# ZihaoW123/UniMM

Hardware: AMD Instinct MI355X
Metric: dialog-sequences/sec (fwd+bwd) at bs=240 seq=256 regions=36(+1 <IMG>) (higher is better)
Workload: dtype bf16; 1 GPU; UniMM-UL sparse training step (BASELINE configs[1]): bert_base_6layer_6conect, sequences_per_image=6, num_negative_samples=5, mask_prob=0.15, dropout on, MLM+UL / NSP / region-KL losses, fwd+bwd, optimizer step not included; global_batch=240, per_gpu_batch=240, seq_len=256, regions=37, parallelism=dp1, executor=eager launches, step_api=loss = combine(losses); loss.backward() (autograd, as train.py:164-168, :315)

## Files before the change

include/unimm_hip.h:

```cpp
#ifndef UNIMM_HIP_H
#define UNIMM_HIP_H

#include <stdint.h>

#ifdef __cplusplus
extern "C" {
#endif

#define UNIMM_OK 0
#define UNIMM_E_ARG (-1)
#define UNIMM_E_SHAPE (-2)
#define UNIMM_E_ALIGN (-3)
#define UNIMM_E_HIP (-4)

int unimm_version(void);
const char* unimm_arch(void);

enum {
  UNIMM_EPI_BIAS = 0,
  UNIMM_EPI_BIAS_GELU = 1,
  UNIMM_EPI_BIAS_DROP_RESID = 2,
  UNIMM_EPI_BIAS_RELU = 3,
  UNIMM_EPI_DGELU = 4,
  UNIMM_EPI_ADD = 5,
  UNIMM_EPI_MUL = 6,
  UNIMM_EPI_BIAS_GELU_DG = 7
};

typedef struct {
  const void* x;
  const void* w;
  const float* bias;
  const void* aux;
  void* out;
  void* out2;
  int32_t M, N, K;
  int32_t ldx, ldw, ldaux, ldo;
  int32_t epilogue;
  int32_t out_f32;
  uint32_t drop_key;
  uint32_t drop_thr;
  float drop_scale;
  const float* aux_mean;
  const float* aux_rstd;
  const float* aux_gamma;
  const float* aux_beta;
  int32_t tile;
  const uint32_t* drop_salt;
  void* splitk_ws;
  int64_t splitk_ws_bytes;
  int32_t splitk;
} unimm_gemm_nt_args;

int unimm_gemm_nt(const unimm_gemm_nt_args* args, void* stream);

typedef struct {
  const void* dy;
  const void* x;
  float* dw;
  float* dbias;
  int32_t M, N, K;
  int32_t lddy, ldx, lddw;
  const int32_t* m_dev;
  int32_t overwrite;
} unimm_gemm_tn_args;

int unimm_gemm_tn(const unimm_gemm_tn_args* args, void* stream);
int unimm_gemm_tn_grouped(const unimm_gemm_tn_args* args, int32_t count, void* stream);
int unimm_gemm_tn_grouped_ws(const unimm_gemm_tn_args* args, int32_t count, int32_t shared_chip, void* ws, int64_t ws_bytes,
                             void* stream);

typedef struct {
  const void* q; const void* k; const void* v;
  void* out;
  float* lse;
  const uint32_t* mask;
  const int32_t* q_off; const int32_t* q_len; const int32_t* k_off; const int32_t* k_len;
  int32_t B, H, Tq, Tk, D;
  int32_t ldq, ldk, ldv, ldo;
  int32_t mask_q_stride, mask_b_stride;
  float scale;
  uint32_t drop_key, drop_thr; float drop_scale;
  const uint32_t* drop_salt;
  const int32_t* ks_off; const int32_t* ks_len;
  int32_t ks_ins;
  const int32_t* order;
} unimm_attn_args;

int unimm_attn_fwd(const unimm_attn_args* args, void* stream);

int unimm_attn_probs(const unimm_attn_args* args, float* probs, void* stream);

typedef struct {
  const void* q; const void* k; const void* v; const void* out; const void* dout;
  const float* lse; float* delta;
  void* dq; void* dk; void* dv;
  const uint32_t* mask;
  const int32_t* q_off; const int32_t* q_len; const int32_t* k_off; const int32_t* k_len;
  int32_t B, H, Tq, Tk, D;
  int32_t ldq, ldk, ldv, ldo, lddo, lddq, lddk, lddv;
  int32_t mask_q_stride, mask_b_stride;
  float scale;
  uint32_t drop_key, drop_thr; float drop_scale;
  const uint32_t* drop_salt;
  const int32_t* order;
} unimm_attn_bwd_args;

int unimm_attn_bwd(const unimm_attn_bwd_args* args, void* stream);

enum { UNIMM_DT_U8 = 0, UNIMM_DT_I32 = 1, UNIMM_DT_I64 = 2, UNIMM_DT_F32 = 3 };

int unimm_mask_pack(const void* mask, int dtype, uint32_t* out, int64_t rows, int32_t t, void* stream);
int unimm_host_mask_pack(const void* mask, int dtype, uint32_t* out, int64_t rows, int32_t t, int32_t threads);
int unimm_host_memcpy(void* dst, const void* src, int64_t bytes, int32_t threads);
int unimm_mask_synth(const int32_t* mode, const int32_t* len, const int32_t* nans, uint32_t* text_words, uint32_t* co_words,
                     int32_t B, int32_t T, void* stream);

int unimm_plan_lengths(const uint32_t* text_words, int32_t t_q_stride, int32_t t_b_stride, const uint32_t* co_words,
                       int32_t c_q_stride, int32_t c_b_stride, int32_t R, const int32_t* labels, const int32_t* weights,
                       const float* nsp_weight, const int32_t* image_label, int32_t B, int32_t T, int32_t* header,
                       void* stream);
int unimm_plan_build(const int32_t* header, const int32_t* labels, const int32_t* weights, int32_t B, int32_t T,
                     int32_t* off, int32_t* lens, int64_t* rows, int64_t* inv, int32_t* lm_pos, int32_t* lm_idx,
                     int32_t* lm_label, int32_t* lm_weight, int32_t rows_cap, int32_t lm_cap, int32_t* dims_i, float* dims_f,
                     int32_t* order, void* stream);

int unimm_layernorm_fwd(const float* x, const float* gamma, const float* beta, float* y32, void* y16, float* mean,
                        float* rstd, int32_t M, int32_t H, float eps, uint32_t drop_key, uint32_t drop_thr,
                        float drop_scale, const uint32_t* drop_salt, void* stream);

int64_t unimm_colpartials_bytes(int32_t H);

int unimm_layernorm_bwd(const void* dy, const float* x, const float* mean, const float* rstd, const float* gamma,
                        void* dx, void* dx_drop, float* dgamma, float* dbeta, float* dbias, float* partials,
                        int32_t M, int32_t H, uint32_t drop_key, uint32_t drop_thr, float drop_scale,
                        uint32_t odrop_key, uint32_t odrop_thr, float odrop_scale, const uint32_t* drop_salt, void* stream);
int unimm_layernorm_bwd_partials(const void* dy, const float* x, const float* mean, const float* rstd, const float* gamma,
                                 void* dx, void* dx_drop, float* partials, int32_t M, int32_t H, uint32_t drop_key,
                                 uint32_t drop_thr, float drop_scale, uint32_t odrop_key, uint32_t odrop_thr,
                                 float odrop_scale, int32_t* blocks_out, const int32_t* m_dev, const uint32_t* drop_salt,
                                 void* stream);
#define UNIMM_FINISH_MAX 8
typedef struct {
  const float* partials;
  float* dst[4];
  int32_t blocks, nq, H, pad_;
} unimm_finish_desc;
int unimm_colpartials_finish_grouped(const unimm_finish_desc* descs, int32_t count, void* stream);

typedef struct {
  const int32_t* ids; const int32_t* pos; const int32_t* typ;
  const float* word; const float* post; const float* type; const float* ext;
  const float* gamma; const float* beta;
  int32_t M, H, type_vocab;
  float eps;
  uint32_t drop_key, drop_thr; float drop_scale;
  const int32_t* m_dev;
  const int64_t* rows;
  const uint32_t* drop_salt;
} unimm_embed_args;

int unimm_embed_fwd(const unimm_embed_args* args, float* y32, void* y16, void* stream);
int unimm_embed_bwd(const unimm_embed_args* args, const void* dy, float* dword, float* dpos, float* dtype,
                    float* dext, float* dgamma, float* dbeta, float* partials, void* stream);

int unimm_colsum(const void* dy, float* db, int32_t M, int32_t N, int32_t ld, void* stream);

int unimm_cast_f32_bf16(const float* src, void* dst, int64_t n, void* stream);
int unimm_transpose_cast(const float* src, void* dst, int32_t R, int32_t C, int32_t ldd, void* stream);
int unimm_transpose_bf16(const void* src, void* dst, int32_t R, int32_t C, int32_t lds, int32_t ldd, void* stream);
int unimm_sum_slabs_bf16(const float* slabs, int32_t count, int64_t stride, void* out, int64_t n, void* stream);
typedef struct {
  const float* src;
  void* dst;
  int32_t R, C, ldd, tile0;
} unimm_transpose_desc;
int unimm_transpose_cast_grouped(const unimm_transpose_desc* table, int32_t count, int32_t total_tiles, void* stream);

int unimm_pack_image(const float* feat, const float* loc, void* out, int32_t rows, int32_t F, int32_t ld, void* stream);

int unimm_mul_dropout(const float* a, const float* b, float* out, int64_t n, uint32_t drop_key, uint32_t drop_thr,
                      float drop_scale, const uint32_t* drop_salt, void* stream);
int unimm_mul_dropout_bwd(const float* a, const float* b, const float* dout, float* da, float* db, int64_t n,
                          uint32_t drop_key, uint32_t drop_thr, float drop_scale, const uint32_t* drop_salt, void* stream);

int unimm_sum_dropout(const float* a, const float* b, float* out, int64_t n, uint32_t drop_key, uint32_t drop_thr,
                      float drop_scale, const uint32_t* drop_salt, void* stream);
int unimm_sum_dropout_bwd(const float* a, const float* b, const float* dout, float* da, float* db, int64_t n,
                          uint32_t drop_key, uint32_t drop_thr, float drop_scale, const uint32_t* drop_salt, void* stream);

typedef struct {
  const float* a; const float* b; const float* bias; float* out; float* rowsum;
  int32_t M, N, K;
  int64_t sa_m, sa_k, sb_k, sb_n, ldo;
// ... 147 lines not shown
```

unimm_amd/bucket_plan.py:

```python
from __future__ import annotations

from typing import List, Tuple

from . import params as PM

ARENA_ALIGN = 64
CHIP_SLOTS = 256


def big_tiles_of(M: int, N: int, K: int) -> int:
    if N >= 256 and K >= 256 and M >= 1024:
        return ((N + 255) // 256) * ((K + 255) // 256)
    return 0


def flush_due(n_problems: int, tiles: int, rounds: int) -> bool:
    if n_problems >= 40:
        return True
    if tiles >= rounds * CHIP_SLOTS:
        return True
    waste = (-tiles) % CHIP_SLOTS
    return tiles >= max(2, rounds // 2) * CHIP_SLOTS - 32 and waste <= CHIP_SLOTS // 8


def arena_ranges(cfg) -> List[Tuple[str, int, int]]:
    out, off = [], 0
    for gname, items in PM.arena_groups(cfg):
        lo = off
        for _, shape in items:
            n = 1
            for s in shape:
                n *= s
            off += (n + ARENA_ALIGN - 1) // ARENA_ALIGN * ARENA_ALIGN
        out.append((gname, lo, off))
    return out


def _self_block(h, inter):
    return [(h, inter), (inter, h), (h, h), (3 * h, h)]


def backward_events(cfg, n_seq: int, text_rows: int, lm_rows: int, regions: int = 37, dual_stream: bool = True,
                    image_head_side: bool = True):
    del dual_stream
    H, Hv, Hb = cfg.hidden_size, cfg.v_hidden_size, cfg.bi_hidden_size
    I, Iv = cfg.intermediate_size, cfg.v_intermediate_size
    Mt, Mi = text_rows, n_seq * regions
    img = 1
    ev = []
    hs = img if image_head_side else 0
    ev.append(("w", hs, Mi, cfg.v_target_size, Hv))
    ev.append(("w", hs, Mi, Hv, Hv))
    if lm_rows > 0:
        ev.append(("w", 0, lm_rows, cfg.vocab_size, H))
        ev.append(("w", 0, lm_rows, H, H))
    ev.append(("b", "heads", False, True, False))
    sched = PM.encoder_schedule(cfg)
    entries = list(reversed(sched))
    pos = 0
    tail_done = False

    def image_tail():
        nonlocal tail_done
        if tail_done or any(k in ("c", "v") for k, _ in entries[pos:]):
            return
        tail_done = True
        ev.extend([("w", img, Mi, Hv, cfg.v_feature_size), ("w", img, Mi, Hv, 5)])
        ev.append(("b", "image_embeddings", bool(img), False, True))

    while pos < len(entries):
        image_tail()
        seg = []
        while pos < len(entries) and entries[pos][0] != "c":
            seg.append(entries[pos])
            pos += 1
        for kind, i in seg:
            if kind == "v":
                ev += [("w", img, Mi, n, k) for n, k in _self_block(Hv, Iv)]
                ev.append(("b", f"v{i}", bool(img), False, False))
        for kind, i in seg:
            if kind == "t":
                ev += [("w", 0, Mt, n, k) for n, k in _self_block(H, I)]
                ev.append(("b", f"t{i}", False, False, False))
        if pos < len(entries):
            _, i = entries[pos]
            pos += 1
            ev += [("w", img, Mi, Hv, Iv), ("w", img, Mi, Iv, Hv), ("w", img, Mi, Hv, Hb)]
            ev += [("w", 0, Mt, H, I), ("w", 0, Mt, I, H), ("w", 0, Mt, H, Hb)]
            ev += [("w", img, Mi, 3 * Hb, Hv), ("w", 0, Mt, 3 * Hb, H)]
            ev.append(("b", f"c{i}", False, False, False))
    image_tail()
    ev.append(("b", "text_embeddings", False, True, False))
    return ev


def hand_overs(cfg, n_seq, text_rows, lm_rows, regions=37, wgrad_group_rounds=2, dual_stream=True, image_head_side=True):
    q = [[], []]
    nq, nf = [0, 0], [0, 0]
    pending, calls, launches = [], [], []

    def flush(side):
        if q[side]:
            launches.append((side, len(q[side]), sum(big_tiles_of(*p) for p in q[side])))
        q[side] = []
        nf[side] = nq[side]

    def due(side):
        return flush_due(len(q[side]), sum(big_tiles_of(*p) for p in q[side]), wgrad_group_rounds)

    for e in backward_events(cfg, n_seq, text_rows, lm_rows, regions, dual_stream, image_head_side):
        if e[0] == "w":
            _, side, M, N, K = e
            q[side].append((M, N, K))
            nq[side] += 1
            continue
        _, group, on_side, force, force_img = e
        pending.append((group, nq[0], nq[1]))
        if q[1] and (force or force_img or due(1)):
            flush(1)
        if not on_side and (force or due(0)):
            flush(0)
        if on_side:
            continue
        ready = [p for p in pending if nf[0] >= p[1] and nf[1] >= p[2]]
        pending = [p for p in pending if p not in ready]
        calls += [(g, j + 1 < len(ready)) for j, (g, _, _) in enumerate(ready)]
    assert not pending, pending
    return calls, launches


def collectives(cfg, calls):
    ranges = {g: (lo, hi) for g, lo, hi in arena_ranges(cfg)}
    out, run = [], None
    for group, more in calls:
        lo, hi = ranges[group]
        if run and (run[0] == hi or run[1] == lo):
            run = [min(lo, run[0]), max(hi, run[1]), run[2] + 1]
        else:
            if run:
                out.append(tuple(run))
            run = [lo, hi, 1]
        if not more:
            out.append(tuple(run))
            run = None
    assert run is None
    return out


def exchange_plan(cfg, n_seq, text_rows, lm_rows, **kw):
    calls, launches = hand_overs(cfg, n_seq, text_rows, lm_rows, **kw)
    cs = collectives(cfg, calls)
    return dict(calls=calls, launches=launches, collectives=cs, bytes=[(hi - lo) * 4 for lo, hi, _ in cs])
```

unimm_amd/csrc/api.hip:

```cpp
#include "common.h"

extern "C" int unimm_version(void) { return 19; }
extern "C" const char* unimm_arch(void) { return "gfx950"; }
```

unimm_amd/csrc/gemm.hip:

```cpp
#include "gemm_nt.h"

struct ProfRec { hipEvent_t a, b; int variant; int tag; double flops; };
int unimm_nt_launch_cfg1(const GemmNtParams& p, int epi, bool out_f32, int want_persist, hipStream_t s, const NtSplit& sk);
int unimm_nt_launch_cfg3(const GemmNtParams& p, int epi, bool out_f32, int want_persist, hipStream_t s, const NtSplit& sk);
int unimm_nt_launch_cfg6(const GemmNtParams& p, int epi, bool out_f32, int want_persist, hipStream_t s, const NtSplit& sk);
int unimm_nt_launch_cfg7(const GemmNtParams& p, int epi, bool out_f32, int want_persist, hipStream_t s, const NtSplit& sk);
int unimm_nt_launch_cfg8(const GemmNtParams& p, int epi, bool out_f32, int want_persist, hipStream_t s, const NtSplit& sk);
int unimm_nt_launch_cfg9(const GemmNtParams& p, int epi, bool out_f32, int want_persist, hipStream_t s, const NtSplit& sk);
int unimm_nt_launch_cfg10(const GemmNtParams& p, int epi, bool out_f32, int want_persist, hipStream_t s, const NtSplit& sk);
int unimm_nt_launch_cfg12(const GemmNtParams& p, int epi, bool out_f32, int want_persist, hipStream_t s, const NtSplit& sk);
int unimm_nt_launch_cfg14(const GemmNtParams& p, int epi, bool out_f32, int want_persist, hipStream_t s, const NtSplit& sk);
int unimm_nt_launch_cfg15(const GemmNtParams& p, int epi, bool out_f32, int want_persist, hipStream_t s, const NtSplit& sk);

int unimm_cu_count() {
  static int n = 0;
  if (n == 0) {
    int dev = 0;
    hipDeviceProp_t prop;
    if (hipGetDevice(&dev) == hipSuccess && hipGetDeviceProperties(&prop, dev) == hipSuccess) n = prop.multiProcessorCount;
    if (n <= 0) n = 256;
    if (n < 8) n = 8;
  }
  return n;
}
// ... 562 lines not shown
      for (const Cand& c : cand) {
        const long tiles = (long)((p.M + c.bm - 1) / c.bm) * ((p.N + c.bn - 1) / c.bn);
        const long slots = (long)cus * c.w;
        const double area = (double)c.bm * c.bn / 65536.0;
        const long rem = tiles % slots;
        const double cost = ((double)(tiles / slots) * c.w + (rem ? (double)((rem + cus - 1) / cus) : 0.0)) * area / c.eff;
        if (cost < best) { best = cost; cfg = c.cfg; }
      }
    }
  }
  if (cfg == 8 && ((size_t)p.M * (size_t)p.ldx * 2 >= ((size_t)1 << 32) || (size_t)p.N * (size_t)p.ldw * 2 >= ((size_t)1 << 32))) cfg = 3;
  if (cfg == 8) return unimm_nt_launch_cfg8(p, epi, out_f32, wp, s, nosplit);
  if (cfg == 6) return unimm_nt_launch_cfg6(p, epi, out_f32, wp, s, nosplit);
  if (cfg == 7) return unimm_nt_launch_cfg7(p, epi, out_f32, wp, s, sk);
  if (cfg == 9) return unimm_nt_launch_cfg9(p, epi, out_f32, wp, s, sk);
  if (cfg == 10) return unimm_nt_launch_cfg10(p, epi, out_f32, wp, s, sk);
  if (cfg == 3) return unimm_nt_launch_cfg3(p, epi, out_f32, wp, s, nosplit);
  if (cfg == 12) return unimm_nt_launch_cfg12(p, epi, out_f32, wp, s, nosplit);
  if (cfg == 14) return unimm_nt_launch_cfg14(p, epi, out_f32, wp, s, sk);
  if (cfg == 15) return unimm_nt_launch_cfg15(p, epi, out_f32, wp, s, sk);
  return unimm_nt_launch_cfg1(p, epi, out_f32, wp, s, sk);
}

}

ProfRec* unimm_prof_begin(int variant, double flops, hipStream_t s) { return prof_begin(variant, flops, s); }
void unimm_prof_end(ProfRec* r, hipStream_t s) { prof_end(r, s); }

extern "C" int unimm_gemm_nt(const unimm_gemm_nt_args* a, void* stream) {
  if (a == nullptr || a->x == nullptr || a->w == nullptr || a->out == nullptr) return UNIMM_E_ARG;
  if (a->M <= 0 || a->N <= 0 || a->K <= 0 || (a->K % 64) != 0) return UNIMM_E_SHAPE;
  if ((a->ldx % 8) || (a->ldw % 8) || a->ldx < a->K || a->ldw < a->K || a->ldo < a->N) return UNIMM_E_ALIGN;
  if (((uintptr_t)a->x | (uintptr_t)a->w | (uintptr_t)a->out) & 15) return UNIMM_E_ALIGN;
  if (a->out_f32 ? (a->ldo % 4) : (a->ldo % 4)) return UNIMM_E_ALIGN;
  const bool needs_aux = a->epilogue == UNIMM_EPI_BIAS_DROP_RESID || a->epilogue == UNIMM_EPI_DGELU ||
                         a->epilogue == UNIMM_EPI_ADD || a->epilogue == UNIMM_EPI_MUL;
  if (needs_aux && (a->aux == nullptr || (a->ldaux % 4) || a->ldaux < a->N)) return UNIMM_E_ARG;
  if (a->epilogue == UNIMM_EPI_BIAS_DROP_RESID && !a->out_f32) return UNIMM_E_ARG;
  if (((needs_aux ? (uintptr_t)a->aux : 0) | (uintptr_t)a->out2) & 15) return UNIMM_E_ALIGN;
  GemmNtParams p;
  p.x = (const bf16_t*)a->x; p.w = (const bf16_t*)a->w; p.bias = a->bias; p.aux = a->aux;
  p.out = a->out; p.out2 = (bf16_t*)a->out2;
  p.M = a->M; p.N = a->N; p.K = a->K; p.ldx = a->ldx; p.ldw = a->ldw; p.ldaux = a->ldaux; p.ldo = a->ldo;
  p.drop.key = a->drop_key; p.drop.thr = a->drop_thr; p.drop.scale = a->drop_scale; p.drop.salt = a->drop_salt;
  const int n_ln = (a->aux_mean != nullptr) + (a->aux_rstd != nullptr) + (a->aux_gamma != nullptr) + (a->aux_beta != nullptr);
  if (n_ln != 0 && (n_ln != 4 || a->epilogue != UNIMM_EPI_BIAS_DROP_RESID)) return UNIMM_E_ARG;
  p.aux_mean = a->aux_mean; p.aux_rstd = a->aux_rstd; p.aux_gamma = a->aux_gamma; p.aux_beta = a->aux_beta;
  NtTune tune;
  if (!nt_tune_decode(a->tile, tune)) return UNIMM_E_ARG;
  p.gn = tune.gn > 0 ? tune.gn : 4;
  hipStream_t s = (hipStream_t)stream;
  const bool f32 = a->out_f32 != 0;
  p.ksplit = 1; p.slabs = nullptr; p.counters = nullptr;
  if (a->splitk != 0 && a->splitk != 1 && (a->splitk_ws == nullptr || a->splitk_ws_bytes < 32768 || ((uintptr_t)a->splitk_ws & 255) ||
                                           a->splitk > 8 || a->splitk < -1))
    return UNIMM_E_ARG;
  const NtSplit sk{a->splitk, a->splitk_ws, (long)a->splitk_ws_bytes};
  if (a->epilogue < 0 || a->epilogue > UNIMM_EPI_BIAS_GELU_DG) return UNIMM_E_ARG;
  return launch_nt(p, a->epilogue, f32, tune, s, sk);
}

namespace {

int check_tn(const unimm_gemm_tn_args* a) {
  if (a->dy == nullptr || a->x == nullptr || a->dw == nullptr) return UNIMM_E_ARG;
  if (a->M <= 0 || a->N <= 0 || a->K <= 0) return UNIMM_E_SHAPE;
  if ((a->lddy % 8) || (a->ldx % 8) || a->lddy < a->N || a->ldx < a->K || a->lddw < a->K) return UNIMM_E_ALIGN;
  if (((uintptr_t)a->dy | (uintptr_t)a->x) & 15) return UNIMM_E_ALIGN;
  return UNIMM_OK;
}

inline bool tn_is_big(const unimm_gemm_tn_args* a) { return a->N >= 256 && a->K >= 256 && a->M >= 1024; }

int launch_tn_group(const unimm_gemm_tn_args* const* a, int count, bool big, bool shared, bool legacy_loop, void* ws,
                    int64_t ws_bytes, hipStream_t s) {
  GemmTnGroup g;
  const int tb = big ? 256 : 128;
  int tiles = 0, max_m = 0;
  double flops = 0.0;
  const unimm_gemm_tn_args* sorted[TN_MAXG];
  for (int i = 0; i < count; ++i) sorted[i] = a[i];
#ifndef UNIMM_TN_NOSORT
  for (int i = 1; i < count; ++i) {
    const unimm_gemm_tn_args* x = sorted[i];
    int j = i - 1;
    while (j >= 0 && sorted[j]->M < x->M) { sorted[j + 1] = sorted[j]; --j; }
    sorted[j + 1] = x;
  }
#endif
  a = sorted;
  for (int i = 0; i < count; ++i) {
    GemmTnParams& p = g.pr[i];
    p.dy = (const bf16_t*)a[i]->dy; p.x = (const bf16_t*)a[i]->x; p.dw = a[i]->dw; p.dbias = a[i]->dbias;
    p.m_dev = a[i]->m_dev;
    p.overwrite = a[i]->overwrite;
    p.M = a[i]->M; p.N = a[i]->N; p.K = a[i]->K; p.lddy = a[i]->lddy; p.ldx = a[i]->ldx; p.lddw = a[i]->lddw;
    p.tile0 = tiles;
    tiles += ((p.N + tb - 1) / tb) * ((p.K + tb - 1) / tb);
    max_m = p.M > max_m ? p.M : max_m;
    flops += 2.0 * p.M * (double)p.N * p.K;
  }
  g.count = count; g.total_tiles = tiles;
  const int slots = big ? 256 : 512;
  int max_s = max_m / 1024;
  max_s = max_s < 1 ? 1 : (max_s > 32 ? 32 : max_s);
  int splits = 1;
// ... 148 lines not shown
```

unimm_amd/csrc/gemm_nt.h:

```cpp
#pragma once
#include <type_traits>
#include "common.h"
#include <stdlib.h>

struct GemmNtParams {
  const bf16_t* x; const bf16_t* w; const float* bias; const void* aux;
  void* out; bf16_t* out2;
  int M, N, K, ldx, ldw, ldaux, ldo;
  int gn;
  DropoutArg drop;
  const float* aux_mean; const float* aux_rstd; const float* aux_gamma; const float* aux_beta;
  int ksplit; float* slabs; int* counters;
};
struct NtSplit { int want; void* ws; long ws_bytes; };

struct ProfRec;
ProfRec* unimm_prof_begin(int variant, double flops, hipStream_t s);
void unimm_prof_end(ProfRec* r, hipStream_t s);
int unimm_cu_count();

namespace {

__device__ __forceinline__ void tile_of(int lid, int nbm, int nbn, int gn, int& tm, int& tn) {
  const int per_group = nbm * gn;
  const int g = lid / per_group;
  const int r = lid - g * per_group;
  const int gw = (nbn - g * gn) < gn ? (nbn - g * gn) : gn;
  tm = r / gw;
  tn = g * gn + (r - tm * gw);
}

template <int WM_, int WN_, int MT_, int BK_, int STAGES_, int PP_ = 0, int XS_ = 0>
struct Cfg {
  static constexpr int WM = WM_, WN = WN_, MT = MT_, BK = BK_, STAGES = STAGES_;
  static constexpr int XS = XS_ ? XS_ : STAGES_;
  static constexpr bool PP = PP_ != 0;
  static constexpr int BM = 16 * MT * WM, BN = 64 * WN, NW = WM * WN, THREADS = 64 * NW;
  static constexpr int ROWB = BK * 2;
  static constexpr int RPI = 1024 / ROWB;
  static constexpr int STAGE_BYTES = (BM + BN) * ROWB;
  static constexpr int G = (BM + BN) / RPI / NW;
  static constexpr int JP = MT == 6 ? 3 : (MT < 4 ? MT : 4);
  static constexpr int SLAB_ROWS = 16 * JP;
  static constexpr int SLAB_BYTES = NW * SLAB_ROWS * 68 * 4;
  static constexpr int WB = BN * ROWB, XB = BM * ROWB;
  static constexpr int GW = BN / RPI / NW, GX = BM / RPI / NW;
  static constexpr int RING_BYTES = STAGES * WB + XS * XB;
  static constexpr int LDS = RING_BYTES > SLAB_BYTES ? RING_BYTES : SLAB_BYTES;
  static constexpr int WG_PER_CU = LDS <= 53 * 1024 ? 3 : (LDS <= 80 * 1024 ? 2 : 1);
  static constexpr int MIN_WAVES = (WG_PER_CU * NW + 3) / 4;
  static_assert((BM + BN) % (RPI * NW) == 0, "tile rows must split evenly over the waves");
};

template <int BK> __device__ __forceinline__ int kswz(int row) { return BK == 64 ? ((row >> 1) & 7) : ((row >> 2) & 3); }

template <class C> struct RingStage {
  uint32_t so[C::G];
  u32x4 srd_w, srd_x;
  uint32_t lds;
};
template <class C>
__device__ __forceinline__ void ring_stage_init(RingStage<C>& st, const GemmNtParams& p, int n0, int m0, uint32_t lds0, int wave, int lane) {
  constexpr int CPR = C::ROWB / 16;
  static_assert(C::BN % (C::RPI * C::NW) == 0, "an LDS-DMA instruction round must not straddle the W / X boundary");
  const uint64_t bw = (uint64_t)(uintptr_t)(p.w + (size_t)n0 * p.ldw), bx = (uint64_t)(uintptr_t)(p.x + (size_t)m0 * p.ldx);
// ... 239 lines not shown
      (void)pfa1; (void)pfamu; (void)pfars;
      if (m >= p.M || !ncols_ok) continue;
      if constexpr (PRE) {
        uint32_t pw[8];
#pragma unroll
        for (int e = 0; e < 4; ++e) { pw[e] = __float_as_uint(lo[e]); pw[4 + e] = __float_as_uint(hi[e]); }
        bf16_t* op = reinterpret_cast<bf16_t*>(p.out) + (size_t)m * p.ldo + n;
        bf16_t* up = p.out2 != nullptr ? p.out2 + (size_t)m * p.ldo + n : nullptr;
        if (vec_out) {
          u32x4 ow, uw;
#pragma unroll
          for (int k2 = 0; k2 < 4; ++k2) {
            ow[k2] = __builtin_amdgcn_perm(pw[2 * k2 + 1], pw[2 * k2], 0x05040100u);
            uw[k2] = __builtin_amdgcn_perm(pw[2 * k2 + 1], pw[2 * k2], 0x07060302u);
          }
          __builtin_nontemporal_store(ow, reinterpret_cast<u32x4*>(op));
          if (up != nullptr) __builtin_nontemporal_store(uw, reinterpret_cast<u32x4*>(up));
        } else {
          for (int e = 0; e < 8; ++e)
            if (n + e < p.N) {
              op[e] = (bf16_t)(pw[e] & 0xffffu);
              if (up != nullptr) up[e] = (bf16_t)(pw[e] >> 16);
            }
        }
        continue;
      }
      float v[8], u[8];
#pragma unroll
      for (int e = 0; e < 4; ++e) { v[e] = lo[e] + b[e]; v[4 + e] = hi[e] + b[4 + e]; }
      if constexpr (EPI == UNIMM_EPI_BIAS_DROP_RESID || EPI == UNIMM_EPI_DGELU || EPI == UNIMM_EPI_ADD || EPI == UNIMM_EPI_MUL) {
        float a[8];
        if constexpr (EPI == UNIMM_EPI_BIAS_DROP_RESID) {
          const float* ap = reinterpret_cast<const float*>(p.aux) + (size_t)m * p.ldaux;
          if (vec_aux) {
            f32x4 r0, r1;
            if (PF > 0) { r0 = pfa0; r1 = pfa1; }
            else {
              r0 = __builtin_nontemporal_load(reinterpret_cast<const f32x4*>(ap + colA));
              r1 = __builtin_nontemporal_load(reinterpret_cast<const f32x4*>(ap + colB));
            }
#pragma unroll
            for (int e = 0; e < 4; ++e) { a[e] = r0[e]; a[4 + e] = r1[e]; }
          } else {
#pragma unroll
            for (int e = 0; e < 8; ++e) a[e] = (n + e < p.N) ? ap[n + e] : 0.f;
          }
          if (aux_ln) {
            const bool pfd = PF > 0 && (FAST || pf_on);
            const float mu = pfd ? pfamu : p.aux_mean[m], rs = pfd ? pfars : p.aux_rstd[m];
#pragma unroll
            for (int e = 0; e < 8; ++e) a[e] = (a[e] - mu) * rs * lg[e] + lb[e];
          }
          if (p.drop.thr != 0u) {
            const uint32_t kb = (SPLITCOL && FAST)
                ? (drop_bits4(p.drop, (uint32_t)m, (uint32_t)p.N, (uint32_t)colA) | (drop_bits4(p.drop, (uint32_t)m, (uint32_t)p.N, (uint32_t)colB) << 4))
                : drop_bits8(p.drop, (uint32_t)m, (uint32_t)p.N, (uint32_t)n);
#pragma unroll
            for (int e = 0; e < 8; ++e) v[e] = ((kb >> e) & 1u) ? v[e] * p.drop.scale : 0.f;
          }
#pragma unroll
          for (int e = 0; e < 8; ++e) v[e] += a[e];
        } else {
          const bf16_t* ap = reinterpret_cast<const bf16_t*>(p.aux) + (size_t)m * p.ldaux + n;
          if (vec_aux) {
            const u32x4 raw = PF > 0 ? __builtin_bit_cast(u32x4, pfa0)
                                     : __builtin_nontemporal_load(reinterpret_cast<const u32x4*>(ap));
#pragma unroll
            for (int e = 0; e < 4; ++e) { a[2 * e] = __uint_as_float(raw[e] << 16); a[2 * e + 1] = __uint_as_float(raw[e] & 0xffff0000u); }
          } else {
#pragma unroll
            for (int e = 0; e < 8; ++e) a[e] = (n + e < p.N) ? bf2f(ap[e]) : 0.f;
          }
          if constexpr (EPI == UNIMM_EPI_DGELU) {
#pragma unroll
            for (int e = 0; e < 8; ++e) v[e] *= gelu_erf_grad(a[e]);
          } else if constexpr (EPI == UNIMM_EPI_MUL) {
#pragma unroll
            for (int e = 0; e < 8; ++e) v[e] *= a[e];
          } else {
#pragma unroll
            for (int e = 0; e < 8; ++e) v[e] += a[e];
          }
        }
      }
      if constexpr (EPI == UNIMM_EPI_BIAS_GELU || EPI == UNIMM_EPI_BIAS_GELU_DG) {
        if constexpr (EPI == UNIMM_EPI_BIAS_GELU) {
#pragma unroll
          for (int e = 0; e < 8; ++e) { u[e] = v[e]; v[e] = gelu_erf(v[e]); }
        } else {
#pragma unroll
          for (int e = 0; e < 8; ++e) { const float x = v[e]; gelu_and_grad(x, v[e], u[e]); }
        }
        if (p.out2 != nullptr) {
          bf16_t* up = p.out2 + (size_t)m * p.ldo + n;
          if (full && (p.ldo % 8) == 0)
            __builtin_nontemporal_store(u32x4{pack2bf(u[0], u[1]), pack2bf(u[2], u[3]), pack2bf(u[4], u[5]), pack2bf(u[6], u[7])},
                                        reinterpret_cast<u32x4*>(up));
          else
            for (int e = 0; e < 8; ++e) if (n + e < p.N) up[e] = f2bf(u[e]);
        }
      }
      if constexpr (EPI == UNIMM_EPI_BIAS_RELU) {
#pragma unroll
        for (int e = 0; e < 8; ++e) v[e] = fmaxf(v[e], 0.f);
      }
      if constexpr (OUT_F32) {
        float* op = reinterpret_cast<float*>(p.out) + (size_t)m * p.ldo;
        if (vec_out) {
          __builtin_nontemporal_store(f32x4{v[0], v[1], v[2], v[3]}, reinterpret_cast<f32x4*>(op + colA));
// ... 454 lines not shown
```

unimm_amd/csrc/rowops.hip:

```cpp
#include "common.h"
#include "rows.h"

namespace {

template <typename T>
__global__ void mask_pack_ballot_kernel(const T* __restrict__ m, uint32_t* __restrict__ out, size_t ngroups) {
  const size_t wave = (size_t)blockIdx.x * (blockDim.x >> 6) + (threadIdx.x >> 6);
  const size_t nwaves = (size_t)gridDim.x * (blockDim.x >> 6);
  const int lane = threadIdx.x & 63;
  for (size_t g = wave; g < ngroups; g += nwaves) {
    const bool bit = m[g * 64 + lane] != (T)0;
    const unsigned long long bal = __ballot(bit);
    if (lane == 0) {
      out[2 * g] = (uint32_t)bal;
      out[2 * g + 1] = (uint32_t)(bal >> 32);
    }
  }
}

template <typename T>
__global__ void mask_pack_generic_kernel(const T* __restrict__ m, uint32_t* __restrict__ out, size_t rows, int t,
                                         int nw) {
  const size_t i = (size_t)blockIdx.x * blockDim.x + threadIdx.x;
  if (i >= rows * nw) return;
// ... 144 lines not shown
    if (rows != nullptr) for (int i = mv + t; i < rows_cap; i += 256) rows[i] = 0;
    if (lm_pos != nullptr)
      for (int i = nlm + t; i < lm_cap; i += 256) { lm_pos[i] = 0; lm_idx[i] = 0; lm_lab[i] = -1; lm_w[i] = 0; }
    if (order != nullptr)
      for (int i = t; i < B; i += 256) {
        const int li = header[i];
        int rank = 0;
        for (int j = 0; j < B; ++j) { const int lj = header[j]; rank += (lj > li || (lj == li && j < i)) ? 1 : 0; }
        order[rank] = i;
      }
    return;
  }
  int a = 0, c = 0;
  for (int i = t; i < b; i += 256) { a += header[i]; c += header[B + i]; }
  for (int o = 32; o > 0; o >>= 1) { a += __shfl_xor(a, o, 64); c += __shfl_xor(c, o, 64); }
  __shared__ int pa[4], pc[4];
  if ((t & 63) == 0) { pa[t >> 6] = a; pc[t >> 6] = c; }
  __syncthreads();
  if (t == 0) { s_off = pa[0] + pa[1] + pa[2] + pa[3]; s_lmoff = pc[0] + pc[1] + pc[2] + pc[3]; }
  __syncthreads();
  int len = header[b], o0 = s_off;
  if (rows != nullptr && o0 + len > rows_cap) {
    o0 = min(o0, rows_cap - 1);
    len = max(1, min(len, rows_cap - o0));
  }
  if (t == 0) { off[b] = o0; lens[b] = len; }
  if (t < T) {
    const bool in = t < len;
    if (in && rows != nullptr) rows[o0 + t] = (int64_t)b * T + t;
    if (inv != nullptr) inv[(size_t)b * T + t] = in ? (int64_t)(o0 + t) : (int64_t)-1;
  }
  if (labels == nullptr || lm_pos == nullptr) return;
  const int lab = t < T ? labels[(size_t)b * T + t] : -1;
  const int wt = (weights != nullptr && t < T) ? weights[(size_t)b * T + t] : 0;
  const bool sel = t < T && (weights != nullptr ? wt != 0 : lab != -1);
  const unsigned long long bal = __ballot(sel);
  const int lane = t & 63, wv = t >> 6;
  if (lane == 0) wave_cnt[wv] = __popcll(bal);
  __syncthreads();
  if (sel) {
    int r = __popcll(bal & ((1ull << lane) - 1ull));
    for (int w = 0; w < wv; ++w) r += wave_cnt[w];
    const int dst = s_lmoff + r;
    if (dst < lm_cap) {
      lm_pos[dst] = b * T + t;
      lm_idx[dst] = rows != nullptr ? min(o0 + t, rows_cap - 1) : o0 + t;
      lm_lab[dst] = lab;
      lm_w[dst] = weights != nullptr ? wt : 1;
    }
  }
}


__global__ __launch_bounds__(256) void layernorm_fwd_kernel(const float* __restrict__ x, const float* __restrict__ gamma,
                                                            const float* __restrict__ beta, float* __restrict__ y32,
                                                            bf16_t* __restrict__ y,
                                                            float* __restrict__ mean_o, float* __restrict__ rstd_o, int M,
                                                            int H, float eps, DropoutArg drop) {
  drop_resolve(drop);
  const int lane = threadIdx.x & 63;
  const int wave = blockIdx.x * (blockDim.x >> 6) + (threadIdx.x >> 6);
  const int nwaves = gridDim.x * (blockDim.x >> 6);
  Row8 g, b;
  load_vec_f32(gamma, H, lane, g);
  load_vec_f32(beta, H, lane, b);
  Row8 xv;
  if (wave < M) load_vec_f32(x + (size_t)wave * H, H, lane, xv);
  for (int row = wave; row < M; row += nwaves) {
    Row8 nx;
    const int nrow = row + nwaves;
    if (nrow < M) load_vec_f32(x + (size_t)nrow * H, H, lane, nx);
    float mean, rstd;
    row_stats(xv, H, mean, rstd, eps);
#pragma unroll
    for (int i = 0; i < MAXC; ++i) {
      const uint32_t kb = drop.thr != 0u ? drop_bits8(drop, (uint32_t)row, (uint32_t)H, (uint32_t)((lane + 64 * i) * 8)) : 0u;
#pragma unroll
      for (int j = 0; j < 8; ++j) {
        float v = (xv.v[i][j] - mean) * rstd * g.v[i][j] + b.v[i][j];
        if (drop.thr != 0u) v = ((kb >> j) & 1u) ? v * drop.scale : 0.f;
        xv.v[i][j] = v;
      }
    }
    if (y32 != nullptr) store_row_f32(y32 + (size_t)row * H, H, lane, xv);
    if (y != nullptr) store_row_bf16(y + (size_t)row * H, H, lane, xv);
    if (lane == 0 && mean_o != nullptr) { mean_o[row] = mean; rstd_o[row] = rstd; }
    if (nrow < M) xv = nx;
  }
}

__global__ __launch_bounds__(256) void layernorm_bwd_kernel(const bf16_t* __restrict__ dy, const float* __restrict__ x,
                                                            const float* __restrict__ mean_i,
                                                            const float* __restrict__ rstd_i,
                                                            const float* __restrict__ gamma, bf16_t* __restrict__ dx,
                                                            bf16_t* __restrict__ dx_drop, float* __restrict__ partials,
                                                            int M, int H, DropoutArg drop, DropoutArg out_drop,
                                                            const int32_t* __restrict__ m_dev) {
  __shared__ float red[4 * 1024];
  drop_resolve(drop);
  drop_resolve(out_drop);
  if (m_dev != nullptr) M = min(M, m_dev[0]);
  const int lane = threadIdx.x & 63, wv = threadIdx.x >> 6;
  const int wave = blockIdx.x * 4 + wv;
  const int nwaves = gridDim.x * 4;
  Row8 g;
  load_vec_f32(gamma, H, lane, g);
  Row8 dg, db, dbias;
#pragma unroll
  for (int i = 0; i < MAXC; ++i)
#pragma unroll
    for (int j = 0; j < 8; ++j) { dg.v[i][j] = 0.f; db.v[i][j] = 0.f; dbias.v[i][j] = 0.f; }
  const float invH = 1.0f / (float)H;
  u32x4 pdy[MAXC];
  f32x4 pxa[MAXC], pxb[MAXC];
  float pmean = 0.f, prstd = 0.f;
#define UNIMM_LNB_PREFETCH(r_)                                                                                 \
  {                                                                                                            \
    _Pragma("unroll") for (int i = 0; i < MAXC; ++i) {                                                         \
      const int c = lane + 64 * i;                                                                             \
      if (c * 8 < H) {                                                                                         \
        pdy[i] = *reinterpret_cast<const u32x4*>(dy + (size_t)(r_) * H + c * 8);                               \
        pxa[i] = *reinterpret_cast<const f32x4*>(x + (size_t)(r_) * H + c * 8);                                \
        pxb[i] = *reinterpret_cast<const f32x4*>(x + (size_t)(r_) * H + c * 8 + 4);                            \
      }                                                                                                        \
    }                                                                                                          \
    pmean = mean_i[r_]; prstd = rstd_i[r_];                                                                    \
  }
  if (wave < M) UNIMM_LNB_PREFETCH(wave)
  for (int row = wave; row < M; row += nwaves) {
    Row8 dyv, xv;
#pragma unroll
    for (int i = 0; i < MAXC; ++i) {
      if ((lane + 64 * i) * 8 < H) {
#pragma unroll
        for (int j = 0; j < 4; ++j) {
          dyv.v[i][2 * j] = __uint_as_float(pdy[i][j] << 16);
          dyv.v[i][2 * j + 1] = __uint_as_float(pdy[i][j] & 0xffff0000u);
          xv.v[i][j] = pxa[i][j];
          xv.v[i][4 + j] = pxb[i][j];
        }
      } else {
#pragma unroll
        for (int j = 0; j < 8; ++j) { dyv.v[i][j] = 0.f; xv.v[i][j] = 0.f; }
      }
    }
    const float mean = pmean, rstd = prstd;
    if (row + nwaves < M) UNIMM_LNB_PREFETCH(row + nwaves)
    float s1 = 0.f, s2 = 0.f;
#pragma unroll
    for (int i = 0; i < MAXC; ++i) {
      const uint32_t kbo = out_drop.thr != 0u ? drop_bits8(out_drop, (uint32_t)row, (uint32_t)H, (uint32_t)((lane + 64 * i) * 8)) : 0u;
#pragma unroll
      for (int j = 0; j < 8; ++j) {
        float d = dyv.v[i][j];
        if (out_drop.thr != 0u) d = ((kbo >> j) & 1u) ? d * out_drop.scale : 0.f;
        const float xh = (xv.v[i][j] - mean) * rstd;
        const float gg = d * g.v[i][j];
        dg.v[i][j] += d * xh;
        db.v[i][j] += d;
        s1 += gg;
        s2 += gg * xh;
        dyv.v[i][j] = gg;
        xv.v[i][j] = xh;
      }
    }
    s1 = wave_sum(s1) * invH;
    s2 = wave_sum(s2) * invH;
    Row8 dd;
#pragma unroll
    for (int i = 0; i < MAXC; ++i) {
      const uint32_t kb = drop.thr != 0u ? drop_bits8(drop, (uint32_t)row, (uint32_t)H, (uint32_t)((lane + 64 * i) * 8)) : 0u;
#pragma unroll
      for (int j = 0; j < 8; ++j) {
        const float v = rstd * (dyv.v[i][j] - s1 - xv.v[i][j] * s2);
        dyv.v[i][j] = v;
        float vd = v;
        if (drop.thr != 0u) vd = ((kb >> j) & 1u) ? v * drop.scale : 0.f;
        dd.v[i][j] = vd;
        dbias.v[i][j] += vd;
      }
    }
    store_row_bf16(dx + (size_t)row * H, H, lane, dyv);
    if (dx_drop != nullptr) store_row_bf16(dx_drop + (size_t)row * H, H, lane, dd);
  }
#undef UNIMM_LNB_PREFETCH
  float* redf = red;
  for (int qn = 0; qn < 3; ++qn) {
    const Row8& src = qn == 0 ? dg : (qn == 1 ? db : dbias);
    __syncthreads();
#pragma unroll
    for (int i = 0; i < MAXC; ++i)
#pragma unroll
      for (int j = 0; j < 8; ++j) {
        const int col = (lane + 64 * i) * 8 + j;
        if (col < H) redf[wv * 1024 + col] = src.v[i][j];
      }
    __syncthreads();
    for (int col = threadIdx.x; col < H; col += 256)
      partials[((size_t)blockIdx.x * 3 + qn) * H + col] =
          redf[col] + redf[1024 + col] + redf[2048 + col] + redf[3072 + col];
  }
}

__global__ __launch_bounds__(1024) void colpartials_finish_kernel(const float* __restrict__ partials, int nblocks, int nq,
                                                                  int H, float* d0, float* d1, float* d2, float* d3) {
  __shared__ float red[16][64];
  const int cl = threadIdx.x & 63, sl = threadIdx.x >> 6;
  const int col = blockIdx.x * 64 + cl;
  const int qn = blockIdx.y;
  float* dst = qn == 0 ? d0 : (qn == 1 ? d1 : (qn == 2 ? d2 : d3));
  float s = 0.f;
  if (col < H && dst != nullptr) {
    float s0 = 0.f, s1 = 0.f, s2 = 0.f, s3 = 0.f, s4 = 0.f, s5 = 0.f, s6 = 0.f, s7 = 0.f;
    int b = sl;
    const size_t st = (size_t)16 * nq * H;
    const float* pp = partials + ((size_t)b * nq + qn) * H + col;
    for (; b + 7 * 16 < nblocks; b += 8 * 16, pp += 8 * st) {
      s0 += pp[0]; s1 += pp[st]; s2 += pp[2 * st]; s3 += pp[3 * st];
      s4 += pp[4 * st]; s5 += pp[5 * st]; s6 += pp[6 * st]; s7 += pp[7 * st];
    }
    for (; b < nblocks; b += 16, pp += st) s0 += pp[0];
    s = ((s0 + s1) + (s2 + s3)) + ((s4 + s5) + (s6 + s7));
  }
  red[sl][cl] = s;
// ... 331 lines not shown
      }
    }
    *reinterpret_cast<u32x4*>(out + (size_t)row * ld + c) =
        u32x4{pack2bf(v[0], v[1]), pack2bf(v[2], v[3]), pack2bf(v[4], v[5]), pack2bf(v[6], v[7])};
  }
}

template <bool SUM>
__global__ void mul_dropout_kernel(const float* __restrict__ a, const float* __restrict__ b, float* __restrict__ out,
                                   size_t n, DropoutArg drop) {
  drop_resolve(drop);
  const size_t i = (size_t)blockIdx.x * blockDim.x + threadIdx.x;
  if (i >= n) return;
  float v = SUM ? a[i] + b[i] : a[i] * b[i];
  if (drop.thr != 0u) v = drop_apply(drop, 0u, (uint32_t)n, (uint32_t)i, v);
  out[i] = v;
}

template <bool SUM>
__global__ void mul_dropout_bwd_kernel(const float* __restrict__ a, const float* __restrict__ b,
                                       const float* __restrict__ dout, float* __restrict__ da, float* __restrict__ db,
                                       size_t n, DropoutArg drop) {
  drop_resolve(drop);
  const size_t i = (size_t)blockIdx.x * blockDim.x + threadIdx.x;
  if (i >= n) return;
  float d = dout[i];
  if (drop.thr != 0u) d = drop_apply(drop, 0u, (uint32_t)n, (uint32_t)i, d);
  const float av = a[i], bv = b[i];
  da[i] = av > 0.f ? (SUM ? d : d * bv) : 0.f;
  db[i] = bv > 0.f ? (SUM ? d : d * av) : 0.f;
}

__global__ void gelu_bwd_kernel(const bf16_t* __restrict__ dt, const bf16_t* __restrict__ u, bf16_t* __restrict__ du,
                                size_t n8) {
  size_t i = (size_t)blockIdx.x * blockDim.x + threadIdx.x;
  const size_t stride = (size_t)gridDim.x * blockDim.x;
  for (; i < n8; i += stride) {
    const u32x4 a = *reinterpret_cast<const u32x4*>(dt + i * 8);
    const u32x4 b = *reinterpret_cast<const u32x4*>(u + i * 8);
    u32x4 o;
#pragma unroll
    for (int j = 0; j < 4; ++j) {
      const float d0 = __uint_as_float(a[j] << 16), d1 = __uint_as_float(a[j] & 0xffff0000u);
      const float u0 = __uint_as_float(b[j] << 16), u1 = __uint_as_float(b[j] & 0xffff0000u);
      o[j] = pack2bf(d0 * gelu_erf_grad(u0), d1 * gelu_erf_grad(u1));
    }
    *reinterpret_cast<u32x4*>(du + i * 8) = o;
  }
}

__global__ void gather_rows_kernel(const bf16_t* __restrict__ src, const int32_t* __restrict__ idx, bf16_t* __restrict__ dst,
                                   int n, int H, int scatter, const int32_t* __restrict__ n_dev) {
  if (n_dev != nullptr) n = min(n, n_dev[0]);
  const int cpr = H / 8;
  size_t i = (size_t)blockIdx.x * blockDim.x + threadIdx.x;
  const size_t total = (size_t)n * cpr;
  const size_t stride = (size_t)gridDim.x * blockDim.x;
  for (; i < total; i += stride) {
    const int r = (int)(i / cpr), c = (int)(i % cpr) * 8;
    const int g = idx[r];
    if (scatter) *reinterpret_cast<u32x4*>(dst + (size_t)g * H + c) = *reinterpret_cast<const u32x4*>(src + (size_t)r * H + c);
    else *reinterpret_cast<u32x4*>(dst + (size_t)r * H + c) = *reinterpret_cast<const u32x4*>(src + (size_t)g * H + c);
  }
}

inline DropoutArg mk_drop(uint32_t key, uint32_t thr, float scale, const uint32_t* salt = nullptr) {
  DropoutArg d; d.key = key; d.thr = thr; d.scale = scale; d.salt = salt; d.key2 = 0u; return d;
}

}

extern "C" int unimm_mask_pack(const void* mask, int dtype, uint32_t* out, int64_t rows, int32_t t, void* stream) {
  if (!mask || !out || rows <= 0 || t <= 0) return UNIMM_E_ARG;
  hipStream_t s = (hipStream_t)stream;
  switch (dtype) {
    case UNIMM_DT_U8: return mask_pack_impl<uint8_t>(mask, out, (size_t)rows, t, s);
    case UNIMM_DT_I32: return mask_pack_impl<int32_t>(mask, out, (size_t)rows, t, s);
    case UNIMM_DT_I64: return mask_pack_impl<int64_t>(mask, out, (size_t)rows, t, s);
    case UNIMM_DT_F32: return mask_pack_impl<float>(mask, out, (size_t)rows, t, s);
    default: return UNIMM_E_ARG;
  }
}

extern "C" int unimm_layernorm_fwd(const float* x, const float* gamma, const float* beta, float* y32, void* y16, float* mean,
                                   float* rstd, int32_t M, int32_t H, float eps, uint32_t drop_key, uint32_t drop_thr,
                                   float drop_scale, const uint32_t* drop_salt, void* stream) {
  if (!x || !gamma || !beta || (!y32 && !y16)) return UNIMM_E_ARG;
  if (M <= 0 || H <= 0 || H > MAXC * 512 || (H % 8)) return UNIMM_E_SHAPE;
  int blocks = (M + 3) / 4;
  blocks = blocks > 2048 ? 2048 : blocks;
  hipLaunchKernelGGL(layernorm_fwd_kernel, dim3(blocks), dim3(256), 0, (hipStream_t)stream, x, gamma, beta, y32,
                     (bf16_t*)y16, mean, rstd, M, H, eps, mk_drop(drop_key, drop_thr, drop_scale, drop_salt));
  UNIMM_CHECK_LAUNCH();
  return UNIMM_OK;
}

extern "C" int64_t unimm_colpartials_bytes(int32_t H) { return (int64_t)RED_BLOCKS * 4 * H * sizeof(float); }

extern "C" int unimm_layernorm_bwd(const void* dy, const float* x, const float* mean, const float* rstd, const float* gamma,
                                   void* dx, void* dx_drop, float* dgamma, float* dbeta, float* dbias, float* partials,
                                   int32_t M, int32_t H, uint32_t drop_key, uint32_t drop_thr, float drop_scale,
                                   uint32_t odrop_key, uint32_t odrop_thr, float odrop_scale, const uint32_t* drop_salt,
                                   void* stream) {
  if (!dy || !x || !mean || !rstd || !gamma || !dx || !partials) return UNIMM_E_ARG;
  if (M <= 0 || H <= 0 || H > MAXC * 512 || (H % 8)) return UNIMM_E_SHAPE;
  int blocks = (M + 3) / 4;
  blocks = blocks > RED_BLOCKS ? RED_BLOCKS : blocks;
  hipStream_t s = (hipStream_t)stream;
  hipLaunchKernelGGL(layernorm_bwd_kernel, dim3(blocks), dim3(256), 0, s, (const bf16_t*)dy, x, mean, rstd,
                     gamma, (bf16_t*)dx, (bf16_t*)dx_drop, partials, M, H, mk_drop(drop_key, drop_thr, drop_scale, drop_salt),
                     mk_drop(odrop_key, odrop_thr, odrop_scale, drop_salt), (const int32_t*)nullptr);
  UNIMM_CHECK_LAUNCH();
  hipLaunchKernelGGL(colpartials_finish_kernel, dim3((H + 63) / 64, 3), dim3(1024), 0, s, partials, blocks, 3, H, dgamma,
                     dbeta, dbias, (float*)nullptr);
  UNIMM_CHECK_LAUNCH();
  return UNIMM_OK;
}

extern "C" int unimm_layernorm_bwd_partials(const void* dy, const float* x, const float* mean, const float* rstd,
                                            const float* gamma, void* dx, void* dx_drop, float* partials, int32_t M, int32_t H,
                                            uint32_t drop_key, uint32_t drop_thr, float drop_scale, uint32_t odrop_key,
                                            uint32_t odrop_thr, float odrop_scale, int32_t* blocks_out, const int32_t* m_dev,
                                            const uint32_t* drop_salt, void* stream) {
  if (!dy || !x || !mean || !rstd || !gamma || !dx || !partials || !blocks_out) return UNIMM_E_ARG;
  if (M <= 0 || H <= 0 || H > MAXC * 512 || (H % 8)) return UNIMM_E_SHAPE;
  int blocks = (M + 3) / 4;
  blocks = blocks > RED_BLOCKS ? RED_BLOCKS : blocks;
  hipLaunchKernelGGL(layernorm_bwd_kernel, dim3(blocks), dim3(256), 0, (hipStream_t)stream, (const bf16_t*)dy, x, mean, rstd,
                     gamma, (bf16_t*)dx, (bf16_t*)dx_drop, partials, M, H, mk_drop(drop_key, drop_thr, drop_scale, drop_salt),
                     mk_drop(odrop_key, odrop_thr, odrop_scale, drop_salt), m_dev);
  UNIMM_CHECK_LAUNCH();
  *blocks_out = blocks;
  return UNIMM_OK;
}

extern "C" int unimm_colpartials_finish_grouped(const unimm_finish_desc* descs, int32_t count, void* stream) {
  if (descs == nullptr || count < 1) return UNIMM_E_ARG;
  for (int base = 0; base < count; base += UNIMM_FINISH_MAX) {
    const int n = count - base < UNIMM_FINISH_MAX ? count - base : UNIMM_FINISH_MAX;
    FinishGroup g;
    int hmax = 0, qmax = 0;
    for (int i = 0; i < n; ++i) {
      const unimm_finish_desc& d = descs[base + i];
      if (d.partials == nullptr || d.blocks < 1 || d.nq < 1 || d.nq > 4 || d.H < 1) return UNIMM_E_ARG;
      g.d[i] = d;
      hmax = d.H > hmax ? d.H : hmax;
      qmax = d.nq > qmax ? d.nq : qmax;
    }
    hipLaunchKernelGGL(colpartials_finish_grouped_kernel, dim3((hmax + 63) / 64, qmax, n), dim3(1024), 0, (hipStream_t)stream, g);
    UNIMM_CHECK_LAUNCH();
  }
  return UNIMM_OK;
}

extern "C" int unimm_embed_fwd(const unimm_embed_args* a, float* y32, void* y, void* stream) {
  if (!a || !a->ids || !a->pos || !a->typ || !a->word || !a->post || !a->type || !a->ext || !a->gamma || !a->beta || !y ||
      !y32)
    return UNIMM_E_ARG;
  if (a->M <= 0 || a->H <= 0 || a->H > MAXC * 512 || (a->H % 8)) return UNIMM_E_SHAPE;
  EmbArgs e;
  e.ids = a->ids; e.pos = a->pos; e.typ = a->typ;
  e.word = a->word; e.post = a->post; e.type = a->type;
  e.ext = a->ext; e.gamma = a->gamma; e.beta = a->beta;
  e.M = a->M; e.H = a->H; e.type_vocab = a->type_vocab; e.eps = a->eps;
  e.drop = mk_drop(a->drop_key, a->drop_thr, a->drop_scale, a->drop_salt);
  e.m_dev = a->m_dev; e.rows = a->rows;
  int blocks = (a->M + 3) / 4;
  blocks = blocks > 2048 ? 2048 : blocks;
  hipLaunchKernelGGL(embed_fwd_kernel, dim3(blocks), dim3(256), 0, (hipStream_t)stream, e, y32, (bf16_t*)y);
  UNIMM_CHECK_LAUNCH();
  return UNIMM_OK;
}

namespace {
int embed_bwd_any(const unimm_embed_args* a, const void* dy, bool dy_f32, float* dword, float* dpos, float* dtype,
                  float* dext, float* dgamma, float* dbeta, float* partials, void* stream);
}
extern "C" int unimm_embed_bwd(const unimm_embed_args* a, const void* dy, float* dword, float* dpos, float* dtype,
                               float* dext, float* dgamma, float* dbeta, float* partials, void* stream) {
  return embed_bwd_any(a, dy, false, dword, dpos, dtype, dext, dgamma, dbeta, partials, stream);
}
extern "C" int unimm_embed_bwd_f32(const unimm_embed_args* a, const float* dy, float* dword, float* dpos, float* dtype,
                                   float* dext, float* dgamma, float* dbeta, float* partials, void* stream) {
  return embed_bwd_any(a, dy, true, dword, dpos, dtype, dext, dgamma, dbeta, partials, stream);
}
namespace {
int embed_bwd_any(const unimm_embed_args* a, const void* dy, bool dy_f32, float* dword, float* dpos, float* dtype,
                  float* dext, float* dgamma, float* dbeta, float* partials, void* stream) {
  if (!a || !dy || !dword || !dpos || !dtype || !dext || !dgamma || !dbeta || !partials) return UNIMM_E_ARG;
  if (a->M <= 0 || a->H <= 0 || a->H > MAXC * 512 || (a->H % 8) || a->type_vocab != 2) return UNIMM_E_SHAPE;
  EmbArgs e;
  e.ids = a->ids; e.pos = a->pos; e.typ = a->typ;
  e.word = a->word; e.post = a->post; e.type = a->type;
  e.ext = a->ext; e.gamma = a->gamma; e.beta = a->beta;
  e.M = a->M; e.H = a->H; e.type_vocab = a->type_vocab; e.eps = a->eps;
  e.drop = mk_drop(a->drop_key, a->drop_thr, a->drop_scale, a->drop_salt);
  e.m_dev = a->m_dev; e.rows = a->rows;
  int blocks = (a->M + 3) / 4;
  blocks = blocks > RED_BLOCKS ? RED_BLOCKS : blocks;
  hipStream_t s = (hipStream_t)stream;
  if (dy_f32) hipLaunchKernelGGL(embed_bwd_kernel<float>, dim3(blocks), dim3(256), 0, s, e, (const float*)dy, dword, dpos, dext, partials);
  else hipLaunchKernelGGL(embed_bwd_kernel<bf16_t>, dim3(blocks), dim3(256), 0, s, e, (const bf16_t*)dy, dword, dpos, dext, partials);
  UNIMM_CHECK_LAUNCH();
  hipLaunchKernelGGL(colpartials_finish_kernel, dim3((a->H + 63) / 64, 4), dim3(1024), 0, s, partials, blocks, 4, a->H,
                     dgamma, dbeta, dtype, dtype + a->H);
  UNIMM_CHECK_LAUNCH();
  return UNIMM_OK;
}
}

extern "C" int unimm_plan_lengths(const uint32_t* text_words, int32_t t_q_stride, int32_t t_b_stride, const uint32_t* co_words,
                                  int32_t c_q_stride, int32_t c_b_stride, int32_t R, const int32_t* labels, const int32_t* weights,
                                  const float* nsp_weight, const int32_t* image_label, int32_t B, int32_t T, int32_t* header,
                                  void* stream) {
  if (header == nullptr || (text_words == nullptr && co_words == nullptr && labels == nullptr)) return UNIMM_E_ARG;
  if (B <= 0 || T <= 0 || T > 256 || R < 0 || R > 256) return UNIMM_E_SHAPE;
  hipLaunchKernelGGL(plan_lengths_kernel, dim3(B), dim3(256), 0, (hipStream_t)stream, text_words, t_q_stride, t_b_stride,
                     co_words, c_q_stride, c_b_stride, R, labels, weights, nsp_weight, image_label, B, T, (T + 31) / 32, header);
  UNIMM_CHECK_LAUNCH();
  return UNIMM_OK;
}

extern "C" int unimm_plan_build(const int32_t* header, const int32_t* labels, const int32_t* weights, int32_t B, int32_t T,
                                int32_t* off, int32_t* lens, int64_t* rows, int64_t* inv, int32_t* lm_pos, int32_t* lm_idx,
                                int32_t* lm_label, int32_t* lm_weight, int32_t rows_cap, int32_t lm_cap, int32_t* dims_i,
                                float* dims_f, int32_t* order, void* stream) {
  if ((dims_i == nullptr) != (dims_f == nullptr)) return UNIMM_E_ARG;
  if (header == nullptr || off == nullptr || lens == nullptr) return UNIMM_E_ARG;
  if (lm_pos != nullptr && (lm_idx == nullptr || lm_label == nullptr || lm_weight == nullptr || labels == nullptr)) return UNIMM_E_ARG;
  if (B <= 0 || T <= 0 || T > 256) return UNIMM_E_SHAPE;
  hipLaunchKernelGGL(plan_build_kernel, dim3(B + 1), dim3(256), 0, (hipStream_t)stream, header, labels, weights, B, T, off, lens,
                     rows, inv, lm_pos, lm_idx, lm_label, lm_weight, rows_cap, lm_cap, dims_i, dims_f, order);
  UNIMM_CHECK_LAUNCH();
  return UNIMM_OK;
}

extern "C" int unimm_colsum(const void* dy, float* db, int32_t M, int32_t N, int32_t ld, void* stream) {
  if (!dy || !db) return UNIMM_E_ARG;
  if (M <= 0 || N <= 0 || (ld % 8) || ld < ((N + 7) & ~7)) return UNIMM_E_ALIGN;
  int ysplit = (M + 255) / 256;
  ysplit = ysplit > 64 ? 64 : ysplit;
  hipLaunchKernelGGL(colsum_kernel, dim3((N + 511) / 512, ysplit), dim3(256), 0, (hipStream_t)stream, (const bf16_t*)dy, db,
                     M, N, ld);
  UNIMM_CHECK_LAUNCH();
  return UNIMM_OK;
}

extern "C" int unimm_cast_f32_bf16(const float* src, void* dst, int64_t n, void* stream) {
  if (!src || !dst || n <= 0) return UNIMM_E_ARG;
  if (((uintptr_t)src | (uintptr_t)dst) & 15) return UNIMM_E_ALIGN;
  int64_t blocks = (n / 8 + 255) / 256;
  blocks = blocks > 4096 ? 4096 : (blocks < 1 ? 1 : blocks);
  hipLaunchKernelGGL(cast_f32_bf16_kernel, dim3((unsigned)blocks), dim3(256), 0, (hipStream_t)stream, src, (bf16_t*)dst,
                     (size_t)n);
  UNIMM_CHECK_LAUNCH();
  return UNIMM_OK;
}

extern "C" int unimm_transpose_cast(const float* src, void* dst, int32_t R, int32_t C, int32_t ldd, void* stream) {
  if (!src || !dst || R <= 0 || C <= 0 || ldd < R) return UNIMM_E_ARG;
  hipLaunchKernelGGL(transpose_cast_kernel, dim3((C + 31) / 32, (ldd + 31) / 32), dim3(256), 0, (hipStream_t)stream, src,
                     (bf16_t*)dst, R, C, ldd);
  UNIMM_CHECK_LAUNCH();
  return UNIMM_OK;
}

extern "C" int unimm_transpose_bf16(const void* src, void* dst, int32_t R, int32_t C, int32_t lds, int32_t ldd, void* stream) {
  if (!src || !dst || R <= 0 || C <= 0 || lds < C || ldd < R) return UNIMM_E_ARG;
  if ((lds % 8) || (ldd % 8) || (((uintptr_t)src | (uintptr_t)dst) & 15)) return UNIMM_E_ALIGN;
  hipLaunchKernelGGL(transpose_bf16_kernel, dim3((C + 63) / 64, (ldd + 63) / 64), dim3(256), 0, (hipStream_t)stream,
                     (const bf16_t*)src, (bf16_t*)dst, R, C, lds, ldd);
  UNIMM_CHECK_LAUNCH();
  return UNIMM_OK;
}

extern "C" int unimm_sum_slabs_bf16(const float* slabs, int32_t count, int64_t stride, void* out, int64_t n, void* stream) {
  if (!slabs || !out || count <= 0 || n <= 0 || stride < n) return UNIMM_E_ARG;
  if ((n % 8) || (stride % 4) || (((uintptr_t)slabs | (uintptr_t)out) & 15)) return UNIMM_E_ALIGN;
  int64_t blocks = (n / 8 + 255) / 256;
  blocks = blocks > 2048 ? 2048 : blocks;
  hipLaunchKernelGGL(sum_slabs_bf16_kernel, dim3((unsigned)blocks), dim3(256), 0, (hipStream_t)stream, slabs, count,
                     (size_t)stride, (bf16_t*)out, (size_t)(n / 8));
  UNIMM_CHECK_LAUNCH();
  return UNIMM_OK;
}

extern "C" int unimm_mask_synth(const int32_t* mode, const int32_t* len, const int32_t* nans, uint32_t* text_words,
                                uint32_t* co_words, int32_t B, int32_t T, void* stream) {
  if (!mode || !len || !nans || !text_words || !co_words || B <= 0 || T <= 0) return UNIMM_E_ARG;
// ... 26 lines not shown

extern "C" int unimm_mul_dropout(const float* a, const float* b, float* out, int64_t n, uint32_t drop_key, uint32_t drop_thr,
                                 float drop_scale, const uint32_t* drop_salt, void* stream) {
  if (!a || !b || !out || n <= 0) return UNIMM_E_ARG;
  hipLaunchKernelGGL(mul_dropout_kernel<false>, dim3((unsigned)((n + 255) / 256)), dim3(256), 0, (hipStream_t)stream,
                     a, b, out, (size_t)n, mk_drop(drop_key, drop_thr, drop_scale, drop_salt));
  UNIMM_CHECK_LAUNCH();
  return UNIMM_OK;
}

extern "C" int unimm_mul_dropout_bwd(const float* a, const float* b, const float* dout, float* da, float* db, int64_t n,
                                     uint32_t drop_key, uint32_t drop_thr, float drop_scale, const uint32_t* drop_salt,
                                     void* stream) {
  if (!a || !b || !dout || !da || !db || n <= 0) return UNIMM_E_ARG;
  hipLaunchKernelGGL(mul_dropout_bwd_kernel<false>, dim3((unsigned)((n + 255) / 256)), dim3(256), 0, (hipStream_t)stream,
                     a, b, dout, da, db, (size_t)n,
                     mk_drop(drop_key, drop_thr, drop_scale, drop_salt));
  UNIMM_CHECK_LAUNCH();
  return UNIMM_OK;
}

extern "C" int unimm_sum_dropout(const float* a, const float* b, float* out, int64_t n, uint32_t drop_key, uint32_t drop_thr,
                                 float drop_scale, const uint32_t* drop_salt, void* stream) {
  if (!a || !b || !out || n <= 0) return UNIMM_E_ARG;
  hipLaunchKernelGGL(mul_dropout_kernel<true>, dim3((unsigned)((n + 255) / 256)), dim3(256), 0, (hipStream_t)stream,
                     a, b, out, (size_t)n, mk_drop(drop_key, drop_thr, drop_scale, drop_salt));
  UNIMM_CHECK_LAUNCH();
  return UNIMM_OK;
}

extern "C" int unimm_sum_dropout_bwd(const float* a, const float* b, const float* dout, float* da, float* db, int64_t n,
                                     uint32_t drop_key, uint32_t drop_thr, float drop_scale, const uint32_t* drop_salt,
                                     void* stream) {
  if (!a || !b || !dout || !da || !db || n <= 0) return UNIMM_E_ARG;
  hipLaunchKernelGGL(mul_dropout_bwd_kernel<true>, dim3((unsigned)((n + 255) / 256)), dim3(256), 0, (hipStream_t)stream,
                     a, b, dout, da, db, (size_t)n,
                     mk_drop(drop_key, drop_thr, drop_scale, drop_salt));
  UNIMM_CHECK_LAUNCH();
  return UNIMM_OK;
}

extern "C" int unimm_gelu_bwd(const void* dt, const void* u, void* du, int64_t n, void* stream) {
  if (!dt || !u || !du || n <= 0 || (n % 8)) return UNIMM_E_ARG;
  int64_t blocks = (n / 8 + 255) / 256;
  blocks = blocks > 8192 ? 8192 : blocks;
  hipLaunchKernelGGL(gelu_bwd_kernel, dim3((unsigned)blocks), dim3(256), 0, (hipStream_t)stream, (const bf16_t*)dt,
                     (const bf16_t*)u, (bf16_t*)du, (size_t)(n / 8));
  UNIMM_CHECK_LAUNCH();
  return UNIMM_OK;
}

extern "C" int unimm_gather_rows(const void* src, const int32_t* idx, void* dst, int32_t n, int32_t H, int32_t scatter,
                                 const int32_t* n_dev, void* stream) {
  if (!src || !idx || !dst || n <= 0 || H <= 0 || (H % 8)) return UNIMM_E_ARG;
  size_t blocks = ((size_t)n * (H / 8) + 255) / 256;
  blocks = blocks > 8192 ? 8192 : blocks;
  hipLaunchKernelGGL(gather_rows_kernel, dim3((unsigned)blocks), dim3(256), 0, (hipStream_t)stream, (const bf16_t*)src, idx,
                     (bf16_t*)dst, n, H, scatter, n_dev);
  UNIMM_CHECK_LAUNCH();
  return UNIMM_OK;
}
```

unimm_amd/engine.py:

```python
from __future__ import annotations

import math
import zlib
from contextlib import contextmanager
from typing import Dict, List, Optional

import torch

from . import bucket_plan as BP
from . import dropout as DR
from . import lib as L
from . import params as PM
from .arena import FlatArena
from .inputs import DialogMaskSpec, HostStager, PackedMask

BF16 = torch.bfloat16
F32 = torch.float32


def _site(name: str) -> int:
    return zlib.crc32(name.encode()) & 0xFFFFFFFF


def _rup(x, m):
# ... 27 lines not shown
        self.arena: Optional[FlatArena] = None
        self.seed = 0x5EED
        self.step = 0
        self._w_version = None
        self.lin: Dict[str, _Lin] = {}
        self.ln: Dict[str, tuple] = {}
        self.grad_bucket_hook = None
        self._anchor = None
        self.last_seq_t = None
        self.unpad = True
        self._wq = []
        self.lazy_ln = True
        self.attn_longest_first = True
        self.wgrad_stream = False
        self._side = None
        self.dual_stream = True
        self._text_stream = None
        self._text_scope = None
        self._vside = None
        self.text_priority = False
        self._tstream = None
        self._on_side = False
        self._wq_img = []
        self._fq, self._fq_img = [], []
        self.last_plan = None
        self._arena_users = []
        self.wgrad_ws_bytes = 0
        self._wgrad_ws = {}
        self._plist = []
        self.gemm_tile = 0
        self.wgrad_group_rounds = 4
        self.row_bucket, self.lm_bucket = 1, 1
        self.salt_word = None
        self._inject_header = None
        self.graphs = None
        self.image_tile = 0
        self.wgrad_overwrite = True
        self._bwd_fresh = False
        self.debug_fresh = False
        self.tile_table = {}
        self.small_rows = 12000
        self._step_rows = None
        self.image_head_side = True
        self.attn_sink = None
        self.skinny_dx_rows = 3072
        self.prof_conn = None
        self.splitk = True
        self.splitk_ws_bytes = 48 << 20
        self._splitk_ws = {}
        self._pending = []
        self._nq = [0, 0]
        self._nf = [0, 0]
        self._reported = set()
        self.host_staging = True
        self._stager = None

    def schedule_key(self):
        return (self.dual_stream, self.unpad, self.lazy_ln, self.gemm_tile, self.wgrad_group_rounds, self.wgrad_stream, self.splitk,
                self.attn_longest_first, self.wgrad_overwrite, tuple(sorted(self.tile_table.items())), self.image_tile,
                self.small_rows, self.image_head_side, self.skinny_dx_rows, self.wgrad_ws_bytes, self.text_priority)

    def register_arena_user(self, obj):
        import weakref
        self._arena_users.append(weakref.ref(obj))

    def ensure(self, device):
        device = torch.device(device)
        if device.type != "cuda":
            raise L.UnimmHipError("unimm_amd runs on the GPU only (gfx950); move the model with .cuda() first")
        L.lib()
        if self.arena is not None and self.arena.is_current() and self.arena.device == device:
            return
        if self.arena is not None:
            users = [u() for u in self._arena_users]
            users = [type(u).__name__ for u in users if u is not None]
            if users:
                raise L.UnimmHipError(
                    "the model's parameters were re-pointed (module.to(), load_state_dict(assign=True), a replaced "
                    f"Parameter) while {', '.join(users)} still hold the engine's flat arena: build the optimizer / "
                    "data-parallel wrapper after the model has reached its final device")
        self.cfg.validate_for_hip()
        named = {n: p for n, p in self.model.named_parameters()}
        self.arena = FlatArena(named, PM.arena_groups(self.cfg), device=device, no_grad=PM.no_grad_names(self.cfg))
        A = self.arena
        self.w16 = torch.zeros(A.numel, dtype=BF16, device=device)
        self._anchor = torch.zeros(1, device=device, requires_grad=True)
        self._plist = list(named.values())
        self._build_tables(device)
        self._w_version = None
        self._wt_table = None

    def invalidate_weights(self):
        self._w_version = None

    def _weight_version(self):
        v = self.arena.flat._version
        for p in self._plist:
            v += p._version
        return v

    def _fused(self, names):
        A = self.arena
        o0, shape0 = A.offsets[names[0]]
        rows = sum(A.offsets[n][1][0] for n in names)
        tail = shape0[1:]
        n_el = rows * (tail[0] if tail else 1)
        shp = (rows,) + tail
        o = o0
        for n in names:
            oo, s = A.offsets[n]
            assert oo == o, f"arena layout: {n} not contiguous"
            o += s[0] * (s[1] if len(s) > 1 else 1)
        return (self.w16[o0:o0 + n_el].view(shp), A.flat[o0:o0 + n_el].view(shp), A.grad_flat[o0:o0 + n_el].view(shp))
# ... 60 lines not shown
        ln("lmtr", "cls.predictions.transform.LayerNorm")
        self._mk_lin("dec", [PM.WORD_EMB], None, device)
        d = self.lin["dec"]
        d.bias, d.gb = A.view("cls.predictions.bias"), A.grad("cls.predictions.bias")
        self._mk_lin("imgtr", ["cls.imagePredictions.transform.dense.weight"],
                     ["cls.imagePredictions.transform.dense.bias"], device)
        ln("imgtr", "cls.imagePredictions.transform.LayerNorm")
        self._mk_lin("imgdec", ["cls.imagePredictions.decoder.weight"], ["cls.imagePredictions.decoder.bias"], device)
        F = cfg.v_feature_size
        self.vemb_k = F + 64
        self.vemb_w = torch.zeros((cfg.v_hidden_size, self.vemb_k), dtype=BF16, device=device)
        self.vemb_b = torch.zeros(cfg.v_hidden_size, dtype=F32, device=device)
        e = "bert.embeddings."
        self.tab = {k: A.view(e + n + ".weight") for k, n in
                    (("word", "word_embeddings"), ("pos", "position_embeddings"), ("type", "token_type_embeddings"),
                     ("ext", "token_type_embeddings_extension"))}
        self.part = {h: torch.empty(L.colpartials_bytes(h) // 4, dtype=F32, device=device)
                     for h in {cfg.hidden_size, cfg.v_hidden_size}}
        self.part_side = {h: torch.empty(L.colpartials_bytes(h) // 4, dtype=F32, device=device)
                          for h in {cfg.hidden_size, cfg.v_hidden_size}}

    def refresh_weights(self, force=False, cast=True):
        A = self.arena
        ver = self._weight_version()
        if not force and ver == self._w_version:
            return
        if cast:
            L.cast_f32_bf16(A.flat, self.w16, A.numel)
        if self._wt_table is None:
            ents = []
            for key, wnames in self._wt_src:
                lin = self.lin[key]
                if lin.wt is None:
                    continue
                o0, _ = A.offsets[wnames[0]]
                ents.append((A.flat[o0:o0 + lin.N * lin.K].view(lin.N, lin.K), lin.wt))
            self._wt_table = L.transpose_table(ents, A.flat.device)
        L.transpose_cast_grouped(*self._wt_table)
        cfg = self.cfg
        F = cfg.v_feature_size
        v = "bert.v_embeddings."
        self.vemb_w[:, :F].copy_(A.view(v + "image_embeddings.weight"))
        self.vemb_w[:, F:F + 5].copy_(A.view(v + "image_location_embeddings.weight"))
        torch.add(A.view(v + "image_embeddings.bias"), A.view(v + "image_location_embeddings.bias"), out=self.vemb_b)
        self._w_version = ver

    def _drop(self, name, p, train):
        if not train or p <= 0.0:
            return L.NO_DROP
        if self.salt_word is not None:
            return DR.drop_arg(p, DR.site_key(self.seed, _site(name))) + (self.salt_word,)
        return DR.drop_arg(p, DR.make_key(self.seed, self.step, _site(name)))

    def _linear(self, x, lin, epi=L.EPI_BIAS, aux=None, want_u=False, drop=None, out_f32=False, ldo=None, M=None, out=None):
        M = x.shape[0] if M is None else M
        ldo = ldo or lin.N
        if out is None:
            out = torch.empty((M, ldo), dtype=F32 if out_f32 else BF16, device=x.device)
        u = torch.empty((M, ldo), dtype=BF16, device=x.device) if want_u else None
        aux_ln = None
        if isinstance(aux, _LazyLN):
            aux, aux_ln = aux.x, (aux.mean, aux.rstd, aux.gamma, aux.beta)
        sk = self._splitk(M, lin.N, lin.K)
        if sk is not None:
            L.gemm_nt(x, lin.w, out, bias=lin.bias, epilogue=epi, aux=aux, out2=u, drop=drop, M=M, N=lin.N, K=lin.K, aux_ln=aux_ln,
                      tile=sk[0], splitk=sk[1], splitk_ws=sk[2])
        else:
            L.gemm_nt(x, lin.w, out, bias=lin.bias, epilogue=epi, aux=aux, out2=u, drop=drop, M=M, N=lin.N, K=lin.K, aux_ln=aux_ln,
                      tile=self._tile(M, lin.N, lin.K))
        return (out, u) if want_u else out

    def _tile(self, M, N, K=None):
        if self.gemm_tile != 0:
            return self.gemm_tile
        if self._step_rows is None:
            return 0
        if self.tile_table and K is not None:
            code = self.tile_table.get(("i" if self._on_side else "t", N, K))
            if code is not None and self._step_rows < self.small_rows:
                return code
        if self._step_rows >= self.small_rows:
            return self.image_tile if (self._on_side and self.image_tile) else 0
        if self._on_side:
            return 14
        t128 = ((M + 127) // 128) * ((N + 127) // 128)
        return 7 if t128 < 256 else 1

    def _splitk(self, M, N, K):
        if not self.splitk or self._on_side or self.gemm_tile != 0 or self._step_rows is None or self._step_rows >= self.small_rows:
            return None
        if M != self._step_rows:
            return None
        if K < 2048 or N > 1024 or ((M + 127) // 128) * ((N + 127) // 128) > 256:
            return None
        dev = self.arena.flat.device
        key = int(torch.cuda.current_stream(dev).cuda_stream)
        ws = self._splitk_ws.get(key)
        if ws is None:
            ws = self._splitk_ws[key] = torch.zeros(self.splitk_ws_bytes, dtype=torch.uint8, device=dev)
        return 1, 2, ws

    def _linear32(self, x, key, relu=False, out=None):
        w32, b32 = self.lin32[key][:2]
        N, K = w32.shape
        M = x.shape[0]
        if out is None:
            out = torch.empty((M, N), dtype=F32, device=x.device)
        return L.linear_f32(x, w32, out, M, N, K, (x.stride(0), 1), (1, w32.stride(0)), bias=b32, relu=relu)

    def _linear32_bwd(self, dy, x, key):
        w32, _, gw, gb = self.lin32[key]
        N, K = w32.shape
        M = dy.shape[0]
        L.linear_f32(dy, x, gw, N, K, M, (1, dy.stride(0)), (x.stride(0), 1), accumulate=True, rowsum=gb)
        dx = torch.empty((M, K), dtype=F32, device=dy.device)
        return L.linear_f32(dy, w32, dx, M, K, N, (dy.stride(0), 1), (w32.stride(0), 1))

    def _wgrad(self, dy, x, gw, M, N, K, dbias=None, m_dev=None, sole=False):
        ow = bool(sole and self._bwd_fresh and self.wgrad_overwrite)
        (self._wq_img if self._on_side else self._wq).append((dy, x, gw, M, N, K, dbias, m_dev, ow))
        self._nq[1 if self._on_side else 0] += 1
        if self.prof_conn is not None:
# ... 151 lines not shown
        if not self._dual():
            was, self._on_side = self._on_side, True
            try:
                yield
            finally:
                self._on_side = was
            return
        side = self._side_stream()
        was, self._on_side = self._on_side, True
        main = self._text_stream
        if was or main is None or L.scoped_stream() is not self._text_scope:
            try:
                with torch.cuda.stream(side), L.stream_scope(side):
                    yield
            finally:
                self._on_side = was
            return
        torch.cuda.set_stream(side)
        try:
            with L.stream_scope(side):
                yield
        finally:
            torch.cuda.set_stream(main)
            self._on_side = was

    @contextmanager
    def _img_if(self, flag):
        if flag:
            with self._img():
                yield
        else:
            yield

    def _to_img(self, *reads):
        if not self._dual():
            return
        side = self._side_stream()
        ev = torch.cuda.Event()
        ev.record(torch.cuda.current_stream())
        side.wait_event(ev)
        for t in reads:
            self._touch(t, side)

    def _to_txt(self, *reads):
        if not self._dual() or self._vside is None:
            return
        main = torch.cuda.current_stream()
        ev = torch.cuda.Event()
        ev.record(self._vside)
        main.wait_event(ev)
        for t in reads:
            self._touch(t, main)

    def _layernorm_bwd(self, dy, x, mean, rstd, key, dbias=None, drop=L.NO_DROP, out_drop=L.NO_DROP, defer=True, m_dev=None):
        gmm, _, gg, gb = self.ln[key]
        M, H = x.shape
        dx = torch.empty((M, H), dtype=BF16, device=x.device)
        dxd = torch.empty((M, H), dtype=BF16, device=x.device) if drop[1] != 0 else None
        if not defer:
            scratch = (self.part_side if self._on_side else self.part)[H]
            L.layernorm_bwd(dy, x, mean, rstd, gmm, dx, dxd, gg, gb, dbias, scratch, M, H, drop=drop, out_drop=out_drop)
            return dx, (dxd if dxd is not None else dx)
        part = torch.empty(self.part[H].numel(), dtype=F32, device=x.device)
        blocks = L.layernorm_bwd_partials(dy, x, mean, rstd, gmm, dx, dxd, part, M, H, drop=drop, out_drop=out_drop, m_dev=m_dev)
        (self._fq_img if self._on_side else self._fq).append((part, blocks, H, [gg, gb, dbias]))
        return dx, (dxd if dxd is not None else dx)

    def _attn(self, q, k, v, mask, B, H, Tq, Tk, D, drop, save, qvar=None, kvar=None, tag=None):
        out = torch.empty((q.shape[0], H * D), dtype=BF16, device=q.device)
        lse = torch.empty((B, H, Tq), dtype=F32, device=q.device) if save else None
        words, mq, mb = mask
        L.attn_fwd(q, k, v, out, lse, words, B, H, Tq, Tk, D, 1.0 / math.sqrt(D), mq, mb, drop, qvar=qvar, kvar=kvar)
        if self.attn_sink is not None:
            if qvar is not None or kvar is not None:
                raise RuntimeError("attention probabilities are collected on the padded schedule only")
            probs = torch.empty((B, H, Tq, Tk), dtype=F32, device=q.device)
            L.attn_probs(q, k, probs, words, B, H, Tq, Tk, D, 1.0 / math.sqrt(D), mq, mb, drop)
            self.attn_sink[tag] = probs
        return out, lse

    def _self_block(self, key, x32, x, mask, B, T, heads, pname, p_attn, p_hid, st, var=None):
        train, tape = st["train"], st["tape"]
        save = tape is not None
        Hd = x.shape[1]
        D = Hd // heads
        qkv_l, so, ff1, ff2 = (self.lin[key + s] for s in (".qkv", ".so", ".ff1", ".ff2"))
        qkv = self._linear(x, qkv_l)
        q, k, v = qkv[:, :Hd], qkv[:, Hd:2 * Hd], qkv[:, 2 * Hd:]
        d_attn = self._drop(pname + "attn", p_attn, train)
        ctx, lse = self._attn(q, k, v, mask, B, heads, T, T, D, d_attn, save, qvar=var, kvar=var, tag=key)
        d_so = self._drop(pname + "so", p_hid, train)
        pre1 = self._linear(ctx, so, L.EPI_BIAS_DROP_RESID, aux=x32, drop=d_so, out_f32=True)
        x1_32, x1, m1, r1 = self._layernorm(pre1, key + ".ln1", save, lazy=True)
        h, u = self._linear(x1, ff1, L.EPI_BIAS_GELU_DG, want_u=True) if save else (self._linear(x1, ff1, L.EPI_BIAS_GELU), None)
        d_out = self._drop(pname + "out", p_hid, train)
        pre2 = self._linear(h, ff2, L.EPI_BIAS_DROP_RESID, aux=x1_32, drop=d_out, out_f32=True)
        x2_32, x2, m2, r2 = self._layernorm(pre2, key + ".ln2", save, lazy=True)
        md = var[2] if var is not None else None
        if save:
            def bwd(dx2):
                dpre2, dpre2d = self._layernorm_bwd(dx2, pre2, m2, r2, key + ".ln2", dbias=ff2.gb, drop=d_out, m_dev=md)
                du = self._linear_bwd(dpre2d, h, ff2, L.EPI_MUL, aux=u, bias_grad=False, m_dev=md)
                dx1 = self._linear_bwd(du, x1, ff1, L.EPI_ADD, aux=dpre2, m_dev=md)
                dpre1, dpre1d = self._layernorm_bwd(dx1, pre1, m1, r1, key + ".ln1", dbias=so.gb, drop=d_so, m_dev=md)
                dctx = self._linear_bwd(dpre1d, ctx, so, bias_grad=False, m_dev=md)
                dqkv = torch.empty_like(qkv)
                delta = torch.empty_like(lse)
                words, mq, mb = mask
                L.attn_bwd(q, k, v, ctx, dctx, lse, delta, dqkv[:, :Hd], dqkv[:, Hd:2 * Hd], dqkv[:, 2 * Hd:], words,
                           B, heads, T, T, D, 1.0 / math.sqrt(D), mq, mb, d_attn, qvar=var, kvar=var)
                return self._linear_bwd(dqkv, x, qkv_l, L.EPI_ADD, aux=dpre1, m_dev=md)
            tape.append((key, bwd))
        return x2_32, x2

    def _conn_block(self, key, i, xv32, xv, xt32, xt, B, R, T, vmask, comask, st, var=None):
        cfg = self.cfg
        train, tape = st["train"], st["tape"]
        save = tape is not None
        pn = f"bert.encoder.c_layer.{i}."
        Hb, nh = cfg.bi_hidden_size, cfg.bi_num_attention_heads
        D = Hb // nh
        lq1, lq2, d1, d2 = (self.lin[key + s] for s in (".qkv1", ".qkv2", ".d1", ".d2"))
        vff1, vff2, tff1, tff2 = (self.lin[key + s] for s in (".vff1", ".vff2", ".tff1", ".tff2"))
        with self._img():
            qkv1 = self._linear(xv, lq1)
        qkv2 = self._linear(xt, lq2)
        self._to_txt(qkv1)
        self._to_img(qkv2)
        q1, k1, v1 = qkv1[:, :Hb], qkv1[:, Hb:2 * Hb], qkv1[:, 2 * Hb:]
        q2, k2, v2 = qkv2[:, :Hb], qkv2[:, Hb:2 * Hb], qkv2[:, 2 * Hb:]
        da1 = self._drop(pn + "attn1", cfg.v_attention_probs_dropout_prob, train)
        da2 = self._drop(pn + "attn2", cfg.attention_probs_dropout_prob, train)
        db1 = self._drop(pn + "bo1", cfg.v_hidden_dropout_prob, train)
        db2 = self._drop(pn + "bo2", cfg.hidden_dropout_prob, train)
        dvo = self._drop(pn + "vout", cfg.v_hidden_dropout_prob, train)
        dto = self._drop(pn + "tout", cfg.hidden_dropout_prob, train)
        with self._img():
            ctx_v, lse_v = self._attn(q1, k2, v2, comask, B, nh, R, T, D, da2, save, kvar=var, tag=key + "/2")
            prev = self._linear(ctx_v, d1, L.EPI_BIAS_DROP_RESID, aux=xv32, drop=db1, out_f32=True)
            av32, av, mv1, rv1 = self._layernorm(prev, key + ".lnb1", save, lazy=True)
            if save:
                hv, uv = self._linear(av, vff1, L.EPI_BIAS_GELU_DG, want_u=True)
            else:
                hv, uv = self._linear(av, vff1, L.EPI_BIAS_GELU), None
            prev2 = self._linear(hv, vff2, L.EPI_BIAS_DROP_RESID, aux=av32, drop=dvo, out_f32=True)
            ov32, ov, mv2, rv2 = self._layernorm(prev2, key + ".lnv", save, lazy=True)
        ctx_t, lse_t = self._attn(q2, k1, v1, vmask, B, nh, T, R, D, da1, save, qvar=var, tag=key + "/1")
        pret = self._linear(ctx_t, d2, L.EPI_BIAS_DROP_RESID, aux=xt32, drop=db2, out_f32=True)
        at32, at, mt1, rt1 = self._layernorm(pret, key + ".lnb2", save, lazy=True)
        if save:
            ht, ut = self._linear(at, tff1, L.EPI_BIAS_GELU_DG, want_u=True)
        else:
            ht, ut = self._linear(at, tff1, L.EPI_BIAS_GELU), None
        pret2 = self._linear(ht, tff2, L.EPI_BIAS_DROP_RESID, aux=at32, drop=dto, out_f32=True)
        ot32, ot, mt2, rt2 = self._layernorm(pret2, key + ".lnt", save, lazy=True)
        md = var[2] if var is not None else None
        if save:
            def bwd(dov, dot):
                sc = 1.0 / math.sqrt(D)
                with self._img():
                    dqkv1 = torch.empty_like(qkv1)
                dqkv2 = torch.empty_like(qkv2)
                self._to_txt(dqkv1)
                self._to_img(dqkv2)
                with self._img():
# ... 63 lines not shown

    def _on_text_stream(self, fn, *args):
        if not self.arena.flat.is_cuda:
            return fn(*args)
        caller = torch.cuda.current_stream()
        if not (self.text_priority and self._dual()):
            self._text_stream = caller
            try:
                with L.stream_scope(caller) as sc:
                    self._text_scope = sc.ptr
                    return fn(*args)
            finally:
                self._text_stream = self._text_scope = None
        if self._tstream is None:
            self._tstream = torch.cuda.Stream(device=self.arena.flat.device, priority=-1)
        hp = self._tstream
        hp.wait_stream(caller)
        self._text_stream = hp
        try:
            with torch.cuda.stream(hp), L.stream_scope(hp) as sc:
                self._text_scope = sc.ptr
                return fn(*args)
        finally:
            self._text_stream = self._text_scope = None
            caller.wait_stream(hp)

    def enable_graphs(self, on=True, **kw):
        from .graphs import StepGraphs
        self.graphs = StepGraphs(self, **kw) if on else None
        return self.graphs

    def count_rows(self, inp: dict, lm_rows="labelled"):
        dev = self.arena.device
        ids, feat = inp["input_ids"], inp["image_feat"]
        B, T = ids.shape
        R = feat.shape[1]
        am, im, cm = inp.get("attention_mask"), inp.get("image_attention_mask"), inp.get("co_attention_mask")
        if am is None or isinstance(am, DialogMaskSpec) or cm is None:
            raise ValueError("count_rows needs dense attention_mask / co_attention_mask tensors")
        self._dev_masks = []
        tmask = self._pack_mask(am, dev, T)
        comask = self._pack_mask(cm, dev, R)
        self._dev_masks = []
        labels, weights = inp.get("masked_lm_labels"), inp.get("lm_weight")
        lab32 = self._i32(labels.reshape(B, T), dev) if labels is not None else None
        w32 = self._i32(weights.reshape(B, T), dev) if (weights is not None and labels is not None) else None
        il = inp.get("image_label")
        il32 = self._i32(il.reshape(B, R), dev) if (il is not None and inp.get("image_target") is not None) else None
        nw_in = inp.get("nsp_weight")
        nw_dev = nw_in.reshape(-1)[:2].to(F32).contiguous() if (torch.is_tensor(nw_in) and nw_in.is_cuda) else None
        header = L.plan_lengths(tmask, comask, R, lab32, w32, nw_dev, B, T, image_label=il32)
        return header.tolist()

    def forward(self, inp: dict, train: bool, save: bool, lm_rows: str, want_pred_v: bool):
        return self._on_text_stream(self._forward, inp, train, save, lm_rows, want_pred_v)

    def forward_with_attention(self, inp, train, lm_rows, want_pred_v):
        was = (self.unpad, self.dual_stream, self.attn_sink)
        self.unpad, self.dual_stream, self.attn_sink = False, False, {}
        try:
            out = self.forward(inp, train=train, save=False, lm_rows=lm_rows, want_pred_v=want_pred_v)
            sink = self.attn_sink
        finally:
            self.unpad, self.dual_stream, self.attn_sink = was

        def order(prefix):
            ks = [k for k in sink if k.startswith(prefix) and "/" not in k]
            return sorted(ks, key=lambda k: int("".join(ch for ch in k if ch.isdigit())))
        att_t = [sink[k] for k in order("t")]
        att_v = [sink[k] for k in order("v")]
        cs = sorted({k.split("/")[0] for k in sink if "/" in k}, key=lambda k: int("".join(ch for ch in k if ch.isdigit())))
        att_c = [(sink[k + "/1"], sink[k + "/2"]) for k in cs]
        return out, (att_t, att_v, att_c)

    def backward(self, out, g_lm, g_img, g_nsp, g_nsp_scores=None):
        return self._on_text_stream(self._backward, out, g_lm, g_img, g_nsp, g_nsp_scores)

    def losses(self, out, inp):
        return self._on_text_stream(self._losses, out, inp)

    def _prep_masks(self, inp, B, T, R, dev):
        ids, feat = inp["input_ids"], inp["image_feat"]
        am = inp.get("attention_mask")
        spec = am if isinstance(am, DialogMaskSpec) else None
        if spec is not None:
            if len(spec) != B or int(spec.length.max()) > T:
                raise ValueError(f"DialogMaskSpec for {len(spec)} sequences / max length {int(spec.length.max())} "
                                 f"does not fit input_ids of shape {tuple(ids.shape)}")
            if inp.get("co_attention_mask") is not None:
                raise ValueError("co_attention_mask must be None when attention_mask is a DialogMaskSpec (it is derived)")
            am = torch.ones((B, T), dtype=torch.uint8, device=dev)
        if am is None:
            am = torch.ones((B, T), dtype=torch.uint8, device=dev)
        if am.dim() not in (2, 3):
            raise ValueError(f"Wrong shape for txt input_ids (shape {tuple(ids.shape)}) or attention_mask (shape {tuple(am.shape)})")
        im = inp.get("image_attention_mask")
        if im is None:
            im = torch.ones((B, R), dtype=torch.uint8, device=dev)
        if im.dim() not in (2, 3):
            raise ValueError(f"Wrong shape for img input_ids (shape {tuple(feat.shape)}) or attention_mask (shape {tuple(im.shape)})")
        self._dev_masks = []
        if spec is not None:
            tw, cw = L.mask_synth(*spec.to_device(dev), T)
            nw = tw.shape[-1]
            tmask, comask = (tw, nw, T * nw), (cw, 0, nw)
            vmask = self._pack_mask(im, dev, R)
        else:
            cm = inp.get("co_attention_mask")
# ... 6 lines not shown
        self._dev_masks = []
        return tmask, vmask, comask

    def _prep_plan(self, inp, B, T, R, tmask, comask, lm_rows, dev):
        ids = inp["input_ids"]
        tt = inp.get("token_type_ids")
        ids32 = self._i32(ids.reshape(-1), dev)
        typ32 = self._i32(tt.reshape(-1), dev) if tt is not None else torch.zeros(B * T, dtype=torch.int32, device=dev)
        pos = inp.get("position_ids")
        pos32 = self._i32(pos.reshape(-1), dev) if pos is not None else \
            torch.arange(T, dtype=torch.int32, device=dev).repeat(B)
        labels, weights = inp.get("masked_lm_labels"), inp.get("lm_weight")
        want_sel = lm_rows == "labelled" and labels is not None
        lab32 = self._i32(labels.reshape(B, T), dev) if labels is not None else None
        w32 = self._i32(weights.reshape(B, T), dev) if (weights is not None and labels is not None) else None
        nw_in = inp.get("nsp_weight")
        nw_dev = nw_in.reshape(-1)[:2].to(F32).contiguous() if (torch.is_tensor(nw_in) and nw_in.is_cuda) else None
        il = inp.get("image_label")
        il32 = self._i32(il.reshape(B, R), dev) if (il is not None and inp.get("image_target") is not None) else None
        plan, sel, n_img = None, None, None
        dyn = None
        if self.unpad or want_sel or nw_dev is not None or il32 is not None:
            header = L.plan_lengths(tmask, comask, R, lab32, w32, nw_dev, B, T, image_label=il32)
            hh = self._inject_header if self._inject_header is not None else header.tolist()
            n_img = sum(hh[2 * B + 2:3 * B + 2]) if il32 is not None else None
            lens_h, n_lm = hh[:B], (sum(hh[B:2 * B]) if want_sel else 0)
            Mv = sum(lens_h)
            Mcap = min(_rup(Mv, self.row_bucket), B * T)
            ncap = _rup(n_lm, self.lm_bucket) if n_lm > 0 else 0
            unpadded = self.unpad and (Mv < B * T or self.row_bucket > 1)
            di, df = torch.zeros(8, dtype=torch.int32, device=dev), torch.zeros(8, dtype=F32, device=dev)
            built = L.plan_build(header, lab32 if want_sel else None, w32 if want_sel else None, B, T, Mcap if unpadded else Mv,
                                 ncap, want_rows=unpadded, dims=(di, df))
            dyn = dict(m=di[0:1], n_lm=di[1:2], n_img=di[2:3], inv_lm=df[0:1], inv_img=df[1:2])
            if unpadded:
                plan = dict(Mv=Mcap, lens_h=lens_h, rows=built["rows"], inv=built["inv"],
                            var=(built["off"], built["lens"], dyn["m"], built["order"] if self.attn_longest_first else None))
            if want_sel:
                sel = dict(n=ncap, pos=built["lm_pos"], idx=built["lm_idx"] if unpadded else built["lm_pos"],
                           label=built["lm_label"], weight=built["lm_weight"])
            if nw_dev is not None:
                import struct
                st_nspw = struct.unpack("<2f", struct.pack("<2i", hh[2 * B], hh[2 * B + 1]))
            else:
                st_nspw = None
        else:
            st_nspw = None
        self.last_plan = plan
        var = plan["var"] if plan is not None else None
        Mt = plan["Mv"] if plan is not None else B * T
        self._step_rows = Mt

        return dict(ids32=ids32, typ32=typ32, pos32=pos32, labels=labels, lab32=lab32, w32=w32, il32=il32, plan=plan, sel=sel,
                    n_img=n_img, dyn=dyn, st_nspw=st_nspw, var=var, Mt=Mt)

    def _forward(self, inp: dict, train: bool, save: bool, lm_rows: str, want_pred_v: bool):
        cfg = self.cfg
        dev = self.arena.device
        self.refresh_weights()
        ids = inp["input_ids"]
        B, T = ids.shape
        feat = inp["image_feat"]
        R = feat.shape[1]
        img_idx = inp.get("image_index")
        if img_idx is not None:
            img_idx = img_idx.to(dev, dtype=torch.int64, non_blocking=True).reshape(-1)
            if img_idx.numel() != B:
                raise ValueError("image_index needs one entry per sequence")
        elif feat.shape[0] != B:
            raise ValueError(f"image_feat has {feat.shape[0]} rows for {B} sequences and no image_index was given")
        if T > 256 or R > 256:
            raise ValueError("sequence / region count above 256 is not supported by the attention kernels")
        H, Hv = cfg.hidden_size, cfg.v_hidden_size
        st = dict(train=train, tape=[] if save else None)
        tape = st["tape"]

        tmask, vmask, comask = self._prep_masks(inp, B, T, R, dev)
        A = self.arena
        F = cfg.v_feature_size
        self._to_img()
        with self._img():
            featd = feat.to(dev, dtype=F32, non_blocking=True)
            locd = inp["image_loc"].to(dev, dtype=F32, non_blocking=True)
            if img_idx is not None:
                featd, locd = featd.index_select(0, img_idx), locd.index_select(0, img_idx)
            featd, locd = featd.contiguous().view(B * R, F), locd.contiguous().view(B * R, 5)
            packed = torch.empty((B * R, self.vemb_k), dtype=BF16, device=dev)
            L.pack_image(featd, locd, packed, B * R, F, self.vemb_k)
            prev = torch.empty((B * R, Hv), dtype=F32, device=dev)
            L.gemm_nt(packed, self.vemb_w, prev, bias=self.vemb_b, M=B * R, N=Hv, K=self.vemb_k)
            d_embv = self._drop("emb_v", cfg.hidden_dropout_prob, train)
            xv32, xv, mv, rv = self._layernorm(prev, "emb_v", save, drop=d_embv)
            if save:
                v = "bert.v_embeddings."

                def bwd_embv(dxv):
                    dbias = A.grad(v + "image_embeddings.bias")
                    before = dbias.clone()
                    dpre, _ = self._layernorm_bwd(dxv, prev, mv, rv, "emb_v", dbias=dbias, out_drop=d_embv, defer=False)
                    A.grad(v + "image_location_embeddings.bias").add_(dbias - before)
                    self._wgrad(dpre, packed, A.grad(v + "image_embeddings.weight"), B * R, Hv, F, sole=True)
                    self._wgrad(dpre, packed[:, F:], A.grad(v + "image_location_embeddings.weight"), B * R, Hv, 5, sole=True)

        pl = self._prep_plan(inp, B, T, R, tmask, comask, lm_rows, dev)
        ids32, typ32, pos32, labels = pl["ids32"], pl["typ32"], pl["pos32"], pl["labels"]
        il32, plan, sel, n_img, dyn, st_nspw, var, Mt = (pl[k] for k in ("il32", "plan", "sel", "n_img", "dyn", "st_nspw", "var", "Mt"))
        erows = plan["rows"] if plan is not None else None
        emd = plan["var"][2] if plan is not None else None
        gmm, bta, ggm, gbt = self.ln["emb_t"]
        d_embt = self._drop("emb_t", cfg.hidden_dropout_prob, train)
        xt = torch.empty((Mt, H), dtype=BF16, device=dev)
        xt32 = torch.empty((Mt, H), dtype=F32, device=dev)
        tabs = (self.tab["word"], self.tab["pos"], self.tab["type"], self.tab["ext"])
        L.embed_fwd(ids32, pos32, typ32, *tabs, gmm, bta, xt32, xt, Mt, H, cfg.type_vocab_size, drop=d_embt, m_dev=emd, rows=erows)
        A = self.arena
        e = "bert.embeddings."
        if save:
            def bwd_embt(dxt):
                L.embed_bwd(ids32, pos32, typ32, *tabs, gmm, bta, dxt, A.grad(e + "word_embeddings.weight"),
                            A.grad(e + "position_embeddings.weight"), A.grad(e + "token_type_embeddings.weight"),
                            A.grad(e + "token_type_embeddings_extension.weight"), ggm, gbt, self.part[H], Mt, H,
                            cfg.type_vocab_size, drop=d_embt, m_dev=emd, rows=erows)

        sched = PM.encoder_schedule(cfg)
        st_frozen = dict(train=train, tape=None)
        pos = 0
        while pos < len(sched):
            seg = []
            while pos < len(sched) and sched[pos][0] != "c":
                seg.append(sched[pos])
                pos += 1
            for kind, i in seg:
                if kind == "v":
                    fz = i < cfg.fixed_v_layer
                    with self._img():
                        xv32, xv = self._self_block(f"v{i}", xv32, xv, vmask, B, R, cfg.v_num_attention_heads,
                                                    f"bert.encoder.v_layer.{i}.", cfg.v_attention_probs_dropout_prob,
                                                    cfg.v_hidden_dropout_prob, st_frozen if fz else st)
                    if save and not fz:
                        tape[-1] = ("v", tape[-1][0], tape[-1][1])
            for kind, i in seg:
                if kind == "t":
                    fz = i < cfg.fixed_t_layer
                    xt32, xt = self._self_block(f"t{i}", xt32, xt, tmask, B, T, cfg.num_attention_heads, f"bert.encoder.layer.{i}.",
                                                cfg.attention_probs_dropout_prob, cfg.hidden_dropout_prob, st_frozen if fz else st, var=var)
                    if save and not fz:
                        tape[-1] = ("t", tape[-1][0], tape[-1][1])
            if pos < len(sched):
                i = sched[pos][1]
                pos += 1
                if cfg.with_coattention:
                    with self._conn_tag():
                        xv32, xv, xt32, xt = self._conn_block(f"c{i}", i, xv32, xv, xt32, xt, B, R, T, vmask, comask, st, var=var)
                    if save:
                        tape[-1] = ("c", tape[-1][0], tape[-1][1])
        img = None
        pred_v_out = None
        if want_pred_v or inp.get("image_target") is not None:
            with self._img_if(self.image_head_side):
                itr, idec = self.lin["imgtr"], self.lin["imgdec"]
                C = cfg.v_target_size
                if save:
                    tv, uvh = self._linear(xv, itr, L.EPI_BIAS_GELU, want_u=True, out_f32=True)
                else:
                    tv, uvh = self._linear(xv, itr, L.EPI_BIAS_GELU, out_f32=True), None
                _, hvn, mh, rh = self._layernorm(tv, "imgtr", save, want32=False)
                pred_v = self._linear(hvn, idec, out_f32=True, ldo=_rup(C, 4))
            pred_v_out = pred_v.view(B, R, -1)[:, :, :C]
            img = dict(tv=tv, u=uvh, hn=hvn, mean=mh, rstd=rh, pred=pred_v)
        self._to_txt(xv32, xv, img["pred"] if img is not None else None)
        seq_t, seq_v = xt, xv

        xt32, xv32 = self._dense32(xt32), self._dense32(xv32)
        out = dict(seq_out_t=seq_t, seq_out_v=seq_v, seq32_t=xt32, seq32_v=xv32, B=B, T=T, R=R, plan=plan, Mt=Mt,
                   nsp_weight_host=st_nspw, n_img=n_img, img_label32=il32, dyn=dyn, img=img)
        if pred_v_out is not None:
            out["pred_v"] = pred_v_out
        cls_idx_t = var[0] if var is not None else torch.arange(0, B * T, T, dtype=torch.int32, device=dev)
        cls_idx_v = torch.arange(0, B * R, R, dtype=torch.int32, device=dev)
        cls_t = torch.empty((B, H), dtype=F32, device=dev)
        cls_v = torch.empty((B, Hv), dtype=F32, device=dev)
        L.gather_rows(xt32.view(BF16), cls_idx_t, cls_t.view(BF16), B, 2 * H)
        L.gather_rows(xv32.view(BF16), cls_idx_v, cls_v.view(BF16), B, 2 * Hv)
        pooled_t = self._linear32(cls_t, "tpool", relu=True)
        pooled_v = self._linear32(cls_v, "vpool", relu=True)
        d_fuse = self._drop("fuse", 0.1, train)
        fused = torch.empty_like(pooled_t)
        L.mul_dropout(pooled_t, pooled_v, fused, fused.numel(), d_fuse, fusion_sum=cfg.fusion_method == "sum")
        nsp = torch.zeros((B, 4), dtype=F32, device=dev)
        self._linear32(fused, "nsp", out=nsp)
        out["nsp"] = nsp[:, :2]

        V = cfg.vocab_size
        Vp = _rup(V, 64)
        lmtr, dec = self.lin["lmtr"], self.lin["dec"]
        lm = None
        if lm_rows == "labelled" and labels is not None:
            n = sel["n"]
            if n > 0:
                xs = torch.empty((n, H), dtype=BF16, device=dev)
                L.gather_rows(seq_t, sel["idx"], xs, n, H, n_dev=dyn["n_lm"])
                lm = self._lm_head(xs, n, sel["label"], sel["weight"], save, n_dev=dyn["n_lm"])
                lm.update(idx=sel["idx"], pos_idx=sel["pos"], n=n, n_dev=dyn["n_lm"], inv_dev=dyn["inv_lm"])
            out["lm"] = lm
        elif lm_rows == "all":
            out["pred_t"] = self.decode_rows(self.padded(out, seq_t), B * T).view(B, T, Vp)[:, :, :V]

        if save:
            out["bwd"] = dict(tape=tape, embt=bwd_embt, embv=bwd_embv, pooled_t=pooled_t, pooled_v=pooled_v, fused=fused,
                              d_fuse=d_fuse, nsp_pad=nsp, cls_t=cls_t, cls_v=cls_v, cls_idx_t=cls_idx_t,
                              cls_idx_v=cls_idx_v)
        return out

    @staticmethod
    def padded(out, x):
        plan = out.get("plan")
        if plan is None:
            return x
        full = torch.zeros((out["B"] * out["T"], x.shape[1]), dtype=x.dtype, device=x.device)
        if "rows32" not in plan:
            plan["rows32"] = plan["rows"].to(torch.int32)
        w = 2 if x.dtype == F32 else 1
        L.gather_rows(x.view(BF16) if w == 2 else x, plan["rows32"], full.view(BF16) if w == 2 else full, x.shape[0],
                      w * x.shape[1], scatter=True, n_dev=plan["var"][2])
        return full

    def _lm_head(self, xs, n, lab_sel, w_sel, save, n_dev=None):
        cfg = self.cfg
        V = cfg.vocab_size
        Vp = _rup(V, 64)
        lmtr, dec = self.lin["lmtr"], self.lin["dec"]
        if save:
            t1, u = self._linear(xs, lmtr, L.EPI_BIAS_GELU, want_u=True, out_f32=True)
        else:
            t1, u = self._linear(xs, lmtr, L.EPI_BIAS_GELU, out_f32=True), None
        _, hn, mean, rstd = self._layernorm(t1, "lmtr", save, want32=False)
        logits = self._linear(hn, dec, out_f32=True, ldo=Vp)
        rowloss, rownll, lse = (torch.empty(n, dtype=F32, device=xs.device) for _ in range(3))
        L.lm_loss_fwd(logits, lab_sel, w_sel, rowloss, rownll, lse, n, V, n_dev=n_dev)
        return dict(xs=xs, t1=t1, u=u, hn=hn, mean=mean, rstd=rstd, logits=logits, rowloss=rowloss, rownll=rownll,
                    lse=lse, labels=lab_sel, weights=w_sel)

    def decode_rows(self, x, n):
        t1 = self._linear(x, self.lin["lmtr"], L.EPI_BIAS_GELU, M=n, out_f32=True)
        _, hn, _, _ = self._layernorm(t1, "lmtr", False, want32=False)
        return self._linear(hn, self.lin["dec"], out_f32=True, ldo=_rup(self.cfg.vocab_size, 64))

    def _losses(self, out, inp):
        cfg = self.cfg
        dev = self.arena.device
        B, R = out["B"], out["R"]
        res = {}
        lm = out.get("lm")
        lm_loss = torch.empty(1, dtype=F32, device=dev)
        if lm is None:
            lm_loss.fill_(float("nan"))
# ... 4 lines not shown
        C = cfg.v_target_size
        label = inp["image_label"]
        n_img = out["n_img"] if out.get("n_img") is not None else int((label == 1).sum())
        tgt = inp["image_target"].to(dev, dtype=F32, non_blocking=True)
        if inp.get("image_index") is not None and tgt.shape[0] != B:
            tgt = tgt.index_select(0, inp["image_index"].to(dev, dtype=torch.int64).reshape(-1))
        tgt = tgt.contiguous().view(B * R, C)
        lab32 = out["img_label32"].reshape(-1) if out.get("img_label32") is not None else self._i32(label.reshape(-1), dev)
        rl, lse = torch.empty(B * R, dtype=F32, device=dev), torch.empty(B * R, dtype=F32, device=dev)
        img_loss = torch.empty(1, dtype=F32, device=dev)
        if cfg.predict_feature:
            L.mse_loss_fwd(img["pred"], tgt, lab32, rl, B * R, C)
            inv_img, inv_img_dev = 1.0 / max(n_img, 1), None
        else:
            L.kl_loss_fwd(img["pred"], tgt, lab32, rl, lse, B * R, C)
            inv_img = 1.0 / n_img if n_img > 0 else float("inf")
            inv_img_dev = out["dyn"]["inv_img"] if (out.get("dyn") is not None and out.get("n_img") is not None) else None
        L.reduce_sum(rl, B * R, img_loss, inv_img, scale_dev=inv_img_dev)
        img.update(target=tgt, label=lab32, lse=lse, inv=inv_img, inv_dev=inv_img_dev)
        res["img_loss"] = img_loss
        nw = inp.get("nsp_weight")
        if nw is None:
            w0, w1 = 1.0, 1.0
        else:
            w = out["nsp_weight_host"] if out.get("nsp_weight_host") is not None else \
                [float(x) for x in nw.reshape(-1, 2)[0].tolist()]
            w0, w1 = 1.0, w[1] / w[0]
        nlab = self._i32(inp["next_sentence_label"].reshape(-1), dev)
        nsp_loss = torch.empty(1, dtype=F32, device=dev)
        L.nsp_loss_fwd(out["bwd"]["nsp_pad"] if "bwd" in out else out["nsp"], nlab, w0, w1, nsp_loss, B)
        out["nsp_state"] = (nlab, w0, w1)
        res["nsp_loss"] = nsp_loss
        return res

    def _backward(self, out, g_lm, g_img, g_nsp, g_nsp_scores=None):
        cfg = self.cfg
        dev = self.arena.device
        bw = out["bwd"]
        B, T, R = out["B"], out["T"], out["R"]
        H, Hv = cfg.hidden_size, cfg.v_hidden_size
        seq_t, seq_v = out["seq_out_t"], out["seq_out_v"]
        self.arena.attach_grads()
        self._bwd_fresh = bool(self.arena.fresh)
        self._reported = set()
        if self._bwd_fresh and self.debug_fresh and bool(self.arena.grad_flat.any()):
            raise RuntimeError("the gradient arena is marked fresh (zeroed since the last backward) but holds non-zero values: "
                               "something wrote into .grad / grad_flat between zero_grad() and backward() without clearing "
                               "`model.engine.arena.fresh` (INTEGRATION.md, 'Gradient arena')")
        self._step_rows = out["Mt"]

        def gvec(g):
            return torch.zeros(1, dtype=F32, device=dev) if g is None else g.detach().to(F32).reshape(1).contiguous()

        dseq_t = torch.zeros((out["Mt"], H), dtype=BF16, device=dev)
        img = out["img"]
        C = cfg.v_target_size
        itr, idec = self.lin["imgtr"], self.lin["imgdec"]
        Cp = idec.wt.shape[1]
        gimg = gvec(g_img)
        self._to_img(gimg, img["target"], img["lse"], img["label"])
        with self._img_if(self.image_head_side):
            dpred = torch.empty((B * R, Cp), dtype=BF16, device=dev)
            if cfg.predict_feature:
                L.mse_loss_bwd(img["pred"], img["target"], img["label"], gimg, img["inv"], dpred, B * R, C)
            else:
                L.kl_loss_bwd(img["pred"], img["target"], img["label"], img["lse"], gimg, img["inv"], dpred, B * R, C,
                              inv_dev=img.get("inv_dev"))
            dhn_v = self._linear_bwd(dpred, img["hn"], idec, M=B * R, N=C)
            dtv, _ = self._layernorm_bwd(dhn_v, img["tv"], img["mean"], img["rstd"], "imgtr")
            duv = torch.empty_like(dtv)
            L.gelu_bwd(dtv, img["u"], duv, duv.numel())
            dseq_v = self._linear_bwd(duv, seq_v, itr)
        lm = out.get("lm")
        if lm is not None:
            n, V = lm["n"], cfg.vocab_size
            Vp = _rup(V, 64)
            lmtr, dec = self.lin["lmtr"], self.lin["dec"]
            dlog = torch.empty((n, Vp), dtype=BF16, device=dev)
            nd = lm.get("n_dev")
            L.lm_loss_bwd(lm["logits"], lm["labels"], lm["weights"], lm["lse"], gvec(g_lm), 1.0 / n, dlog, n, V, n_dev=nd,
                          inv_dev=lm.get("inv_dev"))
            if n <= self.skinny_dx_rows:
                self._linear_bwd(dlog, lm["hn"], dec, M=n, N=V, m_dev=nd, need_dx=False)
                dhn = self._decoder_dx(dlog, dec, n, V)
            else:
                dhn = self._linear_bwd(dlog, lm["hn"], dec, M=n, N=V, m_dev=nd)
            dt1, _ = self._layernorm_bwd(dhn, lm["t1"], lm["mean"], lm["rstd"], "lmtr", m_dev=nd)
            du = torch.empty_like(dt1)
            L.gelu_bwd(dt1, lm["u"], du, du.numel())
            dxs = self._linear_bwd(du, lm["xs"], lmtr, m_dev=nd)
            L.gather_rows(dxs, lm["idx"], dseq_t, n, H, scatter=True, n_dev=nd)
        nlab, w0, w1 = out["nsp_state"]
        dnsp = torch.empty((B, 2), dtype=F32, device=dev)
        extra = None
        if g_nsp_scores is not None:
            extra = g_nsp_scores.detach().to(device=dev, dtype=F32).reshape(B, 2).contiguous()
        L.nsp_loss_bwd(bw["nsp_pad"], nlab, w0, w1, gvec(g_nsp), dnsp, B, extra=extra)
        dfused = self._linear32_bwd(dnsp, bw["fused"], "nsp")
        dpt, dpv = torch.empty_like(dfused), torch.empty_like(dfused)
        L.mul_dropout_bwd(bw["pooled_t"], bw["pooled_v"], dfused, dpt, dpv, dfused.numel(), bw["d_fuse"],
                          fusion_sum=cfg.fusion_method == "sum")
        dcls_t = self._linear32_bwd(dpt, bw["cls_t"], "tpool")
        L.rows_add_f32(dseq_t, bw["cls_idx_t"], dcls_t, B, dcls_t.shape[1])
        dcls_v = self._linear32_bwd(dpv, bw["cls_v"], "vpool")
        self._to_img(dcls_v)
        with self._img_if(self.image_head_side):
            L.rows_add_f32(dseq_v, bw["cls_idx_v"], dcls_v, B, dcls_v.shape[1])
# ... 73 lines not shown
```

unimm_amd/engine_x3.py:

```python
from __future__ import annotations

import math

import torch

from . import lib as L
from . import params as PM
from .engine import BF16, F32, Engine, _rup


class _Lin3:
    __slots__ = ("w32", "w3", "wt3", "bias", "gw", "gb", "N", "K", "Np", "Kp")

    def __init__(self, w32, bias, gw, gb, device, make_wt=True):
        self.w32, self.bias, self.gw, self.gb = w32, bias, gw, gb
        self.N, self.K = w32.shape
        self.Np, self.Kp = _rup(self.N, 64), _rup(self.K, 64)
        self.w3 = torch.zeros((self.N, 3 * self.Kp), dtype=BF16, device=device)
        self.wt3 = torch.zeros((self.K, 3 * self.Np), dtype=BF16, device=device) if make_wt else None


class EngineX3(Engine):
    compute_dtype = "fp32x3"

# ... 202 lines not shown
        da1 = self._drop(pn + "attn1", cfg.v_attention_probs_dropout_prob, train)
        da2 = self._drop(pn + "attn2", cfg.attention_probs_dropout_prob, train)
        db1 = self._drop(pn + "bo1", cfg.v_hidden_dropout_prob, train)
        db2 = self._drop(pn + "bo2", cfg.hidden_dropout_prob, train)
        dvo = self._drop(pn + "vout", cfg.v_hidden_dropout_prob, train)
        dto = self._drop(pn + "tout", cfg.hidden_dropout_prob, train)
        with self._img():
            ctx_v, ctx_v3, lse_v = self._attn(q1, k2, v2, comask, B, nh, R, T, D, da2, save, kvar=var, tag=key + "/2")
            prev = self._lin3(ctx_v3, d1, L.EPI_BIAS_DROP_RESID, aux=xv32, drop=db1)
            av32, av3, mv1, rv1 = self._ln3(prev, key + ".lnb1", save)
            uv = self._lin3(av3, vff1)
            hv3 = self._op3(uv, op=L.X3_GELU)[0]
            prev2 = self._lin3(hv3, vff2, L.EPI_BIAS_DROP_RESID, aux=av32, drop=dvo)
            ov32, ov3, mv2, rv2 = self._ln3(prev2, key + ".lnv", save)
        ctx_t, ctx_t3, lse_t = self._attn(q2, k1, v1, vmask, B, nh, T, R, D, da1, save, qvar=var, tag=key + "/1")
        pret = self._lin3(ctx_t3, d2, L.EPI_BIAS_DROP_RESID, aux=xt32, drop=db2)
        at32, at3, mt1, rt1 = self._ln3(pret, key + ".lnb2", save)
        ut = self._lin3(at3, tff1)
        ht3 = self._op3(ut, op=L.X3_GELU)[0]
        pret2 = self._lin3(ht3, tff2, L.EPI_BIAS_DROP_RESID, aux=at32, drop=dto)
        ot32, ot3, mt2, rt2 = self._ln3(pret2, key + ".lnt", save)
        md = var[2] if var is not None else None
        if save:
            def bwd(dov, dot):
                with self._img():
                    dqkv1 = self._qkv_grad(qkv1)
                dqkv2 = self._qkv_grad(qkv2)
                self._to_txt(dqkv1)
                self._to_img(dqkv2)
                with self._img():
                    dp, dpd3 = self._ln3_bwd(dov, prev2, mv2, rv2, key + ".lnv", dbias=vff2.gb, drop=dvo)
                    duv3 = self._op3(self._lin3_bwd(dpd3, hv3, vff2, bias_grad=False), op=L.X3_MUL_DGELU, b=uv)[0]
                    dav = self._lin3_bwd(duv3, av3, vff1, add=dp)
                    dprev, dprevd3 = self._ln3_bwd(dav, prev, mv1, rv1, key + ".lnb1", dbias=d1.gb, drop=db1)
                    dctx_v = self._lin3_bwd(dprevd3, ctx_v3, d1, bias_grad=False)
                    self._attn_bwd(q1, k2, v2, ctx_v, dctx_v, lse_v, comask, dqkv1[:, :Hb], dqkv2[:, Hb:2 * Hb], dqkv2[:, 2 * Hb:3 * Hb],
                                   3 * Hb, B, nh, R, T, D, da2, kvar=var)
                dp, dpd3 = self._ln3_bwd(dot, pret2, mt2, rt2, key + ".lnt", dbias=tff2.gb, drop=dto, m_dev=md)
                dut3 = self._op3(self._lin3_bwd(dpd3, ht3, tff2, bias_grad=False, m_dev=md), op=L.X3_MUL_DGELU, b=ut)[0]
                dat = self._lin3_bwd(dut3, at3, tff1, m_dev=md, add=dp)
                dpret, dpretd3 = self._ln3_bwd(dat, pret, mt1, rt1, key + ".lnb2", dbias=d2.gb, drop=db2, m_dev=md)
                dctx_t = self._lin3_bwd(dpretd3, ctx_t3, d2, bias_grad=False, m_dev=md)
                self._attn_bwd(q2, k1, v1, ctx_t, dctx_t, lse_t, vmask, dqkv2[:, :Hb], dqkv1[:, Hb:2 * Hb], dqkv1[:, 2 * Hb:3 * Hb],
                               3 * Hb, B, nh, T, R, D, da1, qvar=var)
                self._to_img()
                self._to_txt()
                with self._img():
                    dxv = self._lin3_bwd(self._qkv_grad3(dqkv1), xv3, lq1, add=dprev)
                dxt = self._lin3_bwd(self._qkv_grad3(dqkv2), xt3, lq2, m_dev=md, add=dpret)
                return dxv, dxt
            tape.append((key, bwd))
        return ov32, ov3, ot32, ot3

    def _forward(self, inp: dict, train: bool, save: bool, lm_rows: str, want_pred_v: bool):
        cfg = self.cfg
        if cfg.fixed_t_layer or cfg.fixed_v_layer or not cfg.with_coattention:
            raise NotImplementedError("fixed_t_layer / fixed_v_layer / with_coattention=False run on the bf16 engine only")
        dev = self.arena.device
        self.refresh_weights()
        ids = inp["input_ids"]
        B, T = ids.shape
        feat = inp["image_feat"]
        R = feat.shape[1]
        img_idx = inp.get("image_index")
        if img_idx is not None:
            img_idx = img_idx.to(dev, dtype=torch.int64, non_blocking=True).reshape(-1)
            if img_idx.numel() != B:
                raise ValueError("image_index needs one entry per sequence")
        elif feat.shape[0] != B:
            raise ValueError(f"image_feat has {feat.shape[0]} rows for {B} sequences and no image_index was given")
        if T > 256 or R > 256:
            raise ValueError("sequence / region count above 256 is not supported by the attention kernels")
        H, Hv = cfg.hidden_size, cfg.v_hidden_size
        st = dict(train=train, tape=[] if save else None)
        tape = st["tape"]
        tmask, vmask, comask = self._prep_masks(inp, B, T, R, dev)
        pl = self._prep_plan(inp, B, T, R, tmask, comask, lm_rows, dev)
        ids32, typ32, pos32, labels = pl["ids32"], pl["typ32"], pl["pos32"], pl["labels"]
        il32, plan, sel, n_img, dyn, st_nspw, var, Mt = (pl[k] for k in ("il32", "plan", "sel", "n_img", "dyn", "st_nspw", "var", "Mt"))
        A = self.arena
        F = cfg.v_feature_size

        self._to_img()
        with self._img():
            featd = feat.to(dev, dtype=F32, non_blocking=True)
            locd = inp["image_loc"].to(dev, dtype=F32, non_blocking=True)
            if img_idx is not None:
                featd, locd = featd.index_select(0, img_idx), locd.index_select(0, img_idx)
            packed32 = torch.zeros((B * R, self.vemb_k), dtype=F32, device=dev)
            packed32[:, :F].copy_(featd.reshape(B * R, F))
            packed32[:, F:F + 5].copy_(locd.reshape(B * R, 5))
            packed3 = self._split(packed32)
            prev = torch.empty((B * R, Hv), dtype=F32, device=dev)
            L.gemm_nt(packed3, self.vemb_w3, prev, bias=self.vemb_b, M=B * R, N=Hv, K=3 * self.vemb_k)
            d_embv = self._drop("emb_v", cfg.hidden_dropout_prob, train)
            xv32, xv3, mv, rv = self._ln3(prev, "emb_v", save, drop=d_embv)
            if save:
                v = "bert.v_embeddings."

                def bwd_embv(dxv):
                    _, dpre3 = self._ln3_bwd(dxv, prev, mv, rv, "emb_v", dbias=A.grad(v + "image_embeddings.bias"), out_drop=d_embv,
                                             want32=False, dbias2=A.grad(v + "image_location_embeddings.bias"))
                    K3 = self.vemb_k
                    self._wgrad3(dpre3, packed3, A.grad(v + "image_embeddings.weight"), B * R, Hv, F, Hv, K3)
                    self._wgrad3(dpre3, packed3, A.grad(v + "image_location_embeddings.weight"), B * R, Hv, 5, Hv, K3, xcol0=F)

        erows = plan["rows"] if plan is not None else None
# ... 164 lines not shown
```

unimm_amd/graphs.py:

```python
from __future__ import annotations

import contextlib
import gc
import weakref
from collections import OrderedDict

import torch

from . import dropout as DR
from . import lib as L
from .inputs import PackedMask

_TENSOR_KEYS = ("input_ids", "image_feat", "image_loc", "token_type_ids", "position_ids", "attention_mask",
                "image_attention_mask", "co_attention_mask", "masked_lm_labels", "image_label", "image_target",
                "next_sentence_label", "lm_weight", "image_index")


def _rup(x, m):
    return (x + m - 1) // m * m


_KEPT = []
_FREE_POOLS = {}

# ... 162 lines not shown
                self.stats["eager"] += 1
                return None
            ent = self._capture_forward(sig, inp, opts, hh)
        else:
            self.entries.move_to_end(sig)
            for k, t in ent.sin.items():
                if isinstance(t, PackedMask):
                    t.words.copy_(inp[k].words, non_blocking=True)
                elif torch.is_tensor(t) and t is not inp[k]:
                    t.copy_(inp[k], non_blocking=True)
        ent.salt_val = self._set_salt()
        self._replay(ent.gF)
        self.stats["replays"] += 1
        tok = _Token()
        ent.inflight = weakref.ref(tok)
        ent.out["_token"] = tok
        if defer_outputs:
            return None, None, None, None, ent
        return self.outputs(ent) + (ent,)

    @staticmethod
    def outputs(ent):
        ls = ent.lvec.clone()
        return ls[0].reshape(ent.lshape), ls[1].reshape(ent.lshape), ls[2].reshape(ent.lshape), ent.nsp.clone()

    def _capture_forward(self, sig, inp, opts, hh):
        eng = self.eng
        dev = eng.arena.device
        while len(self.entries) >= self.max_entries:
            self.entries.popitem(last=False)
        ent = _Entry()
        side = int(eng._side_stream().cuda_stream) if eng._dual() else 0
        ent.pool, ent.stream = _take_pool(dev, sig, side)
        weakref.finalize(ent, _give_pool, _dev_index(dev), sig, side, ent.pool, ent.stream)
        ent.sin = {k: (v.clone() if torch.is_tensor(v) and v.is_cuda else
                       (PackedMask(v.words.clone(), v.shape) if isinstance(v, PackedMask) else v)) for k, v in inp.items()}
        ent.gB, ent.gin, ent.gkey = None, None, None
        ent.inflight, ent.salt_val = None, None
        was = (eng.row_bucket, eng.lm_bucket, eng.salt_word, eng._inject_header)
        if self.salt is None:
            self._set_salt()
        eng.row_bucket, eng.lm_bucket, eng.salt_word, eng._inject_header = self.row_bucket, self.lm_bucket, self.salt, hh
        try:
            ent.stream.wait_stream(torch.cuda.current_stream())
            with torch.cuda.stream(ent.stream):
                with torch.no_grad():
                    out = eng.forward(ent.sin, train=opts["train"], save=False, lm_rows="labelled", want_pred_v=True)
                    eng.losses(out, ent.sin)
                del out
            torch.cuda.current_stream().wait_stream(ent.stream)
            torch.cuda.synchronize()
            ent.gF = _new_graph()
            with _quiet_collector(), torch.cuda.graph(ent.gF, pool=ent.pool, stream=ent.stream, capture_error_mode="thread_local"):
                ent.out = eng.forward(ent.sin, train=opts["train"], save=True, lm_rows="labelled", want_pred_v=True)
                ent.losses = eng.losses(ent.out, ent.sin)
                ent.nsp = ent.out["nsp"]
                ls = ent.losses
                ent.lshape = tuple(ls["lm_loss"].shape)
                ent.lvec = torch.stack([ls["lm_loss"].reshape(()), ls["img_loss"].reshape(()), ls["nsp_loss"].reshape(())])
        finally:
            eng.row_bucket, eng.lm_bucket, eng.salt_word, eng._inject_header = was
        self.entries[sig] = ent
        self.stats["captures"] += 1
        return ent

    def _capture_backward(self, ent):
        eng = self.eng
        prog, cur = [], [None]
        hook = eng.grad_bucket_hook

        def begin():
            g = _new_graph()
            g.capture_begin(pool=ent.pool, capture_error_mode="thread_local")
            cur[0] = g

        def end():
            cur[0].capture_end()
            prog.append(cur[0])
            cur[0] = None

        def cut(group, more=False):
            if cur[0] is not None:
                end()
            prog.append((group, more))
            if not more and group != "text_embeddings":
                begin()
                eng._to_img()

        was = (eng.row_bucket, eng.lm_bucket, eng.salt_word)
        eng.row_bucket, eng.lm_bucket, eng.salt_word = self.row_bucket, self.lm_bucket, self.salt
        if hook is not None:
            eng.grad_bucket_hook = cut
        try:
            torch.cuda.synchronize()
            ent.stream.wait_stream(torch.cuda.current_stream())
            with _quiet_collector(), torch.cuda.stream(ent.stream):
                begin()
                try:
                    eng.backward(ent.out, *ent.gin)
                finally:
                    if cur[0] is not None:
                        end()
            torch.cuda.current_stream().wait_stream(ent.stream)
        finally:
            eng.row_bucket, eng.lm_bucket, eng.salt_word = was
            eng.grad_bucket_hook = hook
        if hook is not None and not any(isinstance(i, tuple) and i[0] == "text_embeddings" for i in prog):
# ... 38 lines not shown
```

unimm_amd/lib.py:

```python
from __future__ import annotations

import ctypes as C
import os
import threading

import torch

_PKG = os.path.dirname(os.path.abspath(__file__))
LIB_PATH = os.path.join(_PKG, "libunimm_hip.so")
ABI_VERSION = 19

EPI_BIAS, EPI_BIAS_GELU, EPI_BIAS_DROP_RESID, EPI_BIAS_RELU, EPI_DGELU, EPI_ADD, EPI_MUL, EPI_BIAS_GELU_DG = range(8)

_ERR = {-1: "UNIMM_E_ARG", -2: "UNIMM_E_SHAPE", -3: "UNIMM_E_ALIGN", -4: "UNIMM_E_HIP"}


class UnimmHipError(RuntimeError):
    pass


class GemmNtArgs(C.Structure):
    _fields_ = [("x", C.c_void_p), ("w", C.c_void_p), ("bias", C.c_void_p), ("aux", C.c_void_p),
                ("out", C.c_void_p), ("out2", C.c_void_p),
                ("M", C.c_int32), ("N", C.c_int32), ("K", C.c_int32),
                ("ldx", C.c_int32), ("ldw", C.c_int32), ("ldaux", C.c_int32), ("ldo", C.c_int32),
                ("epilogue", C.c_int32), ("out_f32", C.c_int32),
                ("drop_key", C.c_uint32), ("drop_thr", C.c_uint32), ("drop_scale", C.c_float),
                ("aux_mean", C.c_void_p), ("aux_rstd", C.c_void_p), ("aux_gamma", C.c_void_p), ("aux_beta", C.c_void_p),
                ("tile", C.c_int32), ("drop_salt", C.c_void_p),
                ("splitk_ws", C.c_void_p), ("splitk_ws_bytes", C.c_int64), ("splitk", C.c_int32)]


class GemmTnArgs(C.Structure):
    _fields_ = [("dy", C.c_void_p), ("x", C.c_void_p), ("dw", C.c_void_p), ("dbias", C.c_void_p),
                ("M", C.c_int32), ("N", C.c_int32), ("K", C.c_int32),
                ("lddy", C.c_int32), ("ldx", C.c_int32), ("lddw", C.c_int32), ("m_dev", C.c_void_p), ("overwrite", C.c_int32)]


_lib = None


def lib():
    global _lib
    if _lib is not None:
        return _lib
    path = os.environ.get("UNIMM_HIP_LIB", LIB_PATH)
    if not os.path.exists(path):
        raise UnimmHipError(
            f"{path} is missing: build it with `python -m unimm_amd.build` (hipcc, gfx950). "
            "unimm_amd has no CPU or PyTorch fallback for its kernels.")
    L = C.CDLL(path)
    L.unimm_version.restype = C.c_int
    L.unimm_arch.restype = C.c_char_p
    if L.unimm_version() != ABI_VERSION:
        raise UnimmHipError(f"libunimm_hip.so ABI {L.unimm_version()} != expected {ABI_VERSION}: rebuild")
    for name in SYMBOLS:
        fn = getattr(L, name)
        if name == "unimm_colpartials_bytes":
            fn.restype = C.c_int64
        elif name != "unimm_arch":
            fn.restype = C.c_int
    VP, I32, U32, F32, I64 = C.c_void_p, C.c_int32, C.c_uint32, C.c_float, C.c_int64
    L.unimm_gemm_nt.argtypes = [VP, VP]
    L.unimm_attn_fwd.argtypes = [VP, VP]
    L.unimm_attn_bwd.argtypes = [VP, VP]
    L.unimm_x3_split.argtypes = [VP, VP]
    L.unimm_x3_attn_fwd.argtypes = [VP, VP, VP]
    L.unimm_x3_attn_bwd.argtypes = [VP, VP, VP]
    L.unimm_attn_probs.argtypes = [VP, VP, VP]
    L.unimm_attn_decode.argtypes = [VP, VP]
    L.unimm_kv_cache_update.argtypes = [VP, VP]
    L.unimm_lm_topk.argtypes = [VP, I32, I32, I32, VP, I32, VP, I32, I32, VP, VP, VP, VP]
    L.unimm_gemm_tn_grouped.argtypes = [VP, I32, VP]
    L.unimm_gemm_tn_grouped_ws.argtypes = [VP, I32, I32, VP, I64, VP]
    L.unimm_colpartials_finish_grouped.argtypes = [VP, I32, VP]
    L.unimm_layernorm_fwd.argtypes = [VP] * 7 + [I32, I32, F32, U32, U32, F32, VP, VP]
    L.unimm_x3_layernorm_fwd.argtypes = [VP] * 7 + [I32, I32, F32, U32, U32, F32, VP, VP]
    L.unimm_layernorm_bwd_partials.argtypes = [VP] * 8 + [I32, I32, U32, U32, F32, U32, U32, F32, VP, VP, VP, VP]
    L.unimm_layernorm_bwd.argtypes = [VP] * 11 + [I32, I32, U32, U32, F32, U32, U32, F32, VP, VP]
    _lib = L
    return L


SYMBOLS = ["unimm_version", "unimm_arch", "unimm_gemm_nt", "unimm_gemm_tn", "unimm_gemm_tn_grouped", "unimm_attn_fwd", "unimm_attn_bwd",
           "unimm_mask_pack", "unimm_layernorm_fwd", "unimm_colpartials_bytes", "unimm_layernorm_bwd",
           "unimm_embed_fwd", "unimm_embed_bwd", "unimm_colsum", "unimm_cast_f32_bf16", "unimm_transpose_cast",
           "unimm_pack_image", "unimm_mul_dropout", "unimm_mul_dropout_bwd", "unimm_lm_loss_fwd",
           "unimm_lm_loss_bwd", "unimm_kl_loss_fwd", "unimm_kl_loss_bwd", "unimm_nsp_loss_fwd",
           "unimm_nsp_loss_bwd", "unimm_reduce_sum", "unimm_segment_sum", "unimm_gelu_bwd", "unimm_gather_rows", "unimm_prof_enable", "unimm_prof_collect", "unimm_adamw_step", "unimm_transpose_cast_grouped", "unimm_mask_synth", "unimm_neural_ndcg", "unimm_plan_lengths", "unimm_plan_build", "unimm_layernorm_bwd_partials",
           "unimm_colpartials_finish_grouped", "unimm_gemm_tn_grouped_ws", "unimm_linear_f32", "unimm_rows_add_f32", "unimm_transpose_bf16", "unimm_sum_slabs_bf16", "unimm_attn_probs",
           "unimm_x3_split", "unimm_x3_split_wt", "unimm_x3_layernorm_bwd_partials", "unimm_embed_bwd_f32", "unimm_x3_lm_loss_bwd",
           "unimm_x3_kl_loss_bwd", "unimm_x3_rows_add", "unimm_x3_attn_fwd", "unimm_x3_attn_bwd", "unimm_x3_attn_set_impl", "unimm_x3_layernorm_fwd", "unimm_prof_tag", "unimm_prof_tagged",
           "unimm_sum_dropout", "unimm_sum_dropout_bwd", "unimm_mse_loss_fwd", "unimm_mse_loss_bwd", "unimm_host_mask_pack", "unimm_host_memcpy",
           "unimm_attn_decode", "unimm_kv_cache_update", "unimm_lm_topk"]


def _check(rc, what):
    if rc != 0:
        raise UnimmHipError(f"{what} failed: {_ERR.get(rc, rc)}")


_tls = threading.local()


def scoped_stream():
    return getattr(_tls, "stream", None)


def _stream():
    s = getattr(_tls, "stream", None)
    if s is not None:
        return s
    return C.c_void_p(torch.cuda.current_stream().cuda_stream)


class stream_scope:

    def __init__(self, stream):
        self.ptr = C.c_void_p(stream.cuda_stream)

    def __enter__(self):
        self.old, _tls.stream = getattr(_tls, "stream", None), self.ptr
        return self

    def __exit__(self, *exc):
        _tls.stream = self.old
        return False


def _ptr(t):
    return C.c_void_p(t.data_ptr()) if t is not None else C.c_void_p(0)


def _P(t):
    return t.data_ptr() if t is not None else None


def _salt(*drops):
    for d in drops:
        if d is not None and len(d) > 3 and d[3] is not None:
            return d[3].data_ptr()
    return None


def _dev(*ts):
    for t in ts:
        if t is not None and not t.is_cuda:
            raise UnimmHipError("unimm_amd kernels need device tensors (got a CPU tensor)")


def gemm_nt(x, w, out, bias=None, epilogue=EPI_BIAS, aux=None, out2=None, drop=None, M=None, N=None, K=None, aux_ln=None, tile=0,
            splitk=0, splitk_ws=None):
    _dev(x, w, out, bias, aux, out2)
    st = getattr(_tls, "nt", None)
    if st is None:
        a = GemmNtArgs()
        st = _tls.nt = (a, C.addressof(a), lib().unimm_gemm_nt)
    a, addr, fn = st
    a.x, a.w, a.out = x.data_ptr(), w.data_ptr(), out.data_ptr()
    a.bias = bias.data_ptr() if bias is not None else None
    a.out2 = out2.data_ptr() if out2 is not None else None
    if aux is not None:
        a.aux, a.ldaux = aux.data_ptr(), aux.stride(0)
    else:
        a.aux, a.ldaux = None, 0
    a.M = x.shape[0] if M is None else M
    a.N = w.shape[0] if N is None else N
    a.K = x.shape[1] if K is None else K
    a.ldx, a.ldw, a.ldo = x.stride(0), w.stride(0), out.stride(0)
    a.epilogue = epilogue
    a.tile = tile
    a.out_f32 = 1 if out.dtype == torch.float32 else 0
    a.drop_key, a.drop_thr, a.drop_scale = drop[:3] if drop is not None else (0, 0, 0.0)
    a.drop_salt = _salt(drop)
    if splitk_ws is not None and splitk not in (0, 1):
        a.splitk, a.splitk_ws, a.splitk_ws_bytes = splitk, splitk_ws.data_ptr(), splitk_ws.numel() * splitk_ws.element_size()
    else:
        a.splitk, a.splitk_ws, a.splitk_ws_bytes = 0, None, 0
    if aux_ln is not None:
        _dev(*aux_ln)
        a.aux_mean, a.aux_rstd, a.aux_gamma, a.aux_beta = (t.data_ptr() for t in aux_ln)
    else:
        a.aux_mean = a.aux_rstd = a.aux_gamma = a.aux_beta = None
    rc = fn(addr, _stream())
    if rc != 0:
        _check(rc, "unimm_gemm_nt")
    return out


def gemm_tn(dy, x, dw, M=None, N=None, K=None, dbias=None, m_dev=None):
    _dev(dy, x, dw, dbias, m_dev)
    a = GemmTnArgs()
    a.dy, a.x, a.dw, a.dbias = _ptr(dy), _ptr(x), _ptr(dw), _ptr(dbias)
    a.m_dev = _P(m_dev)
    a.M = dy.shape[0] if M is None else M
    a.N = dy.shape[1] if N is None else N
    a.K = x.shape[1] if K is None else K
    a.lddy, a.ldx, a.lddw = dy.stride(0), x.stride(0), dw.stride(0)
    _check(lib().unimm_gemm_tn(C.byref(a), _stream()), "unimm_gemm_tn")
    return dw


def gemm_tn_grouped(problems, shared=None, ws=None):
    n = len(problems)
    if n == 0:
        return
    arr = (GemmTnArgs * n)()
    for a, (dy, x, dw, M, N, K, dbias, *rest) in zip(arr, problems):
        _dev(dy, x, dw, dbias)
        a.dy, a.x, a.dw, a.dbias = dy.data_ptr(), x.data_ptr(), dw.data_ptr(), (dbias.data_ptr() if dbias is not None else None)
        a.m_dev = rest[0].data_ptr() if rest and rest[0] is not None else None
        a.overwrite = 1 if (len(rest) > 1 and rest[1]) else 0
        a.M = dy.shape[0] if M is None else M
        a.N = dy.shape[1] if N is None else N
        a.K = x.shape[1] if K is None else K
        a.lddy, a.ldx, a.lddw = dy.stride(0), x.stride(0), dw.stride(0)
    if shared is None and ws is None:
        _check(lib().unimm_gemm_tn_grouped(C.addressof(arr), n, _stream()), "unimm_gemm_tn_grouped")
        return
    _check(lib().unimm_gemm_tn_grouped_ws(C.addressof(arr), n, int(shared or 0), _P(ws),
                                          ws.numel() if ws is not None else 0, _stream()), "unimm_gemm_tn_grouped_ws")


class AttnArgs(C.Structure):
    _fields_ = [("q", C.c_void_p), ("k", C.c_void_p), ("v", C.c_void_p), ("out", C.c_void_p),
                ("lse", C.c_void_p), ("mask", C.c_void_p),
                ("q_off", C.c_void_p), ("q_len", C.c_void_p), ("k_off", C.c_void_p), ("k_len", C.c_void_p),
# ... 149 lines not shown

def mask_pack(mask, out=None):
    _dev(mask)
    if mask.dtype not in _DT:
        raise UnimmHipError(f"mask dtype {mask.dtype} not supported (bool, uint8, int32, int64, float32)")
    mask = mask.contiguous()
    t = mask.shape[-1]
    rows = mask.numel() // t
    nw = (t + 31) // 32
    if out is None:
        out = torch.empty(mask.shape[:-1] + (nw,), dtype=torch.int32, device=mask.device)
    _check(lib().unimm_mask_pack(_ptr(mask), _DT[mask.dtype], _ptr(out), C.c_int64(rows), C.c_int32(t), _stream()),
           "unimm_mask_pack")
    return out


def host_mask_pack(mask, out=None, threads=0):
    if mask.is_cuda:
        raise UnimmHipError("host_mask_pack takes a CPU tensor (device masks: mask_pack)")
    if mask.dtype not in _DT:
        raise UnimmHipError(f"mask dtype {mask.dtype} not supported (bool, uint8, int32, int64, float32)")
    mask = mask.contiguous()
    t = mask.shape[-1]
    rows = mask.numel() // t
    nw = (t + 31) // 32
    if out is None:
        out = torch.empty(mask.shape[:-1] + (nw,), dtype=torch.int32)
    if out.is_cuda or out.dtype != torch.int32 or out.numel() != rows * nw or not out.is_contiguous():
        raise UnimmHipError("host_mask_pack: out must be a contiguous int32 CPU tensor of rows x ceil(T/32) words")
    _check(lib().unimm_host_mask_pack(C.c_void_p(mask.data_ptr()), _DT[mask.dtype], C.c_void_p(out.data_ptr()), C.c_int64(rows),
                                      C.c_int32(t), C.c_int32(threads)), "unimm_host_mask_pack")
    return out


def host_copy(dst, src, threads=0):
    if (dst.is_cuda or src.is_cuda or dst.dtype != src.dtype or dst.shape != src.shape or not dst.is_contiguous()
            or not src.is_contiguous() or src.numel() * src.element_size() < (8 << 20)):
        dst.copy_(src)
        return dst
    _check(lib().unimm_host_memcpy(C.c_void_p(dst.data_ptr()), C.c_void_p(src.data_ptr()), C.c_int64(src.numel() * src.element_size()),
                                   C.c_int32(threads)), "unimm_host_memcpy")
    return dst


def colpartials_bytes(H):
    return int(lib().unimm_colpartials_bytes(C.c_int32(H)))


class FinishDesc(C.Structure):
    _fields_ = [("partials", C.c_void_p), ("dst", C.c_void_p * 4), ("blocks", C.c_int32), ("nq", C.c_int32), ("H", C.c_int32),
                ("pad_", C.c_int32)]


def layernorm_bwd_partials(dy, x, mean, rstd, gamma, dx, dx_drop, partials, M, H, drop=None, out_drop=None, m_dev=None):
    drop = drop or NO_DROP
    out_drop = out_drop or NO_DROP
    _dev(dy, x, mean, rstd, gamma, dx, dx_drop, partials)
    blocks = C.c_int32(0)
    rc = lib().unimm_layernorm_bwd_partials(dy.data_ptr(), x.data_ptr(), mean.data_ptr(), rstd.data_ptr(), gamma.data_ptr(),
                                            dx.data_ptr(), _P(dx_drop), partials.data_ptr(), M, H, drop[0], drop[1], drop[2],
                                            out_drop[0], out_drop[1], out_drop[2], C.addressof(blocks), _P(m_dev),
                                            _salt(drop, out_drop), _stream())
    if rc != 0:
        _check(rc, "unimm_layernorm_bwd_partials")
    return blocks.value


def colpartials_finish_grouped(pending):
    n = len(pending)
    if n == 0:
        return
    arr = (FinishDesc * n)()
    for d, (part, blocks, H, dsts) in zip(arr, pending):
        d.partials, d.blocks, d.nq, d.H = part.data_ptr(), blocks, len(dsts), H
        for q, t in enumerate(dsts):
            d.dst[q] = t.data_ptr() if t is not None else None
    _check(lib().unimm_colpartials_finish_grouped(C.addressof(arr), n, _stream()), "unimm_colpartials_finish_grouped")


def layernorm_fwd(x, gamma, beta, y32, y16, mean, rstd, M, H, eps=1e-12, drop=NO_DROP):
    _dev(x, gamma, beta, y32, y16, mean, rstd)
    rc = lib().unimm_layernorm_fwd(x.data_ptr(), gamma.data_ptr(), beta.data_ptr(), _P(y32), _P(y16), _P(mean), _P(rstd), M, H, eps,
                                   drop[0], drop[1], drop[2], _salt(drop), _stream())
    if rc != 0:
        _check(rc, "unimm_layernorm_fwd")


def layernorm_bwd(dy, x, mean, rstd, gamma, dx, dx_drop, dgamma, dbeta, dbias, partials, M, H, drop=NO_DROP,
                  out_drop=NO_DROP):
    _dev(dy, x, mean, rstd, gamma, dx, dx_drop, dgamma, dbeta, dbias, partials)
    _check(lib().unimm_layernorm_bwd(_P(dy), _P(x), _P(mean), _P(rstd), _P(gamma), _P(dx), _P(dx_drop),
                                     _P(dgamma), _P(dbeta), _P(dbias), _P(partials), M, H, drop[0], drop[1], drop[2],
                                     out_drop[0], out_drop[1], out_drop[2], _salt(drop, out_drop), _stream()), "unimm_layernorm_bwd")


class EmbedArgs(C.Structure):
    _fields_ = [("ids", C.c_void_p), ("pos", C.c_void_p), ("typ", C.c_void_p),
                ("word", C.c_void_p), ("post", C.c_void_p), ("type", C.c_void_p), ("ext", C.c_void_p),
                ("gamma", C.c_void_p), ("beta", C.c_void_p),
                ("M", C.c_int32), ("H", C.c_int32), ("type_vocab", C.c_int32), ("eps", C.c_float),
                ("drop_key", C.c_uint32), ("drop_thr", C.c_uint32), ("drop_scale", C.c_float),
                ("m_dev", C.c_void_p), ("rows", C.c_void_p), ("drop_salt", C.c_void_p)]


def _embed_args(ids, pos, typ, word, post, type_, ext, gamma, beta, M, H, type_vocab, eps, drop, m_dev=None, rows=None):
    _dev(ids, pos, typ, word, post, type_, ext, gamma, beta, m_dev, rows)
    a = EmbedArgs()
    a.ids, a.pos, a.typ = _ptr(ids), _ptr(pos), _ptr(typ)
    a.word, a.post, a.type, a.ext = _ptr(word), _ptr(post), _ptr(type_), _ptr(ext)
    a.gamma, a.beta = _ptr(gamma), _ptr(beta)
    a.M, a.H, a.type_vocab, a.eps = M, H, type_vocab, eps
    a.drop_key, a.drop_thr, a.drop_scale = drop[:3]
    a.drop_salt = _salt(drop)
    a.m_dev, a.rows = _P(m_dev), _P(rows)
    return a
# ... 14 lines not shown
                                 _ptr(dbeta), _ptr(partials), _stream()), "unimm_embed_bwd")


def colsum(dy, db, M, N):
    _dev(dy, db)
    _check(lib().unimm_colsum(_ptr(dy), _ptr(db), C.c_int32(M), C.c_int32(N), C.c_int32(dy.stride(0)), _stream()),
           "unimm_colsum")


def cast_f32_bf16(src, dst, n=None):
    _dev(src, dst)
    _check(lib().unimm_cast_f32_bf16(_ptr(src), _ptr(dst), C.c_int64(src.numel() if n is None else n), _stream()),
           "unimm_cast_f32_bf16")


def mask_synth(mode, length, nans, T):
    _dev(mode, length, nans)
    B, nw = mode.numel(), (T + 31) // 32
    text = torch.empty((B, T, nw), dtype=torch.int32, device=mode.device)
    co = torch.empty((B, nw), dtype=torch.int32, device=mode.device)
    _check(lib().unimm_mask_synth(_ptr(mode), _ptr(length), _ptr(nans), _ptr(text), _ptr(co), C.c_int32(B), C.c_int32(T),
                                  _stream()), "unimm_mask_synth")
    return text, co


def plan_lengths(text_mask, co_mask, R, labels, weights, nsp_weight, B, T, image_label=None):
    tw, tq, tb = text_mask if text_mask is not None else (None, 0, 0)
    cw, cq, cb = co_mask if co_mask is not None else (None, 0, 0)
    ref = tw if tw is not None else (cw if cw is not None else labels)
    header = torch.zeros(3 * B + 2, dtype=torch.int32, device=ref.device)
    _dev(tw, cw, labels, weights, nsp_weight, image_label)
    _check(lib().unimm_plan_lengths(_ptr(tw), C.c_int32(tq), C.c_int32(tb), _ptr(cw), C.c_int32(cq), C.c_int32(cb), C.c_int32(R),
                                    _ptr(labels), _ptr(weights), _ptr(nsp_weight), _ptr(image_label), C.c_int32(B), C.c_int32(T),
                                    _ptr(header),
                                    _stream()), "unimm_plan_lengths")
    return header


def plan_build(header, labels, weights, B, T, Mv, n_lm, want_rows=True, dims=None):
    dev = header.device
    i32 = lambda n: torch.empty(max(n, 1), dtype=torch.int32, device=dev)
    off, lens = i32(B), i32(B)
    rows = torch.empty(Mv, dtype=torch.int64, device=dev) if want_rows else None
    inv = torch.empty(B * T, dtype=torch.int64, device=dev) if want_rows else None
    lm = [i32(n_lm) for _ in range(4)] if (n_lm > 0 and labels is not None) else [None] * 4
    di, df = dims if dims is not None else (None, None)
    _dev(di, df)
    order = i32(B)
    _check(lib().unimm_plan_build(_ptr(header), _ptr(labels), _ptr(weights), C.c_int32(B), C.c_int32(T), _ptr(off), _ptr(lens),
                                  _ptr(rows), _ptr(inv), *[_ptr(t) for t in lm], C.c_int32(Mv if want_rows else 0),
                                  C.c_int32(n_lm if lm[0] is not None else 0), _ptr(di), _ptr(df), _ptr(order), _stream()),
           "unimm_plan_build")
    return dict(off=off, lens=lens, rows=rows, inv=inv, lm_pos=lm[0], lm_idx=lm[1], lm_label=lm[2], lm_weight=lm[3], order=order)


def transpose_cast(src, dst, R, C_, ldd):
    _dev(src, dst)
    _check(lib().unimm_transpose_cast(_ptr(src), _ptr(dst), C.c_int32(R), C.c_int32(C_), C.c_int32(ldd), _stream()),
           "unimm_transpose_cast")


def transpose_bf16(src, dst, R, C_):
    _dev(src, dst)
    _check(lib().unimm_transpose_bf16(_ptr(src), _ptr(dst), C.c_int32(R), C.c_int32(C_), C.c_int32(src.stride(0)),
                                      C.c_int32(dst.stride(0)), _stream()), "unimm_transpose_bf16")


def sum_slabs_bf16(slabs, out, n):
    _dev(slabs, out)
    _check(lib().unimm_sum_slabs_bf16(_ptr(slabs), C.c_int32(slabs.shape[0]), C.c_int64(slabs.stride(0)), _ptr(out),
                                      C.c_int64(n), _stream()), "unimm_sum_slabs_bf16")


class TransposeDesc(C.Structure):
    _fields_ = [("src", C.c_void_p), ("dst", C.c_void_p), ("R", C.c_int32), ("C", C.c_int32), ("ldd", C.c_int32),
                ("tile0", C.c_int32)]


def transpose_table(entries, device):
    arr = (TransposeDesc * len(entries))()
    tiles = 0
    for d, (src, dst) in zip(arr, entries):
        _dev(src, dst)
        R, Cc = src.shape
        d.src, d.dst, d.R, d.C, d.ldd, d.tile0 = src.data_ptr(), dst.data_ptr(), R, Cc, dst.shape[1], tiles
        tiles += ((Cc + 31) // 32) * ((dst.shape[1] + 31) // 32)
    raw = torch.frombuffer(bytearray(bytes(arr)), dtype=torch.uint8).to(device)
    return raw, len(entries), tiles


def transpose_cast_grouped(table, count, tiles):
    _check(lib().unimm_transpose_cast_grouped(_ptr(table), C.c_int32(count), C.c_int32(tiles), _stream()),
           "unimm_transpose_cast_grouped")


def pack_image(feat, loc, out, rows, F, ld):
    _dev(feat, loc, out)
    _check(lib().unimm_pack_image(_ptr(feat), _ptr(loc), _ptr(out), C.c_int32(rows), C.c_int32(F), C.c_int32(ld),
                                  _stream()), "unimm_pack_image")


def mul_dropout(a, b, out, n, drop=NO_DROP, fusion_sum=False):
    _dev(a, b, out)
    fn = lib().unimm_sum_dropout if fusion_sum else lib().unimm_mul_dropout
    _check(fn(_ptr(a), _ptr(b), _ptr(out), C.c_int64(n), C.c_uint32(drop[0]), C.c_uint32(drop[1]),
                                   C.c_float(drop[2]), C.c_void_p(_salt(drop)), _stream()), "unimm_mul_dropout")
# ... 337 lines not shown
```

unimm_amd/modeling.py:

```python
from __future__ import annotations

import logging
import os
import warnings

import torch
from torch import nn

from . import params as PM
from .config import BertConfig
from .engine import Engine

logger = logging.getLogger(__name__)


def _build_param_tree(root: nn.Module, cfg) -> None:
    for name, shape in PM.state_dict_names(cfg).items():
        if name == PM.TIED_DECODER:
            continue
        parts = name.split(".")
        mod = root
        for part in parts[:-1]:
            if not hasattr(mod, part):
                mod.add_module(part, nn.Module())
# ... 9 lines not shown
    root.cls.predictions.decoder.register_parameter("weight", root.bert.embeddings.word_embeddings.weight)


def load_pretrained_state_dict(model: nn.Module, state_dict, default_gpu=True):
    sd = {}
    for key, v in state_dict.items():
        new_key = key
        if "gamma" in new_key:
            new_key = new_key.replace("gamma", "weight")
        if "beta" in new_key:
            new_key = new_key.replace("beta", "bias")
        if new_key.startswith("bert_pretrained."):
            new_key = new_key[len("bert_pretrained."):]
        sd[new_key] = v
    start_prefix = ""
    if not hasattr(model, "bert") and any(k.startswith("bert.") for k in sd):
        start_prefix = "bert."
    own = model.state_dict()
    missing, errors, usable = [], [], {}
    for k, t in own.items():
        src = sd.get(start_prefix + k)
        if src is None:
            missing.append(k)
        elif tuple(src.shape) != tuple(t.shape):
            errors.append(f"size mismatch for {k}: copying a param with shape {tuple(src.shape)} from checkpoint, "
                          f"the shape in current model is {tuple(t.shape)}.")
        else:
            usable[k] = src
    expected = {start_prefix + k for k in own}
    unexpected = [k for k in sd if k not in expected]
    if errors and default_gpu:
        raise RuntimeError("Error(s) in loading state_dict for {}:\n\t{}".format(model.__class__.__name__, "\n\t".join(errors)))
    model.load_state_dict(usable, strict=False)
    if missing and default_gpu:
        logger.info("Weights of {} not initialized from pretrained model: {}".format(model.__class__.__name__, missing))
    if unexpected and default_gpu:
        logger.info("Weights from pretrained model not used in {}: {}".format(model.__class__.__name__, unexpected))
    return missing, unexpected


class _HotPath(torch.autograd.Function):

    @staticmethod
    def forward(ctx, anchor, engine, inp, opts):
        ctx.set_materialize_grads(False)
        ctx.graph_entry = None
        if engine.graphs is not None and engine.graphs.eligible(inp, opts):
            res = engine.graphs.forward(inp, opts)
            if res is not None:
                ctx.engine, ctx.out, ctx.graph_entry = engine, None, res[4]
                ctx.graph_token = res[4].out.pop("_token", None)
                engine.last_seq_t = (None, None)
                return res[0], res[1], res[2], res[3]
        out = engine.forward(inp, train=opts["train"], save=True, lm_rows="labelled", want_pred_v=True)
        losses = engine.losses(out, inp)
        ctx.engine, ctx.out = engine, out
        engine.last_seq_t = (engine.padded(out, out["seq32_t"]) if opts["want_seq"] else None,
                             engine.padded(out, out["seq_out_t"]) if opts["want_seq"] else None)
        nsp = out["nsp"].clone()
        return losses["lm_loss"], losses["img_loss"], losses["nsp_loss"], nsp

    @staticmethod
    def backward(ctx, g_lm, g_img, g_nsp, g_scores):
        engine, out = ctx.engine, ctx.out
        ctx.out = None
        if ctx.graph_entry is not None:
            engine.graphs.backward(ctx.graph_entry, g_lm, g_img, g_nsp, g_scores)
            ctx.graph_token = None
            return None, None, None, None
        engine.backward(out, g_lm, g_img, g_nsp, g_scores)
        return None, None, None, None


class BertForMultiModalPreTraining(nn.Module):

    def __init__(self, config, compute_dtype="bf16"):
        super().__init__()
        if not isinstance(config, BertConfig):
            raise ValueError(
                "Parameter config in `{}(config)` should be an instance of class `BertConfig`. ".format(
                    self.__class__.__name__))
        self.config = config
        _build_param_tree(self, config)
        self.predict_feature = config.predict_feature
        if compute_dtype not in ("bf16", "fp32x3"):
            raise ValueError(f"compute_dtype must be 'bf16' or 'fp32x3', got {compute_dtype!r}")
        self.compute_dtype = compute_dtype
        if compute_dtype == "fp32x3":
            from .engine_x3 import EngineX3
            self._engine = EngineX3(self, config)
        else:
            self._engine = Engine(self, config)
        self.register_load_state_dict_post_hook(lambda module, incompatible: module._engine.invalidate_weights())

    @classmethod
    def from_pretrained(cls, pretrained_model_name_or_path, config, default_gpu=True, state_dict=None, *inputs, **kwargs):
        model = cls(config, *inputs, **kwargs)
        if state_dict is None and isinstance(pretrained_model_name_or_path, str):
            path = pretrained_model_name_or_path
            if os.path.isdir(path):
                path = os.path.join(path, "pytorch_model.bin")
            if os.path.isfile(path):
                state_dict = torch.load(path, map_location="cpu")
        if state_dict is None:
            warnings.warn(f"from_pretrained({pretrained_model_name_or_path!r}): no local weights found, "
                          "keeping random initialisation (no network access)")
            return model
# ... 46 lines not shown
            return lm_loss, img_loss, nsp_loss, seq_t, pred_t, nsp
        att = ([], [], [])
        with torch.no_grad():
            if output_all_attention_masks:
                out, att = eng.forward_with_attention(inp, train=self.training, lm_rows="all" if _want_lm_scores else "none",
                                                      want_pred_v=_want_pred_v)
            else:
                out = eng.forward(inp, train=self.training, save=False, lm_rows="all" if _want_lm_scores else "none",
                                  want_pred_v=_want_pred_v)
        seq_t = eng.padded(out, out["seq32_t"]).view(B, T, H)
        return out.get("pred_t"), out.get("pred_v"), out["nsp"], seq_t, att

    def forward_backward(self, input_ids, image_feat, image_loc, loss_weights, sep_indices=None, sep_len=None, token_type_ids=None,
                         position_ids=None, attention_mask=None, image_attention_mask=None, co_attention_mask=None,
                         masked_lm_labels=None, image_label=None, image_target=None, next_sentence_label=None, nsp_weight=None,
                         lm_weight=None, image_index=None, plan_header=None):
        if masked_lm_labels is None or next_sentence_label is None or image_target is None:
            raise ValueError("forward_backward needs the training inputs (masked_lm_labels, next_sentence_label, image_target)")
        eng = self._engine
        dev = self._device()
        eng.ensure(dev)
        inp = dict(input_ids=input_ids, image_feat=image_feat, image_loc=image_loc, token_type_ids=token_type_ids,
                   position_ids=position_ids, attention_mask=attention_mask, image_attention_mask=image_attention_mask,
                   co_attention_mask=co_attention_mask, masked_lm_labels=masked_lm_labels, image_label=image_label,
                   image_target=image_target, next_sentence_label=next_sentence_label, nsp_weight=nsp_weight,
                   lm_weight=lm_weight, image_index=image_index)
        eng.stage_host_inputs(inp)
        if plan_header is not None:
            inp["_plan_header"] = plan_header
        if self.training:
            eng.step += 1
        c_lm, c_nsp, c_img = (float(c) for c in loss_weights)
        key = (c_lm, c_nsp, c_img, dev)
        seeds = self._fb_seeds.get(key) if hasattr(self, "_fb_seeds") else None
        if seeds is None:
            if not hasattr(self, "_fb_seeds"):
                self._fb_seeds = {}
            w = torch.tensor([c_lm, c_img, c_nsp], dtype=torch.float32, device=dev)
            seeds = self._fb_seeds[key] = (w[0:1], w[1:2], w[2:3], w)
        g_lm, g_img, g_nsp, w = seeds
        opts = dict(train=self.training, want_seq=False)
        with torch.no_grad():
            res = None
            if eng.graphs is not None and eng.graphs.eligible(inp, opts):
                res = eng.graphs.forward(inp, opts, defer_outputs=True)
            if res is not None:
                ent = res[4]
                tok = ent.out.pop("_token", None)
                eng.graphs.backward(ent, g_lm, g_img, g_nsp, None)
                del tok
                lm_loss, img_loss, nsp_loss, nsp = eng.graphs.outputs(ent)
            else:
                inp.pop("_plan_header", None)
                out = eng.forward(inp, train=self.training, save=True, lm_rows="labelled", want_pred_v=True)
                ls = eng.losses(out, inp)
                lm_loss, img_loss, nsp_loss, nsp = ls["lm_loss"], ls["img_loss"], ls["nsp_loss"], out["nsp"].clone()
                eng.backward(out, g_lm.reshape(lm_loss.shape), g_img.reshape(img_loss.shape), g_nsp.reshape(nsp_loss.shape), None)
            eng.last_seq_t = None
            loss = torch.cat((lm_loss.reshape(1), img_loss.reshape(1), nsp_loss.reshape(1))).dot(w).reshape(())
        return loss, lm_loss, img_loss, nsp_loss, nsp

    def _device(self):
        return self.bert.embeddings.word_embeddings.weight.device

    @torch.no_grad()
    def sequence_log_likelihood(self, input_ids, image_feat, image_loc, masked_lm_labels, average=False, shared_context=None, **kw):
        if shared_context is not None and self.compute_dtype == "bf16":
            from .scoring import sequence_log_likelihood_shared
            return sequence_log_likelihood_shared(self, input_ids, image_feat, image_loc, masked_lm_labels, shared_context,
                                                  average=average, **kw)
        eng = self._engine
        eng.ensure(self._device())
        inp = dict(input_ids=input_ids, image_feat=image_feat, image_loc=image_loc, masked_lm_labels=masked_lm_labels,
                   lm_weight=None, **kw)
        eng.stage_host_inputs(inp)
        out = eng.forward(inp, train=False, save=False, lm_rows="labelled", want_pred_v=False)
        input_ids = inp["input_ids"]
        B, T = input_ids.shape
        scores = torch.zeros(B, dtype=torch.float32, device=eng.arena.device)
        lm = out.get("lm")
        if lm is not None:
            from . import lib as L
            seg = (lm["pos_idx"] // T).to(torch.int32)
            L.segment_sum(lm["rownll"], seg, scores, lm["n"], -1.0)
            if average:
                cnt = torch.bincount(seg.long(), minlength=B).clamp_min(1)
                scores = scores / cnt
        return scores, out["nsp"]

    @torch.no_grad()
    def generate_answers(self, input_ids, image_feat, image_loc, context_len, token_type_ids=None, position_ids=None,
                         image_attention_mask=None, image_index=None, *, beams=1, max_answer_len=20, min_answer_len=1,
                         length_penalty=0.0, banned_tokens=(0, 101, 103)):
        from .generation import generate_answers
        return generate_answers(self, input_ids, image_feat, image_loc, context_len, token_type_ids, position_ids,
                                image_attention_mask, image_index, beams=beams, max_answer_len=max_answer_len,
                                min_answer_len=min_answer_len, length_penalty=length_penalty, banned_tokens=banned_tokens)


class VisualDialogEncoder(nn.Module):

    def __init__(self, config_path, pretrained="bert-base-uncased", compute_dtype="bf16"):
        super().__init__()
        config = BertConfig.from_json_file(config_path)
        with warnings.catch_warnings():
            warnings.simplefilter("ignore")
            self.bert_pretrained = BertForMultiModalPreTraining.from_pretrained(pretrained, config, compute_dtype=compute_dtype)
# ... 45 lines not shown
```

Measured before the change: 6017 dialog-sequences/sec.

## Compute last text layer only on LM-labelled and CLS rows

Adds an optional sparse path for the final text encoder layer. Its attention output, FFN and layernorm are computed only for rows that feed a loss: the masked-LM labelled tokens plus the first token of each sequence. A new device kernel builds the sparse row index and the LM-to-sparse index map. The GEMM epilogue and layernorm backward gain a row-remap array so dropout masks stay tied to the original row ids. Wgrad scheduling is adjusted to the reduced row counts. This removes most of the last layer's dense FFN and projection work, at the cost of gather/scatter passes and extra planning kernels. The path is off unless the engine flag is enabled.

```diff
diff --git a/include/unimm_hip.h b/include/unimm_hip.h
--- a/include/unimm_hip.h
+++ b/include/unimm_hip.h
@@ -50,6 +50,7 @@
   void* splitk_ws;
   int64_t splitk_ws_bytes;
   int32_t splitk;
+  const int32_t* drop_rows;
 } unimm_gemm_nt_args;
 
 int unimm_gemm_nt(const unimm_gemm_nt_args* args, void* stream);
@@ -124,6 +125,9 @@
                      int32_t* off, int32_t* lens, int64_t* rows, int64_t* inv, int32_t* lm_pos, int32_t* lm_idx,
                      int32_t* lm_label, int32_t* lm_weight, int32_t rows_cap, int32_t lm_cap, int32_t* dims_i, float* dims_f,
                      int32_t* order, void* stream);
+int unimm_plan_sparse(const int32_t* header, const int32_t* labels, const int32_t* weights, const int32_t* off, int32_t B,
+                      int32_t T, int32_t* s_off, int32_t* s_row, int32_t* lm_sidx, int32_t rows_cap, int32_t s_cap,
+                      int32_t lm_cap, int32_t* n_s, void* stream);
 
 int unimm_layernorm_fwd(const float* x, const float* gamma, const float* beta, float* y32, void* y16, float* mean,
                         float* rstd, int32_t M, int32_t H, float eps, uint32_t drop_key, uint32_t drop_thr,
@@ -139,7 +143,7 @@
                                  void* dx, void* dx_drop, float* partials, int32_t M, int32_t H, uint32_t drop_key,
                                  uint32_t drop_thr, float drop_scale, uint32_t odrop_key, uint32_t odrop_thr,
                                  float odrop_scale, int32_t* blocks_out, const int32_t* m_dev, const uint32_t* drop_salt,
-                                 void* stream);
+                                 const int32_t* drop_rows, void* stream);
 #define UNIMM_FINISH_MAX 8
 typedef struct {
   const float* partials;
diff --git a/unimm_amd/bucket_plan.py b/unimm_amd/bucket_plan.py
--- a/unimm_amd/bucket_plan.py
+++ b/unimm_amd/bucket_plan.py
@@ -41,7 +41,7 @@
 
 
 def backward_events(cfg, n_seq: int, text_rows: int, lm_rows: int, regions: int = 37, dual_stream: bool = True,
-                    image_head_side: bool = True):
+                    image_head_side: bool = True, sparse_last_text_layer: bool = False):
     del dual_stream
     H, Hv, Hb = cfg.hidden_size, cfg.v_hidden_size, cfg.bi_hidden_size
     I, Iv = cfg.intermediate_size, cfg.v_intermediate_size
@@ -80,6 +80,11 @@
                 ev.append(("b", f"v{i}", bool(img), False, False))
         for kind, i in seg:
             if kind == "t":
+                if sparse_last_text_layer and lm_rows > 0 and (kind, i) == sched[-1]:
+                    blk = _self_block(H, I)
+                    ev += [("w", 0, lm_rows + n_seq, n, k) for n, k in blk[:3]] + [("w", 0, Mt, *blk[3])]
+                    ev.append(("b", f"t{i}", False, False, False))
+                    continue
                 ev += [("w", 0, Mt, n, k) for n, k in _self_block(H, I)]
                 ev.append(("b", f"t{i}", False, False, False))
         if pos < len(entries):
@@ -94,7 +99,8 @@
     return ev
 
 
-def hand_overs(cfg, n_seq, text_rows, lm_rows, regions=37, wgrad_group_rounds=2, dual_stream=True, image_head_side=True):
+def hand_overs(cfg, n_seq, text_rows, lm_rows, regions=37, wgrad_group_rounds=2, dual_stream=True, image_head_side=True,
+               sparse_last_text_layer=False):
     q = [[], []]
     nq, nf = [0, 0], [0, 0]
     pending, calls, launches = [], [], []
@@ -108,7 +114,7 @@
     def due(side):
         return flush_due(len(q[side]), sum(big_tiles_of(*p) for p in q[side]), wgrad_group_rounds)
 
-    for e in backward_events(cfg, n_seq, text_rows, lm_rows, regions, dual_stream, image_head_side):
+    for e in backward_events(cfg, n_seq, text_rows, lm_rows, regions, dual_stream, image_head_side, sparse_last_text_layer):
         if e[0] == "w":
             _, side, M, N, K = e
             q[side].append((M, N, K))
diff --git a/unimm_amd/csrc/api.hip b/unimm_amd/csrc/api.hip
--- a/unimm_amd/csrc/api.hip
+++ b/unimm_amd/csrc/api.hip
@@ -1,4 +1,4 @@
 #include "common.h"
 
-extern "C" int unimm_version(void) { return 19; }
+extern "C" int unimm_version(void) { return 20; }
 extern "C" const char* unimm_arch(void) { return "gfx950"; }
diff --git a/unimm_amd/csrc/gemm.hip b/unimm_amd/csrc/gemm.hip
--- a/unimm_amd/csrc/gemm.hip
+++ b/unimm_amd/csrc/gemm.hip
@@ -638,6 +638,8 @@
   hipStream_t s = (hipStream_t)stream;
   const bool f32 = a->out_f32 != 0;
   p.ksplit = 1; p.slabs = nullptr; p.counters = nullptr;
+  if (a->drop_rows != nullptr && a->epilogue != UNIMM_EPI_BIAS_DROP_RESID) return UNIMM_E_ARG;
+  p.drop_rows = a->drop_rows;
   if (a->splitk != 0 && a->splitk != 1 && (a->splitk_ws == nullptr || a->splitk_ws_bytes < 32768 || ((uintptr_t)a->splitk_ws & 255) ||
                                            a->splitk > 8 || a->splitk < -1))
     return UNIMM_E_ARG;
diff --git a/unimm_amd/csrc/gemm_nt.h b/unimm_amd/csrc/gemm_nt.h
--- a/unimm_amd/csrc/gemm_nt.h
+++ b/unimm_amd/csrc/gemm_nt.h
@@ -11,6 +11,7 @@
   DropoutArg drop;
   const float* aux_mean; const float* aux_rstd; const float* aux_gamma; const float* aux_beta;
   int ksplit; float* slabs; int* counters;
+  const int32_t* drop_rows;
 };
 struct NtSplit { int want; void* ws; long ws_bytes; };
 
@@ -356,9 +357,10 @@
             for (int e = 0; e < 8; ++e) a[e] = (a[e] - mu) * rs * lg[e] + lb[e];
           }
           if (p.drop.thr != 0u) {
+            const uint32_t dm = p.drop_rows != nullptr ? (uint32_t)p.drop_rows[m] : (uint32_t)m;
             const uint32_t kb = (SPLITCOL && FAST)
-                ? (drop_bits4(p.drop, (uint32_t)m, (uint32_t)p.N, (uint32_t)colA) | (drop_bits4(p.drop, (uint32_t)m, (uint32_t)p.N, (uint32_t)colB) << 4))
-                : drop_bits8(p.drop, (uint32_t)m, (uint32_t)p.N, (uint32_t)n);
+                ? (drop_bits4(p.drop, dm, (uint32_t)p.N, (uint32_t)colA) | (drop_bits4(p.drop, dm, (uint32_t)p.N, (uint32_t)colB) << 4))
+                : drop_bits8(p.drop, dm, (uint32_t)p.N, (uint32_t)n);
 #pragma unroll
             for (int e = 0; e < 8; ++e) v[e] = ((kb >> e) & 1u) ? v[e] * p.drop.scale : 0.f;
           }
diff --git a/unimm_amd/csrc/rowops.hip b/unimm_amd/csrc/rowops.hip
--- a/unimm_amd/csrc/rowops.hip
+++ b/unimm_amd/csrc/rowops.hip
@@ -220,6 +220,49 @@
 }
 
 
+__global__ __launch_bounds__(256) void plan_sparse_kernel(const int32_t* __restrict__ header, const int32_t* __restrict__ labels,
+                                                          const int32_t* __restrict__ weights, const int32_t* __restrict__ off,
+                                                          int B, int T, int32_t* __restrict__ s_off, int32_t* __restrict__ s_row,
+                                                          int32_t* __restrict__ lm_sidx, int rows_cap, int s_cap, int lm_cap,
+                                                          int32_t* __restrict__ n_s) {
+  __shared__ int pa[4], pc[4], wave_s[4], wave_l[4];
+  const int b = blockIdx.x, t = threadIdx.x;
+  const bool last = b == (int)gridDim.x - 1;
+  const int upto = last ? B : b;
+  int a = 0, c = 0;
+  for (int i = t; i < upto; i += 256) {
+    const bool sel0 = weights != nullptr ? weights[(size_t)i * T] != 0 : labels[(size_t)i * T] != -1;
+    const int cnt = header[B + i];
+    c += cnt;
+    a += cnt + (sel0 ? 0 : 1);
+  }
+  for (int o = 32; o > 0; o >>= 1) { a += __shfl_xor(a, o, 64); c += __shfl_xor(c, o, 64); }
+  if ((t & 63) == 0) { pa[t >> 6] = a; pc[t >> 6] = c; }
+  __syncthreads();
+  const int s0 = pa[0] + pa[1] + pa[2] + pa[3], l0 = pc[0] + pc[1] + pc[2] + pc[3];
+  if (last) {
+    if (t == 0) n_s[0] = min(s0, s_cap);
+    for (int i = s0 + t; i < s_cap; i += 256) s_row[i] = 0;
+    for (int i = l0 + t; i < lm_cap; i += 256) lm_sidx[i] = 0;
+    return;
+  }
+  if (t == 0) s_off[b] = min(s0, s_cap - 1);
+  const bool sel = t < T && (weights != nullptr ? weights[(size_t)b * T + t] != 0 : labels[(size_t)b * T + t] != -1);
+  const bool member = sel || t == 0;
+  const unsigned long long bs = __ballot(member), bl = __ballot(sel);
+  const int lane = t & 63, wv = t >> 6;
+  if (lane == 0) { wave_s[wv] = __popcll(bs); wave_l[wv] = __popcll(bl); }
+  __syncthreads();
+  if (!member) return;
+  const unsigned long long below = (1ull << lane) - 1ull;
+  int rs = __popcll(bs & below), rl = __popcll(bl & below);
+  for (int w = 0; w < wv; ++w) { rs += wave_s[w]; rl += wave_l[w]; }
+  const int dst = s0 + rs;
+  if (dst < s_cap) s_row[dst] = min(off[b] + t, rows_cap - 1);
+  if (sel && l0 + rl < lm_cap) lm_sidx[l0 + rl] = min(dst, s_cap - 1);
+}
+
+
 __global__ __launch_bounds__(256) void layernorm_fwd_kernel(const float* __restrict__ x, const float* __restrict__ gamma,
                                                             const float* __restrict__ beta, float* __restrict__ y32,
                                                             bf16_t* __restrict__ y,
@@ -263,7 +306,8 @@
                                                             const float* __restrict__ gamma, bf16_t* __restrict__ dx,
                                                             bf16_t* __restrict__ dx_drop, float* __restrict__ partials,
                                                             int M, int H, DropoutArg drop, DropoutArg out_drop,
-                                                            const int32_t* __restrict__ m_dev) {
+                                                            const int32_t* __restrict__ m_dev,
+                                                            const int32_t* __restrict__ drop_rows) {
   __shared__ float red[4 * 1024];
   drop_resolve(drop);
   drop_resolve(out_drop);
@@ -282,6 +326,7 @@
   u32x4 pdy[MAXC];
   f32x4 pxa[MAXC], pxb[MAXC];
   float pmean = 0.f, prstd = 0.f;
+  int pdrow = 0;
 #define UNIMM_LNB_PREFETCH(r_)                                                                                 \
   {                                                                                                            \
     _Pragma("unroll") for (int i = 0; i < MAXC; ++i) {                                                         \
@@ -293,6 +338,7 @@
       }                                                                                                        \
     }                                                                                                          \
     pmean = mean_i[r_]; prstd = rstd_i[r_];                                                                    \
+    pdrow = drop_rows != nullptr ? drop_rows[r_] : (r_);                                                       \
   }
   if (wave < M) UNIMM_LNB_PREFETCH(wave)
   for (int row = wave; row < M; row += nwaves) {
@@ -313,6 +359,7 @@
       }
     }
     const float mean = pmean, rstd = prstd;
+    const int drow = pdrow;
     if (row + nwaves < M) UNIMM_LNB_PREFETCH(row + nwaves)
     float s1 = 0.f, s2 = 0.f;
 #pragma unroll
@@ -337,7 +384,7 @@
     Row8 dd;
 #pragma unroll
     for (int i = 0; i < MAXC; ++i) {
-      const uint32_t kb = drop.thr != 0u ? drop_bits8(drop, (uint32_t)row, (uint32_t)H, (uint32_t)((lane + 64 * i) * 8)) : 0u;
+      const uint32_t kb = drop.thr != 0u ? drop_bits8(drop, (uint32_t)drow, (uint32_t)H, (uint32_t)((lane + 64 * i) * 8)) : 0u;
 #pragma unroll
       for (int j = 0; j < 8; ++j) {
         const float v = rstd * (dyv.v[i][j] - s1 - xv.v[i][j] * s2);
@@ -775,6 +822,16 @@
 __global__ void gather_rows_kernel(const bf16_t* __restrict__ src, const int32_t* __restrict__ idx, bf16_t* __restrict__ dst,
                                    int n, int H, int scatter, const int32_t* __restrict__ n_dev) {
   if (n_dev != nullptr) n = min(n, n_dev[0]);
+  if (H % 8) {
+    const size_t total = (size_t)n * H, stride = (size_t)gridDim.x * blockDim.x;
+    for (size_t i = (size_t)blockIdx.x * blockDim.x + threadIdx.x; i < total; i += stride) {
+      const int r = (int)(i / H), c = (int)(i % H);
+      const int g = idx[r];
+      if (scatter) dst[(size_t)g * H + c] = src[(size_t)r * H + c];
+      else dst[(size_t)r * H + c] = src[(size_t)g * H + c];
+    }
+    return;
+  }
   const int cpr = H / 8;
   size_t i = (size_t)blockIdx.x * blockDim.x + threadIdx.x;
   const size_t total = (size_t)n * cpr;
@@ -832,7 +889,8 @@
   hipStream_t s = (hipStream_t)stream;
   hipLaunchKernelGGL(layernorm_bwd_kernel, dim3(blocks), dim3(256), 0, s, (const bf16_t*)dy, x, mean, rstd,
                      gamma, (bf16_t*)dx, (bf16_t*)dx_drop, partials, M, H, mk_drop(drop_key, drop_thr, drop_scale, drop_salt),
-                     mk_drop(odrop_key, odrop_thr, odrop_scale, drop_salt), (const int32_t*)nullptr);
+                     mk_drop(odrop_key, odrop_thr, odrop_scale, drop_salt), (const int32_t*)nullptr,
+                     (const int32_t*)nullptr);
   UNIMM_CHECK_LAUNCH();
   hipLaunchKernelGGL(colpartials_finish_kernel, dim3((H + 63) / 64, 3), dim3(1024), 0, s, partials, blocks, 3, H, dgamma,
                      dbeta, dbias, (float*)nullptr);
@@ -844,14 +902,14 @@
                                             const float* gamma, void* dx, void* dx_drop, float* partials, int32_t M, int32_t H,
                                             uint32_t drop_key, uint32_t drop_thr, float drop_scale, uint32_t odrop_key,
                                             uint32_t odrop_thr, float odrop_scale, int32_t* blocks_out, const int32_t* m_dev,
-                                            const uint32_t* drop_salt, void* stream) {
+                                            const uint32_t* drop_salt, const int32_t* drop_rows, void* stream) {
   if (!dy || !x || !mean || !rstd || !gamma || !dx || !partials || !blocks_out) return UNIMM_E_ARG;
   if (M <= 0 || H <= 0 || H > MAXC * 512 || (H % 8)) return UNIMM_E_SHAPE;
   int blocks = (M + 3) / 4;
   blocks = blocks > RED_BLOCKS ? RED_BLOCKS : blocks;
   hipLaunchKernelGGL(layernorm_bwd_kernel, dim3(blocks), dim3(256), 0, (hipStream_t)stream, (const bf16_t*)dy, x, mean, rstd,
                      gamma, (bf16_t*)dx, (bf16_t*)dx_drop, partials, M, H, mk_drop(drop_key, drop_thr, drop_scale, drop_salt),
-                     mk_drop(odrop_key, odrop_thr, odrop_scale, drop_salt), m_dev);
+                     mk_drop(odrop_key, odrop_thr, odrop_scale, drop_salt), m_dev, drop_rows);
   UNIMM_CHECK_LAUNCH();
   *blocks_out = blocks;
   return UNIMM_OK;
@@ -958,6 +1016,17 @@
   return UNIMM_OK;
 }
 
+extern "C" int unimm_plan_sparse(const int32_t* header, const int32_t* labels, const int32_t* weights, const int32_t* off,
+                                 int32_t B, int32_t T, int32_t* s_off, int32_t* s_row, int32_t* lm_sidx, int32_t rows_cap,
+                                 int32_t s_cap, int32_t lm_cap, int32_t* n_s, void* stream) {
+  if (!header || !labels || !off || !s_off || !s_row || !lm_sidx || !n_s) return UNIMM_E_ARG;
+  if (B <= 0 || T <= 0 || T > 256 || rows_cap < 1 || s_cap < 1 || lm_cap < 0) return UNIMM_E_SHAPE;
+  hipLaunchKernelGGL(plan_sparse_kernel, dim3(B + 1), dim3(256), 0, (hipStream_t)stream, header, labels, weights, off, B, T,
+                     s_off, s_row, lm_sidx, rows_cap, s_cap, lm_cap, n_s);
+  UNIMM_CHECK_LAUNCH();
+  return UNIMM_OK;
+}
+
 extern "C" int unimm_colsum(const void* dy, float* db, int32_t M, int32_t N, int32_t ld, void* stream) {
   if (!dy || !db) return UNIMM_E_ARG;
   if (M <= 0 || N <= 0 || (ld % 8) || ld < ((N + 7) & ~7)) return UNIMM_E_ALIGN;
@@ -1090,8 +1159,8 @@
 
 extern "C" int unimm_gather_rows(const void* src, const int32_t* idx, void* dst, int32_t n, int32_t H, int32_t scatter,
                                  const int32_t* n_dev, void* stream) {
-  if (!src || !idx || !dst || n <= 0 || H <= 0 || (H % 8)) return UNIMM_E_ARG;
-  size_t blocks = ((size_t)n * (H / 8) + 255) / 256;
+  if (!src || !idx || !dst || n <= 0 || H <= 0) return UNIMM_E_ARG;
+  size_t blocks = ((size_t)n * ((H % 8) ? H : H / 8) + 255) / 256;
   blocks = blocks > 8192 ? 8192 : blocks;
   hipLaunchKernelGGL(gather_rows_kernel, dim3((unsigned)blocks), dim3(256), 0, (hipStream_t)stream, (const bf16_t*)src, idx,
                      (bf16_t*)dst, n, H, scatter, n_dev);
diff --git a/unimm_amd/engine.py b/unimm_amd/engine.py
--- a/unimm_amd/engine.py
+++ b/unimm_amd/engine.py
@@ -103,13 +103,15 @@
         self._nq = [0, 0]
         self._nf = [0, 0]
         self._reported = set()
+        self.sparse_last_text_layer = False
         self.host_staging = True
         self._stager = None
 
     def schedule_key(self):
         return (self.dual_stream, self.unpad, self.lazy_ln, self.gemm_tile, self.wgrad_group_rounds, self.wgrad_stream, self.splitk,
                 self.attn_longest_first, self.wgrad_overwrite, tuple(sorted(self.tile_table.items())), self.image_tile,
-                self.small_rows, self.image_head_side, self.skinny_dx_rows, self.wgrad_ws_bytes, self.text_priority)
+                self.small_rows, self.image_head_side, self.skinny_dx_rows, self.wgrad_ws_bytes, self.text_priority,
+                self.sparse_last_text_layer)
 
     def register_arena_user(self, obj):
         import weakref
@@ -276,7 +278,8 @@
             return DR.drop_arg(p, DR.site_key(self.seed, _site(name))) + (self.salt_word,)
         return DR.drop_arg(p, DR.make_key(self.seed, self.step, _site(name)))
 
-    def _linear(self, x, lin, epi=L.EPI_BIAS, aux=None, want_u=False, drop=None, out_f32=False, ldo=None, M=None, out=None):
+    def _linear(self, x, lin, epi=L.EPI_BIAS, aux=None, want_u=False, drop=None, out_f32=False, ldo=None, M=None, out=None,
+                drop_rows=None):
         M = x.shape[0] if M is None else M
         ldo = ldo or lin.N
         if out is None:
@@ -288,10 +291,10 @@
         sk = self._splitk(M, lin.N, lin.K)
         if sk is not None:
             L.gemm_nt(x, lin.w, out, bias=lin.bias, epilogue=epi, aux=aux, out2=u, drop=drop, M=M, N=lin.N, K=lin.K, aux_ln=aux_ln,
-                      tile=sk[0], splitk=sk[1], splitk_ws=sk[2])
+                      tile=sk[0], splitk=sk[1], splitk_ws=sk[2], drop_rows=drop_rows)
         else:
             L.gemm_nt(x, lin.w, out, bias=lin.bias, epilogue=epi, aux=aux, out2=u, drop=drop, M=M, N=lin.N, K=lin.K, aux_ln=aux_ln,
-                      tile=self._tile(M, lin.N, lin.K))
+                      tile=self._tile(M, lin.N, lin.K), drop_rows=drop_rows)
         return (out, u) if want_u else out
 
     def _tile(self, M, N, K=None):
@@ -549,17 +552,20 @@
         for t in reads:
             self._touch(t, main)
 
-    def _layernorm_bwd(self, dy, x, mean, rstd, key, dbias=None, drop=L.NO_DROP, out_drop=L.NO_DROP, defer=True, m_dev=None):
+    def _layernorm_bwd(self, dy, x, mean, rstd, key, dbias=None, drop=L.NO_DROP, out_drop=L.NO_DROP, defer=True, m_dev=None,
+                       drop_rows=None):
         gmm, _, gg, gb = self.ln[key]
         M, H = x.shape
         dx = torch.empty((M, H), dtype=BF16, device=x.device)
         dxd = torch.empty((M, H), dtype=BF16, device=x.device) if drop[1] != 0 else None
         if not defer:
+            assert drop_rows is None
             scratch = (self.part_side if self._on_side else self.part)[H]
             L.layernorm_bwd(dy, x, mean, rstd, gmm, dx, dxd, gg, gb, dbias, scratch, M, H, drop=drop, out_drop=out_drop)
             return dx, (dxd if dxd is not None else dx)
         part = torch.empty(self.part[H].numel(), dtype=F32, device=x.device)
-        blocks = L.layernorm_bwd_partials(dy, x, mean, rstd, gmm, dx, dxd, part, M, H, drop=drop, out_drop=out_drop, m_dev=m_dev)
+        blocks = L.layernorm_bwd_partials(dy, x, mean, rstd, gmm, dx, dxd, part, M, H, drop=drop, out_drop=out_drop, m_dev=m_dev,
+                                          drop_rows=drop_rows)
         (self._fq_img if self._on_side else self._fq).append((part, blocks, H, [gg, gb, dbias]))
         return dx, (dxd if dxd is not None else dx)
 
@@ -608,6 +614,60 @@
                            B, heads, T, T, D, 1.0 / math.sqrt(D), mq, mb, d_attn, qvar=var, kvar=var)
                 return self._linear_bwd(dqkv, x, qkv_l, L.EPI_ADD, aux=dpre1, m_dev=md)
             tape.append((key, bwd))
+        return x2_32, x2
+
+    @staticmethod
+    def _rows(x, idx, n):
+        out = torch.empty((n,) + tuple(x.shape[1:]), dtype=x.dtype, device=x.device)
+        w = (x.shape[1] if x.dim() == 2 else 1) * (2 if x.dtype == F32 else 1)
+        L.gather_rows(x.view(BF16) if x.dtype == F32 else x, idx, out.view(BF16) if x.dtype == F32 else out, n, w)
+        return out
+
+    def _self_block_sparse(self, key, x32, x, mask, B, T, heads, pname, p_attn, p_hid, st, var, sp):
+        train, tape = st["train"], st["tape"]
+        Hd = x.shape[1]
+        D = Hd // heads
+        qkv_l, so, ff1, ff2 = (self.lin[key + s] for s in (".qkv", ".so", ".ff1", ".ff2"))
+        srow, ns, Ms = sp["s_row"], sp["n_s"], sp["cap"]
+        qkv = self._linear(x, qkv_l)
+        q, k, v = qkv[:, :Hd], qkv[:, Hd:2 * Hd], qkv[:, 2 * Hd:]
+        d_attn = self._drop(pname + "attn", p_attn, train)
+        ctx, lse = self._attn(q, k, v, mask, B, heads, T, T, D, d_attn, True, qvar=var, kvar=var, tag=key)
+        ctx_s = self._rows(ctx, srow, Ms)
+        if isinstance(x32, _LazyLN):
+            x32_s = _LazyLN(self._rows(x32.x, srow, Ms), self._rows(x32.mean, srow, Ms), self._rows(x32.rstd, srow, Ms),
+                            x32.gamma, x32.beta)
+        else:
+            x32_s = self._rows(x32, srow, Ms)
+        d_so = self._drop(pname + "so", p_hid, train)
+        pre1 = self._linear(ctx_s, so, L.EPI_BIAS_DROP_RESID, aux=x32_s, drop=d_so, out_f32=True, drop_rows=srow)
+        x1_32, x1, m1, r1 = self._layernorm(pre1, key + ".ln1", True, lazy=True)
+        h, u = self._linear(x1, ff1, L.EPI_BIAS_GELU_DG, want_u=True)
+        d_out = self._drop(pname + "out", p_hid, train)
+        pre2 = self._linear(h, ff2, L.EPI_BIAS_DROP_RESID, aux=x1_32, drop=d_out, out_f32=True, drop_rows=srow)
+        x2_32, x2, m2, r2 = self._layernorm(pre2, key + ".ln2", True, lazy=True)
+        md = var[2]
+        Mt = x.shape[0]
+
+        def spread(g_s):
+            g = torch.zeros((Mt, Hd), dtype=BF16, device=g_s.device)
+            L.gather_rows(g_s, srow, g, Ms, Hd, scatter=True, n_dev=ns)
+            return g
+
+        def bwd(dx2):
+            dpre2, dpre2d = self._layernorm_bwd(dx2, pre2, m2, r2, key + ".ln2", dbias=ff2.gb, drop=d_out, m_dev=ns, drop_rows=srow)
+            du = self._linear_bwd(dpre2d, h, ff2, L.EPI_MUL, aux=u, bias_grad=False, m_dev=ns)
+            dx1 = self._linear_bwd(du, x1, ff1, L.EPI_ADD, aux=dpre2, m_dev=ns)
+            dpre1, dpre1d = self._layernorm_bwd(dx1, pre1, m1, r1, key + ".ln1", dbias=so.gb, drop=d_so, m_dev=ns, drop_rows=srow)
+            dctx_s = self._linear_bwd(dpre1d, ctx_s, so, bias_grad=False, m_dev=ns)
+            dctx = spread(dctx_s)
+            dqkv = torch.empty_like(qkv)
+            delta = torch.empty_like(lse)
+            words, mq, mb = mask
+            L.attn_bwd(q, k, v, ctx, dctx, lse, delta, dqkv[:, :Hd], dqkv[:, Hd:2 * Hd], dqkv[:, 2 * Hd:], words,
+                       B, heads, T, T, D, 1.0 / math.sqrt(D), mq, mb, d_attn, qvar=var, kvar=var)
+            return self._linear_bwd(dqkv, x, qkv_l, L.EPI_ADD, aux=spread(dpre1), m_dev=md)
+        tape.append((key, bwd))
         return x2_32, x2
 
     def _conn_block(self, key, i, xv32, xv, xt32, xt, B, R, T, vmask, comask, st, var=None):
@@ -777,8 +837,8 @@
         header = L.plan_lengths(tmask, comask, R, lab32, w32, nw_dev, B, T, image_label=il32)
         return header.tolist()
 
-    def forward(self, inp: dict, train: bool, save: bool, lm_rows: str, want_pred_v: bool):
-        return self._on_text_stream(self._forward, inp, train, save, lm_rows, want_pred_v)
+    def forward(self, inp: dict, train: bool, save: bool, lm_rows: str, want_pred_v: bool, want_seq: bool = True):
+        return self._on_text_stream(self._forward, inp, train, save, lm_rows, want_pred_v, want_seq)
 
     def forward_with_attention(self, inp, train, lm_rows, want_pred_v):
         was = (self.unpad, self.dual_stream, self.attn_sink)
@@ -891,9 +951,9 @@
         self._step_rows = Mt
 
         return dict(ids32=ids32, typ32=typ32, pos32=pos32, labels=labels, lab32=lab32, w32=w32, il32=il32, plan=plan, sel=sel,
-                    n_img=n_img, dyn=dyn, st_nspw=st_nspw, var=var, Mt=Mt)
-
-    def _forward(self, inp: dict, train: bool, save: bool, lm_rows: str, want_pred_v: bool):
+                    n_img=n_img, dyn=dyn, st_nspw=st_nspw, var=var, Mt=Mt, header=header if plan is not None else None)
+
+    def _forward(self, inp: dict, train: bool, save: bool, lm_rows: str, want_pred_v: bool, want_seq: bool = True):
         cfg = self.cfg
         dev = self.arena.device
         self.refresh_weights()
@@ -963,6 +1023,11 @@
 
         sched = PM.encoder_schedule(cfg)
         st_frozen = dict(train=train, tape=None)
+        sp = None
+        if (self.sparse_last_text_layer and save and not want_seq and lm_rows == "labelled" and plan is not None and sel is not None
+                and sel["n"] > 0 and self.attn_sink is None and sched and sched[-1][0] == "t" and sched[-1][1] >= cfg.fixed_t_layer):
+            sp = L.plan_sparse(pl["header"], pl["lab32"], pl["w32"], var[0], B, T, Mt, sel["n"] + B, sel["n"])
+            sp["cap"] = sel["n"] + B
         pos = 0
         while pos < len(sched):
             seg = []
@@ -981,6 +1046,12 @@
             for kind, i in seg:
                 if kind == "t":
                     fz = i < cfg.fixed_t_layer
+                    if sp is not None and (kind, i) == sched[-1]:
+                        xt32, xt = self._self_block_sparse(f"t{i}", xt32, xt, tmask, B, T, cfg.num_attention_heads,
+                                                           f"bert.encoder.layer.{i}.", cfg.attention_probs_dropout_prob,
+                                                           cfg.hidden_dropout_prob, st, var, sp)
+                        tape[-1] = ("t", tape[-1][0], tape[-1][1])
+                        continue
                     xt32, xt = self._self_block(f"t{i}", xt32, xt, tmask, B, T, cfg.num_attention_heads, f"bert.encoder.layer.{i}.",
                                                 cfg.attention_probs_dropout_prob, cfg.hidden_dropout_prob, st_frozen if fz else st, var=var)
                     if save and not fz:
@@ -1011,11 +1082,13 @@
         seq_t, seq_v = xt, xv
 
         xt32, xv32 = self._dense32(xt32), self._dense32(xv32)
-        out = dict(seq_out_t=seq_t, seq_out_v=seq_v, seq32_t=xt32, seq32_v=xv32, B=B, T=T, R=R, plan=plan, Mt=Mt,
-                   nsp_weight_host=st_nspw, n_img=n_img, img_label32=il32, dyn=dyn, img=img)
+        out = dict(seq_out_t=seq_t if sp is None else None, seq_out_v=seq_v, seq32_t=xt32 if sp is None else None, seq32_v=xv32,
+                   B=B, T=T, R=R, plan=plan, Mt=Mt, nsp_weight_host=st_nspw, n_img=n_img, img_label32=il32, dyn=dyn, img=img,
+                   s_rows=sp["cap"] if sp is not None else None)
         if pred_v_out is not None:
             out["pred_v"] = pred_v_out
-        cls_idx_t = var[0] if var is not None else torch.arange(0, B * T, T, dtype=torch.int32, device=dev)
+        cls_idx_t = sp["s_off"] if sp is not None else \
+            (var[0] if var is not None else torch.arange(0, B * T, T, dtype=torch.int32, device=dev))
         cls_idx_v = torch.arange(0, B * R, R, dtype=torch.int32, device=dev)
         cls_t = torch.empty((B, H), dtype=F32, device=dev)
         cls_v = torch.empty((B, Hv), dtype=F32, device=dev)
@@ -1038,9 +1111,10 @@
             n = sel["n"]
             if n > 0:
                 xs = torch.empty((n, H), dtype=BF16, device=dev)
-                L.gather_rows(seq_t, sel["idx"], xs, n, H, n_dev=dyn["n_lm"])
+                lm_idx = sp["lm_sidx"] if sp is not None else sel["idx"]
+                L.gather_rows(seq_t, lm_idx, xs, n, H, n_dev=dyn["n_lm"])
                 lm = self._lm_head(xs, n, sel["label"], sel["weight"], save, n_dev=dyn["n_lm"])
-                lm.update(idx=sel["idx"], pos_idx=sel["pos"], n=n, n_dev=dyn["n_lm"], inv_dev=dyn["inv_lm"])
+                lm.update(idx=lm_idx, pos_idx=sel["pos"], n=n, n_dev=dyn["n_lm"], inv_dev=dyn["inv_lm"])
             out["lm"] = lm
         elif lm_rows == "all":
             out["pred_t"] = self.decode_rows(self.padded(out, seq_t), B * T).view(B, T, Vp)[:, :, :V]
@@ -1151,7 +1225,7 @@
         def gvec(g):
             return torch.zeros(1, dtype=F32, device=dev) if g is None else g.detach().to(F32).reshape(1).contiguous()
 
-        dseq_t = torch.zeros((out["Mt"], H), dtype=BF16, device=dev)
+        dseq_t = torch.zeros((out["s_rows"] if out.get("s_rows") is not None else out["Mt"], H), dtype=BF16, device=dev)
         img = out["img"]
         C = cfg.v_target_size
         itr, idec = self.lin["imgtr"], self.lin["imgdec"]
diff --git a/unimm_amd/engine_x3.py b/unimm_amd/engine_x3.py
--- a/unimm_amd/engine_x3.py
+++ b/unimm_amd/engine_x3.py
@@ -278,7 +278,7 @@
             tape.append((key, bwd))
         return ov32, ov3, ot32, ot3
 
-    def _forward(self, inp: dict, train: bool, save: bool, lm_rows: str, want_pred_v: bool):
+    def _forward(self, inp: dict, train: bool, save: bool, lm_rows: str, want_pred_v: bool, want_seq: bool = True):
         cfg = self.cfg
         if cfg.fixed_t_layer or cfg.fixed_v_layer or not cfg.with_coattention:
             raise NotImplementedError("fixed_t_layer / fixed_v_layer / with_coattention=False run on the bf16 engine only")
diff --git a/unimm_amd/graphs.py b/unimm_amd/graphs.py
--- a/unimm_amd/graphs.py
+++ b/unimm_amd/graphs.py
@@ -238,7 +238,8 @@
             torch.cuda.synchronize()
             ent.gF = _new_graph()
             with _quiet_collector(), torch.cuda.graph(ent.gF, pool=ent.pool, stream=ent.stream, capture_error_mode="thread_local"):
-                ent.out = eng.forward(ent.sin, train=opts["train"], save=True, lm_rows="labelled", want_pred_v=True)
+                ent.out = eng.forward(ent.sin, train=opts["train"], save=True, lm_rows="labelled", want_pred_v=True,
+                                      want_seq=False)
                 ent.losses = eng.losses(ent.out, ent.sin)
                 ent.nsp = ent.out["nsp"]
                 ls = ent.losses
diff --git a/unimm_amd/lib.py b/unimm_amd/lib.py
--- a/unimm_amd/lib.py
+++ b/unimm_amd/lib.py
@@ -8,7 +8,7 @@
 
 _PKG = os.path.dirname(os.path.abspath(__file__))
 LIB_PATH = os.path.join(_PKG, "libunimm_hip.so")
-ABI_VERSION = 19
+ABI_VERSION = 20
 
 EPI_BIAS, EPI_BIAS_GELU, EPI_BIAS_DROP_RESID, EPI_BIAS_RELU, EPI_DGELU, EPI_ADD, EPI_MUL, EPI_BIAS_GELU_DG = range(8)
 
@@ -28,7 +28,7 @@
                 ("drop_key", C.c_uint32), ("drop_thr", C.c_uint32), ("drop_scale", C.c_float),
                 ("aux_mean", C.c_void_p), ("aux_rstd", C.c_void_p), ("aux_gamma", C.c_void_p), ("aux_beta", C.c_void_p),
                 ("tile", C.c_int32), ("drop_salt", C.c_void_p),
-                ("splitk_ws", C.c_void_p), ("splitk_ws_bytes", C.c_int64), ("splitk", C.c_int32)]
+                ("splitk_ws", C.c_void_p), ("splitk_ws_bytes", C.c_int64), ("splitk", C.c_int32), ("drop_rows", C.c_void_p)]
 
 
 class GemmTnArgs(C.Structure):
@@ -76,7 +76,7 @@
     L.unimm_colpartials_finish_grouped.argtypes = [VP, I32, VP]
     L.unimm_layernorm_fwd.argtypes = [VP] * 7 + [I32, I32, F32, U32, U32, F32, VP, VP]
     L.unimm_x3_layernorm_fwd.argtypes = [VP] * 7 + [I32, I32, F32, U32, U32, F32, VP, VP]
-    L.unimm_layernorm_bwd_partials.argtypes = [VP] * 8 + [I32, I32, U32, U32, F32, U32, U32, F32, VP, VP, VP, VP]
+    L.unimm_layernorm_bwd_partials.argtypes = [VP] * 8 + [I32, I32, U32, U32, F32, U32, U32, F32, VP, VP, VP, VP, VP]
     L.unimm_layernorm_bwd.argtypes = [VP] * 11 + [I32, I32, U32, U32, F32, U32, U32, F32, VP, VP]
     _lib = L
     return L
@@ -87,7 +87,7 @@
            "unimm_embed_fwd", "unimm_embed_bwd", "unimm_colsum", "unimm_cast_f32_bf16", "unimm_transpose_cast",
            "unimm_pack_image", "unimm_mul_dropout", "unimm_mul_dropout_bwd", "unimm_lm_loss_fwd",
            "unimm_lm_loss_bwd", "unimm_kl_loss_fwd", "unimm_kl_loss_bwd", "unimm_nsp_loss_fwd",
-           "unimm_nsp_loss_bwd", "unimm_reduce_sum", "unimm_segment_sum", "unimm_gelu_bwd", "unimm_gather_rows", "unimm_prof_enable", "unimm_prof_collect", "unimm_adamw_step", "unimm_transpose_cast_grouped", "unimm_mask_synth", "unimm_neural_ndcg", "unimm_plan_lengths", "unimm_plan_build", "unimm_layernorm_bwd_partials",
+           "unimm_nsp_loss_bwd", "unimm_reduce_sum", "unimm_segment_sum", "unimm_gelu_bwd", "unimm_gather_rows", "unimm_prof_enable", "unimm_prof_collect", "unimm_adamw_step", "unimm_transpose_cast_grouped", "unimm_mask_synth", "unimm_neural_ndcg", "unimm_plan_lengths", "unimm_plan_build", "unimm_plan_sparse", "unimm_layernorm_bwd_partials",
            "unimm_colpartials_finish_grouped", "unimm_gemm_tn_grouped_ws", "unimm_linear_f32", "unimm_rows_add_f32", "unimm_transpose_bf16", "unimm_sum_slabs_bf16", "unimm_attn_probs",
            "unimm_x3_split", "unimm_x3_split_wt", "unimm_x3_layernorm_bwd_partials", "unimm_embed_bwd_f32", "unimm_x3_lm_loss_bwd",
            "unimm_x3_kl_loss_bwd", "unimm_x3_rows_add", "unimm_x3_attn_fwd", "unimm_x3_attn_bwd", "unimm_x3_attn_set_impl", "unimm_x3_layernorm_fwd", "unimm_prof_tag", "unimm_prof_tagged",
@@ -150,8 +150,8 @@
 
 
 def gemm_nt(x, w, out, bias=None, epilogue=EPI_BIAS, aux=None, out2=None, drop=None, M=None, N=None, K=None, aux_ln=None, tile=0,
-            splitk=0, splitk_ws=None):
-    _dev(x, w, out, bias, aux, out2)
+            splitk=0, splitk_ws=None, drop_rows=None):
+    _dev(x, w, out, bias, aux, out2, drop_rows)
     st = getattr(_tls, "nt", None)
     if st is None:
         a = GemmNtArgs()
@@ -173,6 +173,7 @@
     a.out_f32 = 1 if out.dtype == torch.float32 else 0
     a.drop_key, a.drop_thr, a.drop_scale = drop[:3] if drop is not None else (0, 0, 0.0)
     a.drop_salt = _salt(drop)
+    a.drop_rows = drop_rows.data_ptr() if drop_rows is not None else None
     if splitk_ws is not None and splitk not in (0, 1):
         a.splitk, a.splitk_ws, a.splitk_ws_bytes = splitk, splitk_ws.data_ptr(), splitk_ws.numel() * splitk_ws.element_size()
     else:
@@ -428,15 +429,16 @@
                 ("pad_", C.c_int32)]
 
 
-def layernorm_bwd_partials(dy, x, mean, rstd, gamma, dx, dx_drop, partials, M, H, drop=None, out_drop=None, m_dev=None):
+def layernorm_bwd_partials(dy, x, mean, rstd, gamma, dx, dx_drop, partials, M, H, drop=None, out_drop=None, m_dev=None,
+                           drop_rows=None):
     drop = drop or NO_DROP
     out_drop = out_drop or NO_DROP
-    _dev(dy, x, mean, rstd, gamma, dx, dx_drop, partials)
+    _dev(dy, x, mean, rstd, gamma, dx, dx_drop, partials, drop_rows)
     blocks = C.c_int32(0)
     rc = lib().unimm_layernorm_bwd_partials(dy.data_ptr(), x.data_ptr(), mean.data_ptr(), rstd.data_ptr(), gamma.data_ptr(),
                                             dx.data_ptr(), _P(dx_drop), partials.data_ptr(), M, H, drop[0], drop[1], drop[2],
                                             out_drop[0], out_drop[1], out_drop[2], C.addressof(blocks), _P(m_dev),
-                                            _salt(drop, out_drop), _stream())
+                                            _salt(drop, out_drop), _P(drop_rows), _stream())
     if rc != 0:
         _check(rc, "unimm_layernorm_bwd_partials")
     return blocks.value
@@ -557,6 +559,17 @@
                                   C.c_int32(n_lm if lm[0] is not None else 0), _ptr(di), _ptr(df), _ptr(order), _stream()),
            "unimm_plan_build")
     return dict(off=off, lens=lens, rows=rows, inv=inv, lm_pos=lm[0], lm_idx=lm[1], lm_label=lm[2], lm_weight=lm[3], order=order)
+
+
+def plan_sparse(header, labels, weights, off, B, T, rows_cap, s_cap, lm_cap):
+    dev = header.device
+    i32 = lambda n: torch.empty(max(n, 1), dtype=torch.int32, device=dev)
+    s_off, s_row, lm_sidx, n_s = i32(B), i32(s_cap), i32(lm_cap), i32(1)
+    _dev(labels, weights, off)
+    _check(lib().unimm_plan_sparse(_ptr(header), _ptr(labels), _ptr(weights), _ptr(off), C.c_int32(B), C.c_int32(T), _ptr(s_off),
+                                   _ptr(s_row), _ptr(lm_sidx), C.c_int32(rows_cap), C.c_int32(s_cap), C.c_int32(lm_cap), _ptr(n_s),
+                                   _stream()), "unimm_plan_sparse")
+    return dict(s_off=s_off, s_row=s_row, lm_sidx=lm_sidx, n_s=n_s)
 
 
 def transpose_cast(src, dst, R, C_, ldd):
diff --git a/unimm_amd/modeling.py b/unimm_amd/modeling.py
--- a/unimm_amd/modeling.py
+++ b/unimm_amd/modeling.py
@@ -85,7 +85,7 @@
                 ctx.graph_token = res[4].out.pop("_token", None)
                 engine.last_seq_t = (None, None)
                 return res[0], res[1], res[2], res[3]
-        out = engine.forward(inp, train=opts["train"], save=True, lm_rows="labelled", want_pred_v=True)
+        out = engine.forward(inp, train=opts["train"], save=True, lm_rows="labelled", want_pred_v=True, want_seq=bool(opts["want_seq"]))
         losses = engine.losses(out, inp)
         ctx.engine, ctx.out = engine, out
         engine.last_seq_t = (engine.padded(out, out["seq32_t"]) if opts["want_seq"] else None,
@@ -238,7 +238,7 @@
                 lm_loss, img_loss, nsp_loss, nsp = eng.graphs.outputs(ent)
             else:
                 inp.pop("_plan_header", None)
-                out = eng.forward(inp, train=self.training, save=True, lm_rows="labelled", want_pred_v=True)
+                out = eng.forward(inp, train=self.training, save=True, lm_rows="labelled", want_pred_v=True, want_seq=False)
                 ls = eng.losses(out, inp)
                 lm_loss, img_loss, nsp_loss, nsp = ls["lm_loss"], ls["img_loss"], ls["nsp_loss"], out["nsp"].clone()
                 eng.backward(out, g_lm.reshape(lm_loss.shape), g_img.reshape(img_loss.shape), g_nsp.reshape(nsp_loss.shape), None)
diff --git a/unimm_amd/sparse_plan.py b/unimm_amd/sparse_plan.py
--- /dev/null
+++ b/unimm_amd/sparse_plan.py
@@ -0,0 +1,25 @@
+from __future__ import annotations
+
+import numpy as np
+
+
+def plan_sparse_host(sel, off, rows_cap, s_cap, lm_cap):
+    sel = np.asarray(sel, dtype=bool)
+    B, T = sel.shape
+    s_off = np.zeros(B, dtype=np.int32)
+    s_row = np.zeros(max(s_cap, 1), dtype=np.int32)
+    lm_sidx = np.zeros(max(lm_cap, 1), dtype=np.int32)
+    s0 = l0 = 0
+    for b in range(B):
+        s_off[b] = min(s0, s_cap - 1)
+        member = sel[b].copy()
+        member[0] = True
+        for t in np.flatnonzero(member):
+            if s0 < s_cap:
+                s_row[s0] = min(int(off[b]) + int(t), rows_cap - 1)
+            if sel[b, t]:
+                if l0 < lm_cap:
+                    lm_sidx[l0] = min(s0, s_cap - 1)
+                l0 += 1
+            s0 += 1
+    return dict(s_off=s_off, s_row=s_row, lm_sidx=lm_sidx, n_s=min(s0, s_cap))
```

New measurement: 5927 dialog-sequences/sec. 1.5% lower.
